# devmentality/LEAStereo

Hardware: AMD Instinct MI355X
Metric: stereo pairs/s at 576×960 D=192, 1/2/4/8 GPU; EPE vs reference (higher is better)
Workload: dtype f32; 1 GPU; SceneFlow 576x960 D=192 fp32, batch 1 per GPU (BASELINE configs[1]); height=576, width=960, maxdisp=192, global_batch=1, parallelism=dp1 (pairs sharded over ranks, no collective in the step), launch=hip graph replay

## Files before the change

### include/leastereo_hip.h

```cpp
#ifndef LEASTEREO_HIP_H
#define LEASTEREO_HIP_H

#include <stddef.h>
#include <stdint.h>

#ifdef __cplusplus
extern "C" {
#endif

#define LEA_ABI_VERSION 14

#define LEA_F32 0
#define LEA_BF16 1

#define LEA_OK 0
#define LEA_E_INVALID 1001
#define LEA_E_UNSUPPORTED 1002

#define LEA_RELU 1u
#define LEA_RESIDUAL 2u
#define LEA_PAIR_SUM 4u

int lea_abi_version(void);
const char* lea_last_error(void);

int lea_build_cost_volume(const void* left, const void* right, void* cost,
                          int B, int C, int H, int W, int D3, int dtype, void* stream);

size_t lea_conv3d_packed_floats(int cout, int cin, int k);

int lea_conv3d_pack_weights(const float* w, float* packed, int cout, int cin, int k,
                            void* stream);

int lea_conv3d_bnrelu(const void* x, int64_t x_bstride,
                      const void* x2, int64_t x2_bstride, int cin2,
                      const float* w_packed, const float* scale, const float* shift,
                      const void* residual, int64_t r_bstride,
                      void* y, int64_t y_bstride,
                      int B, int cin, int cout, int D, int H, int W, int k,
                      unsigned flags, int dtype, void* stream);

int lea_conv3d_bnrelu_resampled(const void* x, int64_t x_bstride, int Di, int Hi, int Wi,
                                const float* w_packed, const float* scale, const float* shift,
                                const void* residual, int64_t r_bstride,
                                void* y, int64_t y_bstride,
                                int B, int cin, int cout, int D, int H, int W, int k,
                                unsigned flags, int dtype, void* stream);

int lea_conv3d_bnrelu_costvolume(const void* left, const void* right, int64_t f_bstride,
                                 const float* w_packed, const float* scale, const float* shift,
                                 void* y, int64_t y_bstride, int B, int C, int cout, int D3,
                                 int H, int W, unsigned flags, int dtype, void* stream);
const char* lea_conv3d_costvolume_kernel_name(int B, int cout, int D3, int H, int W);

const char* lea_conv3d_kernel_name(int B, int cout, int D, int H, int W, int k, int resampled);


size_t lea_conv2d_packed_floats(int cout, int cin);
int lea_conv2d_pack_weights(const float* w, float* packed, int cout, int cin, void* stream);

int lea_conv2d_bnrelu(const void* x, int64_t x_bstride, const float* w_packed,
                      const float* scale, const float* shift, const void* residual,
                      int64_t r_bstride, void* y, int64_t y_bstride, int B, int cin, int cout,
                      int H, int W, unsigned flags, int dtype, void* stream);

const char* lea_conv2d_kernel_name(int B, int cout, int H, int W);

int lea_conv2d_bnrelu_pair(const void* x, int64_t x_bstride, const float* w_packed,
                           const float* scale, const float* shift, const void* residual,
                           int64_t r_bstride, void* y, int64_t y_bstride, void* y2,
                           int64_t y2_bstride, int B, int cin, int cout, int c1, int H, int W,
                           unsigned flags, void* stream);

int lea_conv2d_s3_bnrelu(const void* x, int64_t x_bstride, const float* w, const float* scale,
                         const float* shift, void* y, int64_t y_bstride, int B, int cin, int cout,
                         int Hi, int Wi, unsigned flags, int dtype, void* stream);

int lea_feature_stem_bnrelu(const float* x, int64_t x_bstride, const float* w0, const float* scale0,
                            const float* shift0, const float* w1, const float* scale1,
                            const float* shift1, void* y, int64_t y_bstride, int B, int cin, int c0,
                            int c1, int Hi, int Wi, int dtype, void* stream);


int lea_resample3d_trilinear(const void* x, int64_t x_bstride, void* y, int64_t y_bstride,
                             int B, int C, int Di, int Hi, int Wi, int Do, int Ho, int Wo,
                             int align_corners, const float* scale, const float* shift,
                             unsigned flags, int dtype, void* stream);

size_t lea_tapsum_workspace_bytes(int B, int cout, int Hi, int Wi, int Do);
int lea_tapsum_upsample(const void* q, int64_t q_bstride, void* y, int64_t y_bstride,
                        int B, int cout, int Di, int Hi, int Wi, int Do, int Ho, int Wo,
                        const float* scale, const float* shift, unsigned flags,
                        void* workspace, int dtype, void* stream);

int lea_disparity_regression(const void* cost, float* disp, int B, int D3, int H3, int W3,
                             int maxdisp, int dtype, void* stream);

int lea_disparity_regression_stats(const void* cost, float* disp, float* entropy, float* peak,
                                   float* disp_local, int B, int D3, int H3, int W3, int maxdisp,
                                   int radius, int dtype, void* stream);

int lea_disparity_regression_right(const void* cost, float* disp_right, int B, int D3, int H3,
                                   int W3, int maxdisp, int dtype, void* stream);

int lea_disparity_lr_check(const float* disp_left, const float* disp_right, uint8_t* state,
                           float* disp_filled, int B, int H, int W, float threshold, void* stream);

int lea_median5x5_f32(const float* x, int64_t x_bstride, float* y, int64_t y_bstride, int B,
                      int H, int W, int iterations, void* stream);

size_t lea_edge_loss_workspace_bytes(int B, int H, int W);
int lea_edge_loss_f32(const float* pred, int64_t pred_bstride, const float* target,
                      int64_t target_bstride, const float* tsmooth, int64_t tsmooth_bstride,
                      int B, int H, int W, float maxdisp, double* sums, void* workspace,
                      void* stream);

int lea_edge_loss_grad_f32(const float* pred, int64_t pred_bstride, const float* target,
                           int64_t target_bstride, const float* tsmooth, int64_t tsmooth_bstride,
                           const double* sums, const float* scales, float* dpred,
                           int64_t dpred_bstride, int B, int H, int W, float maxdisp,
                           void* stream);

size_t lea_photometric_workspace_bytes(int B, int H, int W);
// ... 57 lines not shown
int lea_conv3d_bnrelu_costvolume_bf16(const void* left, const void* right, int64_t f_bstride,
                                      const void* w_packed, const float* scale, const float* shift,
                                      void* y, int64_t y_bstride, int B, int C, int cout, int D3,
                                      int H, int W, unsigned flags, void* stream);


const char* lea_conv3d_kernel_name_bf16(int B, int cout, int cin, int D, int H, int W, int k,
                                        int costvolume);

int lea_conv3d_bf16_pair_supported(int B, int cin, int cout, int D, int H, int W);

int lea_conv1x1_resampled_bf16(const void* x, int64_t x_bstride, int Di, int Hi, int Wi,
                               const void* w_packed, const float* scale, const float* shift,
                               void* y, int64_t y_bstride, int B, int cin, int cout, int D, int H,
                               int W, unsigned flags, void* stream);

int lea_resample3d_trilinear_bf16(const void* x, int64_t x_bstride, void* y, int64_t y_bstride,
                                  int B, int C, int Di, int Hi, int Wi, int Do, int Ho, int Wo,
                                  int align_corners, const float* scale, const float* shift,
                                  unsigned flags, void* stream);


int lea_to_c8_bf16(const float* x, int64_t x_bstride, void* y, int64_t y_bstride, int B, int C,
                   int64_t vol, void* stream);
int lea_from_c8_bf16(const void* x, int64_t x_bstride, float* y, int64_t y_bstride, int B, int C,
                     int64_t vol, void* stream);


size_t lea_conv2d_packed_elems_bf16(int cout, int cin);
int lea_conv2d_pack_weights_bf16(const float* w, void* packed, int cout, int cin, void* stream);
int lea_conv2d_bnrelu_bf16(const void* x, int64_t x_bstride, const void* w_packed,
                           const float* scale, const float* shift, const void* residual,
                           int64_t r_bstride, void* y, int64_t y_bstride, int B, int cin, int cout,
                           int H, int W, unsigned flags, void* stream);

size_t lea_conv3d_wino_packed_floats(int cout, int cin);
int lea_conv3d_wino_pack_weights(const float* w, float* packed, int cout, int cin, void* stream);
int lea_conv3d_bnrelu_wino(const void* x, int64_t x_bstride, const void* x2, int64_t x2_bstride,
                           int cin2, const float* w_packed, const float* scale, const float* shift,
                           const void* residual, int64_t r_bstride, void* y, int64_t y_bstride,
                           int B, int cin, int cout, int D, int H, int W, unsigned flags, int dtype,
                           void* stream);
int lea_conv3d_bnrelu_costvolume_wino(const void* left, const void* right, int64_t f_bstride,
                                      const float* w_packed, const float* scale,
                                      const float* shift, void* y, int64_t y_bstride, int B, int C,
                                      int cout, int D3, int H, int W, unsigned flags, int dtype,
                                      void* stream);
const char* lea_conv3d_wino_kernel_name(int B, int cin, int cout, int D, int H, int W, int costvolume);
int lea_conv3d_wino_down2_supported(int B, int cin, int cout, int D, int H, int W);
const char* lea_conv3d_wino_down2_kernel_name(int B, int cin, int cout, int D, int H, int W);
int lea_conv3d_bnrelu_wino_down2(const void* x, int64_t x_bstride, const float* w_packed,
                                 const float* scale, const float* shift, void* y, int64_t y_bstride,
                                 int B, int cin, int cout, int D, int H, int W, unsigned flags, int dtype,
                                 void* stream);
int lea_conv3d_wino_down2_cat_supported(int B, int cin, int cin2, int cout, int D, int H, int W);
const char* lea_conv3d_wino_down2_cat_kernel_name(int B, int cin, int cin2, int cout, int D, int H, int W);
int lea_conv3d_bnrelu_wino_down2_cat(const void* x, int64_t x_bstride, const void* x2, int64_t x2_bstride,
                                     int cin2, const float* w_packed, const float* scale, const float* shift,
                                     void* y, int64_t y_bstride, int B, int cin, int cout, int D, int H,
                                     int W, unsigned flags, int dtype, void* stream);
int lea_conv3d_wino_dp_down2_supported(int B, int cin, int cout, int D, int H, int W);
const char* lea_conv3d_wino_dp_down2_kernel_name(int B, int cin, int cout, int D, int H, int W, int only);
int lea_conv3d_bnrelu_wino_dp_down2(const void* x, int64_t x_bstride, const float* w_packed,
                                    const float* scale, const float* shift, const void* residual,
                                    int64_t r_bstride, void* y, int64_t y_bstride, void* y2,
                                    int64_t y2_bstride, int B, int cin, int cout, int D, int H, int W,
                                    unsigned flags, int dtype, void* stream);
int lea_resample3d_down2_supported(int Di, int Hi, int Wi, int Do, int Ho, int Wo, int dtype);
int lea_resample3d_trilinear_down2(const void* x, int64_t x_bstride, void* y, int64_t y_bstride, void* y2,
                                   int64_t y2_bstride, int B, int C, int Di, int Hi, int Wi, int Do, int Ho,
                                   int Wo, const float* scale, const float* shift, unsigned flags, int dtype,
                                   void* stream);

int lea_cv_stem_split_weights(const float* w, float* wl, float* wr, int cout, int C, void* stream);
int lea_cv_stem_combine(const void* lmaps, int64_t l_bstride, const void* rmaps, int64_t r_bstride,
                        const float* scale, const float* shift, void* y, int64_t y_bstride, int B,
                        int cout, int D3, int H, int W, unsigned flags, int dtype, void* stream);
int lea_cv_stem_down2_supported(int cout, int D3, int H, int W, int dtype);
int lea_cv_stem_combine_down2(const void* lmaps, int64_t l_bstride, const void* rmaps, int64_t r_bstride,
                              const float* scale, const float* shift, void* y, int64_t y_bstride,
                              void* y2, int64_t y2_bstride, int B, int cout, int D3, int H, int W,
                              unsigned flags, int dtype, void* stream);


size_t lea_standardize_workspace_bytes(int B);
int lea_standardize_crop_u8(const void* left, const void* right, int B, int H, int W,
                            int pix_stride, float* out_left, float* out_right, int crop_h,
                            int crop_w, void* workspace, void* stream);

size_t lea_train_transform_workspace_bytes(int B);
int lea_train_transform_u8(const void* left, const void* right, int B, int H, int W, int pix_stride,
                           const float* disp_left, const float* disp_right, const int* params,
                           float* out_left, float* out_right, float* out_target, int crop_h,
                           int crop_w, float maxdisp, int* n_valid, void* workspace, void* stream);


size_t lea_standardize_tiles_workspace_bytes(void);
int lea_standardize_tiles_u8(const void* left, const void* right, int H, int W, int pix_stride,
                             const int* origins, int N, float* out_left, float* out_right, int tile_h,
                             int tile_w, void* workspace, void* stream);

int lea_tile_blend_f32(const float* tiles, int64_t tile_bstride, const int* ys, int ny, const int* xs,
                       int nx, int tile_h, int tile_w, int guard_y0, int guard_y1, int guard_x0,
                       int guard_x1, int ramp, float* out, int H, int W, int* n_uncovered, void* stream);

size_t lea_disparity_metrics_workspace_bytes(int B, int H, int W);
int lea_disparity_metrics(const float* pred, int64_t pred_bstride, const float* gt,
                          int64_t gt_bstride, int B, int H, int W, float maxdisp, int round_pred,
                          int z_shift, int thr1, int thr2, int thr3, unsigned char* correct,
                          double* out, void* workspace, void* stream);


size_t lea_conv3d_wgrad_workspace_bytes(int B, int cin, int cout, int D, int H, int W, int k);
int lea_conv3d_wgrad(const float* x, const float* dz, float* dw, void* workspace, size_t ws_bytes,
                     int B, int cin, int cout, int D, int H, int W, int k, void* stream);

size_t lea_conv2d_wgrad_workspace_bytes(int B, int cin, int cout, int H, int W);
int lea_conv2d_wgrad(const float* x, const float* dz, float* dw, void* workspace, size_t ws_bytes,
                     int B, int cin, int cout, int H, int W, void* stream);

int lea_conv2d_s3_backward_data(const float* dz, const float* w, float* dx, int B, int cin, int cout,
                                int Hi, int Wi, void* stream);
size_t lea_conv2d_s3_wgrad_workspace_bytes(int B, int cin, int cout, int Hi, int Wi);
int lea_conv2d_s3_wgrad(const float* x, const float* dz, float* dw, void* workspace, size_t ws_bytes,
                        int B, int cin, int cout, int Hi, int Wi, void* stream);

int lea_conv3d_flip_weights(const float* w, float* wt, int cout, int cin, int k, void* stream);

size_t lea_bn_workspace_bytes(int C);
int lea_bn_forward_f32(const float* z, float* y, int B, int C, int64_t V, const float* gamma,
                       const float* beta, float* running_mean, float* running_var, float momentum,
                       float eps, int training, unsigned flags, float* mean, float* invstd,
                       void* workspace, void* stream);

int lea_bn_backward_f32(const float* dy, const float* y, const float* z, float* dz, int B, int C,
                        int64_t V, const float* gamma, const float* mean, const float* invstd,
                        int training, unsigned flags, float* dgamma, float* dbeta, void* workspace,
                        void* stream);

size_t lea_resample3d_backward_workspace_bytes(int B, int C, int Di, int Hi, int Wi, int Do, int Ho,
                                               int Wo);
int lea_resample3d_trilinear_backward(const float* dy, float* dx, void* workspace, size_t ws_bytes,
                                      int B, int C, int Di, int Hi, int Wi, int Do, int Ho, int Wo,
                                      int align_corners, void* stream);

int lea_disparity_regression_backward(const float* cost, const float* disp, const float* dout,
                                      float* dV, int B, int D3, int H3, int W3, int maxdisp,
                                      void* stream);

int lea_build_cost_volume_backward(const float* dcost, float* dleft, float* dright, int B, int C,
                                   int H, int W, int D3, void* stream);

#ifdef __cplusplus
}
#endif
#endif
```

### leastereo_amd/_lib.py

```python
from __future__ import annotations

import ctypes
import os
import threading

LIB_PATH = os.environ.get(
    "LEASTEREO_HIP_LIB",
    os.path.join(os.path.dirname(os.path.abspath(__file__)), "libleastereo_hip.so"))

ABI_VERSION = 14
LEA_F32 = 0
LEA_BF16 = 1
LEA_RELU = 1
LEA_RESIDUAL = 2
LEA_PAIR_SUM = 4
LEA_E_INVALID = 1001

_p = ctypes.c_void_p
_i = ctypes.c_int
_i64 = ctypes.c_int64
_u = ctypes.c_uint

SIGNATURES = {
    "lea_abi_version": (_i, []),
    "lea_last_error": (ctypes.c_char_p, []),
    "lea_build_cost_volume": (_i, [_p, _p, _p, _i, _i, _i, _i, _i, _i, _p]),
    "lea_conv3d_packed_floats": (ctypes.c_size_t, [_i, _i, _i]),
    "lea_conv3d_pack_weights": (_i, [_p, _p, _i, _i, _i, _p]),
    "lea_conv3d_bnrelu": (_i, [_p, _i64, _p, _i64, _i, _p, _p, _p, _p, _i64, _p, _i64,
                               _i, _i, _i, _i, _i, _i, _i, _u, _i, _p]),
    "lea_conv3d_bnrelu_resampled": (_i, [_p, _i64, _i, _i, _i, _p, _p, _p, _p, _i64, _p, _i64,
                                         _i, _i, _i, _i, _i, _i, _i, _u, _i, _p]),
    "lea_conv3d_kernel_name": (ctypes.c_char_p, [_i, _i, _i, _i, _i, _i, _i]),
    "lea_conv3d_set_tile_override": (_i, [_i, _i, _i]),
    "lea_conv3d_bnrelu_costvolume": (_i, [_p, _p, _i64, _p, _p, _p, _p, _i64, _i, _i, _i, _i, _i,
                                          _i, _u, _i, _p]),
    "lea_conv3d_costvolume_kernel_name": (ctypes.c_char_p, [_i, _i, _i, _i, _i]),
    "lea_conv2d_packed_floats": (ctypes.c_size_t, [_i, _i]),
    "lea_conv2d_pack_weights": (_i, [_p, _p, _i, _i, _p]),
    "lea_conv2d_bnrelu": (_i, [_p, _i64, _p, _p, _p, _p, _i64, _p, _i64, _i, _i, _i, _i, _i, _u,
                               _i, _p]),
    "lea_conv2d_kernel_name": (ctypes.c_char_p, [_i, _i, _i, _i]),
    "lea_conv2d_s3_bnrelu": (_i, [_p, _i64, _p, _p, _p, _p, _i64, _i, _i, _i, _i, _i, _u, _i, _p]),
    "lea_feature_stem_bnrelu": (_i, [_p, _i64, _p, _p, _p, _p, _p, _p, _p, _i64, _i, _i, _i, _i, _i, _i,
                                     _i, _p]),
    "lea_resample3d_trilinear": (_i, [_p, _i64, _p, _i64, _i, _i, _i, _i, _i, _i, _i, _i,
                                      _i, _p, _p, _u, _i, _p]),
    "lea_tapsum_workspace_bytes": (ctypes.c_size_t, [_i, _i, _i, _i, _i]),
    "lea_tapsum_upsample": (_i, [_p, _i64, _p, _i64, _i, _i, _i, _i, _i, _i, _i, _i, _p, _p, _u,
                                 _p, _i, _p]),
    "lea_disparity_regression": (_i, [_p, _p, _i, _i, _i, _i, _i, _i, _p]),
    "lea_disparity_regression_stats": (_i, [_p, _p, _p, _p, _p, _i, _i, _i, _i, _i, _i, _i, _p]),
    "lea_disparity_regression_right": (_i, [_p, _p, _i, _i, _i, _i, _i, _i, _p]),
    "lea_disparity_lr_check": (_i, [_p, _p, _p, _p, _i, _i, _i, ctypes.c_float, _p]),
    "lea_median5x5_f32": (_i, [_p, _i64, _p, _i64, _i, _i, _i, _i, _p]),
    "lea_edge_loss_workspace_bytes": (ctypes.c_size_t, [_i, _i, _i]),
    "lea_edge_loss_f32": (_i, [_p, _i64, _p, _i64, _p, _i64, _i, _i, _i, ctypes.c_float, _p, _p, _p]),
    "lea_edge_loss_grad_f32": (_i, [_p, _i64, _p, _i64, _p, _i64, _p, _p, _p, _i64, _i, _i, _i,
                                    ctypes.c_float, _p]),
    "lea_photometric_workspace_bytes": (ctypes.c_size_t, [_i, _i, _i]),
    "lea_photometric_f32": (_i, [_p, _i64, _p, _i64, _p, _i64, _p, _i64, _i, _i, _i, _i, ctypes.c_float,
                                 ctypes.c_float, ctypes.c_float, _p, _p, _p, _p, _p]),
    "lea_photometric_grad_f32": (_i, [_p, _i64, _p, _i64, _p, _i64, _p, _i64, _i, _i, _i, _i, ctypes.c_float,
                                      ctypes.c_float, _p, _p, _p, _i64, _p]),
    "lea_disparity_refine_workspace_bytes": (ctypes.c_size_t, [_i, _i, _i]),
    "lea_disparity_refine_f32": (_i, [_p, _i64, _p, _p, _p, _i, _i, _i, _i, ctypes.c_float, ctypes.c_float, _i,
                                      _p, _p, _p, _p]),
    "lea_disparity_speckle_workspace_bytes": (ctypes.c_size_t, [_i, _i, _i]),
    "lea_disparity_speckle_f32": (_i, [_p, _p, _i, _i, _i, ctypes.c_float, _i, ctypes.c_float, _p, _p, _p, _p, _p,
                                       _p]),
    "lea_disparity_pointcloud_workspace_bytes": (ctypes.c_size_t, [_i, _i, _i]),
    "lea_disparity_pointcloud_f32": (_i, [_p, _p, _p, _i, _p, _i64, _i, _i, _i, ctypes.c_float, ctypes.c_float,
                                          ctypes.c_float, _i, _p, _p, _p, _p, _p, _p, _p, _p, _p]),
    "lea_rectify_pair_u8": (_i, [_p, _p, _i, _i, _i, _i, _p, _i, _p, _i, _i, _i, _i, _p, _p, _p, _p, _p]),
    "lea_rectify_set_tile": (_i, [_i]),
    "lea_forward_warp_f32": (_i, [_p, _i64, _p, _i64, _p, _p, _i, _i, _i, _i, ctypes.c_float, ctypes.c_float, _i,
                                  ctypes.c_float, _p, _p, _p, _p, _p]),
    "lea_conv3d_packed_elems_bf16": (ctypes.c_size_t, [_i, _i, _i]),
    "lea_conv3d_pack_weights_bf16": (_i, [_p, _p, _i, _i, _i, _p]),
    "lea_conv3d_bnrelu_bf16": (_i, [_p, _i64, _p, _i64, _i, _p, _p, _p, _p, _i64, _p, _i64,
                                    _i, _i, _i, _i, _i, _i, _i, _u, _p]),
    "lea_conv3d_bnrelu_costvolume_bf16": (_i, [_p, _p, _i64, _p, _p, _p, _p, _i64, _i, _i, _i, _i,
                                               _i, _i, _u, _p]),
    "lea_conv3d_kernel_name_bf16": (ctypes.c_char_p, [_i, _i, _i, _i, _i, _i, _i, _i]),
    "lea_conv3d_bf16_pair_supported": (_i, [_i, _i, _i, _i, _i, _i]),
    "lea_conv3d_bf16_set_tile_override": (_i, [_i, _i, _i]),
    "lea_conv3d_bf16_set_variant": (_i, [_i]),
    "lea_resample3d_trilinear_bf16": (_i, [_p, _i64, _p, _i64, _i, _i, _i, _i, _i, _i, _i, _i,
                                           _i, _p, _p, _u, _p]),
    "lea_resample_bf16_set_batch": (_i, [_i]),
    "lea_resample_bf16_set_cols": (_i, [_i]),
    "lea_conv3d_wino_set_w22": (_i, [_i]),
    "lea_conv3d_bf16_set_pair_split": (_i, [_i]),
    "lea_disparity_set_register_form": (_i, [_i]),
    "lea_tapsum_set_rows": (_i, [_i]),
    "lea_staged_rows": (_i, [_i, _i, _i, _i, _i]),
    "lea_conv1x1_resampled_bf16": (_i, [_p, _i64, _i, _i, _i, _p, _p, _p, _p, _i64, _i, _i, _i, _i, _i,
                                        _i, _u, _p]),
    "lea_to_c8_bf16": (_i, [_p, _i64, _p, _i64, _i, _i, _i64, _p]),
    "lea_conv2d_packed_elems_bf16": (ctypes.c_size_t, [_i, _i]),
    "lea_conv2d_pack_weights_bf16": (_i, [_p, _p, _i, _i, _p]),
    "lea_conv2d_bnrelu_bf16": (_i, [_p, _i64, _p, _p, _p, _p, _i64, _p, _i64, _i, _i, _i, _i, _i,
                                    _u, _p]),
    "lea_from_c8_bf16": (_i, [_p, _i64, _p, _i64, _i, _i, _i64, _p]),
    "lea_conv3d_wino_packed_floats": (ctypes.c_size_t, [_i, _i]),
    "lea_conv3d_wino_pack_weights": (_i, [_p, _p, _i, _i, _p]),
    "lea_conv3d_bnrelu_wino": (_i, [_p, _i64, _p, _i64, _i, _p, _p, _p, _p, _i64, _p, _i64,
                                    _i, _i, _i, _i, _i, _i, _u, _i, _p]),
    "lea_conv3d_bnrelu_costvolume_wino": (_i, [_p, _p, _i64, _p, _p, _p, _p, _i64, _i, _i, _i,
                                               _i, _i, _i, _u, _i, _p]),
    "lea_conv3d_wino_kernel_name": (ctypes.c_char_p, [_i, _i, _i, _i, _i, _i, _i]),
    "lea_conv3d_wino_down2_supported": (_i, [_i, _i, _i, _i, _i, _i]),
    "lea_conv3d_wino_down2_kernel_name": (ctypes.c_char_p, [_i, _i, _i, _i, _i, _i]),
    "lea_conv3d_bnrelu_wino_down2": (_i, [_p, _i64, _p, _p, _p, _p, _i64, _i, _i, _i, _i, _i, _i, _u, _i, _p]),
    "lea_conv3d_wino_down2_cat_supported": (_i, [_i, _i, _i, _i, _i, _i, _i]),
    "lea_conv3d_wino_down2_cat_kernel_name": (ctypes.c_char_p, [_i, _i, _i, _i, _i, _i, _i]),
    "lea_conv3d_bnrelu_wino_down2_cat": (_i, [_p, _i64, _p, _i64, _i, _p, _p, _p, _p, _i64, _i, _i, _i, _i, _i, _i,
                                              _u, _i, _p]),
    "lea_conv3d_wino_dp_down2_supported": (_i, [_i, _i, _i, _i, _i, _i]),
    "lea_conv3d_wino_dp_down2_kernel_name": (ctypes.c_char_p, [_i, _i, _i, _i, _i, _i, _i]),
    "lea_conv3d_bnrelu_wino_dp_down2": (_i, [_p, _i64, _p, _p, _p, _p, _i64, _p, _i64, _p, _i64, _i, _i, _i, _i, _i,
                                             _i, _u, _i, _p]),
    "lea_resample3d_down2_supported": (_i, [_i, _i, _i, _i, _i, _i, _i]),
    "lea_resample3d_trilinear_down2": (_i, [_p, _i64, _p, _i64, _p, _i64, _i, _i, _i, _i, _i, _i, _i, _i, _p, _p,
                                            _u, _i, _p]),
    "lea_conv3d_wino_set_tile_override": (_i, [_i, _i, _i]),
    "lea_conv3d_wino_set_variant": (_i, [_i]),
    "lea_conv3d_wino2_set_walk": (_i, [_i]),
    "lea_conv3d_wino2_set_halo16": (_i, [_i]),
    "lea_conv3d_wino2_set_lane_halo16": (_i, [_i]),
    "lea_conv3d_wino_set_fence": (_i, [_i]),
    "lea_resample_set_mode": (_i, [_i]),
    "lea_conv2d_set_small": (_i, [_i]),
    "lea_conv2d_kernel_name_cin": (ctypes.c_char_p, [_i, _i, _i, _i, _i]),
    "lea_conv2d_bnrelu_pair": (_i, [_p, _i64, _p, _p, _p, _p, _i64, _p, _i64, _p, _i64, _i, _i, _i, _i, _i,
                                    _i, _u, _p]),
    "lea_conv3d_wino2_set_pipeline": (_i, [_i]),
    "lea_conv3d_wino2p_set_wpre": (_i, [_i]),
    "lea_conv3d_wino44_set": (_i, [_i]),
    "lea_conv3d_wino44_set_upre": (_i, [_i]),
    "lea_conv3d_wino44_set_sched": (_i, [_i]),
    "lea_conv3d_wino44_set_group": (_i, [_i]),
    "lea_conv3d_wino_set_epi_buf": (_i, [_i]),
    "lea_conv3d_set_rs_gather": (_i, [_i]),
    "lea_conv1x1_set_vector": (_i, [_i]),
    "lea_conv3d_bf16_set_stream1x1": (_i, [_i]),
    "lea_conv3d_wino_set_small_cout": (_i, [_i]),
    "lea_conv3d_wino_set_block48": (_i, [_i]),
    "lea_cv_stem_split_weights": (_i, [_p, _p, _p, _i, _i, _p]),
    "lea_cv_stem_combine": (_i, [_p, _i64, _p, _i64, _p, _p, _p, _i64, _i, _i, _i, _i, _i, _u, _i,
                                 _p]),
    "lea_cv_stem_down2_supported": (_i, [_i, _i, _i, _i, _i]),
    "lea_cv_stem_combine_down2": (_i, [_p, _i64, _p, _i64, _p, _p, _p, _i64, _p, _i64, _i, _i, _i, _i, _i,
                                       _u, _i, _p]),
    "lea_standardize_workspace_bytes": (ctypes.c_size_t, [_i]),
    "lea_standardize_crop_u8": (_i, [_p, _p, _i, _i, _i, _i, _p, _p, _i, _i, _p, _p]),
    "lea_train_transform_workspace_bytes": (ctypes.c_size_t, [_i]),
    "lea_train_transform_u8": (_i, [_p, _p, _i, _i, _i, _i, _p, _p, _p, _p, _p, _p, _i, _i,
                                    ctypes.c_float, _p, _p, _p]),
    "lea_standardize_tiles_workspace_bytes": (ctypes.c_size_t, []),
    "lea_standardize_tiles_u8": (_i, [_p, _p, _i, _i, _i, _p, _i, _p, _p, _i, _i, _p, _p]),
    "lea_tile_blend_f32": (_i, [_p, _i64, _p, _i, _p, _i, _i, _i, _i, _i, _i, _i, _i, _p, _i, _i, _p, _p]),
    "lea_disparity_metrics_workspace_bytes": (ctypes.c_size_t, [_i, _i, _i]),
    "lea_disparity_metrics": (_i, [_p, _i64, _p, _i64, _i, _i, _i, ctypes.c_float, _i, _i,
                                   _i, _i, _i, _p, _p, _p, _p]),
    "lea_conv3d_wgrad_workspace_bytes": (ctypes.c_size_t, [_i, _i, _i, _i, _i, _i, _i]),
    "lea_conv3d_wgrad": (_i, [_p, _p, _p, _p, ctypes.c_size_t, _i, _i, _i, _i, _i, _i, _i, _p]),
    "lea_conv2d_wgrad_workspace_bytes": (ctypes.c_size_t, [_i, _i, _i, _i, _i]),
    "lea_conv2d_wgrad": (_i, [_p, _p, _p, _p, ctypes.c_size_t, _i, _i, _i, _i, _i, _p]),
    "lea_conv2d_s3_backward_data": (_i, [_p, _p, _p, _i, _i, _i, _i, _i, _p]),
    "lea_conv2d_s3_wgrad_workspace_bytes": (ctypes.c_size_t, [_i, _i, _i, _i, _i]),
    "lea_conv2d_s3_wgrad": (_i, [_p, _p, _p, _p, ctypes.c_size_t, _i, _i, _i, _i, _i, _p]),
    "lea_conv3d_flip_weights": (_i, [_p, _p, _i, _i, _i, _p]),
    "lea_bn_workspace_bytes": (ctypes.c_size_t, [_i]),
    "lea_bn_forward_f32": (_i, [_p, _p, _i, _i, _i64, _p, _p, _p, _p, ctypes.c_float, ctypes.c_float,
                                _i, _u, _p, _p, _p, _p]),
    "lea_bn_backward_f32": (_i, [_p, _p, _p, _p, _i, _i, _i64, _p, _p, _p, _i, _u, _p, _p, _p, _p]),
    "lea_disparity_regression_backward": (_i, [_p, _p, _p, _p, _i, _i, _i, _i, _i, _p]),
    "lea_build_cost_volume_backward": (_i, [_p, _p, _p, _i, _i, _i, _i, _i, _p]),
    "lea_resample3d_backward_workspace_bytes": (ctypes.c_size_t, [_i, _i, _i, _i, _i, _i, _i, _i]),
    "lea_resample3d_trilinear_backward": (_i, [_p, _p, _p, ctypes.c_size_t, _i, _i, _i, _i, _i, _i, _i, _i,
                                               _i, _p]),
}

_lib = None
_lock = threading.Lock()


class HipKernelError(RuntimeError):
    pass


def load():
    global _lib
    if _lib is not None:
        return _lib
    with _lock:
        if _lib is None:
            if not os.path.exists(LIB_PATH):
                raise HipKernelError(
                    f"{LIB_PATH} not found: build it with `make` (hipcc --offload-arch=gfx950); "
                    "the LEAStereo hot path has no fallback")
            lib = ctypes.CDLL(LIB_PATH)
            for name, (res, args) in SIGNATURES.items():
                fn = getattr(lib, name)
                fn.restype = res
                fn.argtypes = args
            _apply_env_tuning(lib)
            _lib = lib
    return _lib


TUNING_ENV = {"LEASTEREO_WINO2_WALK": "lea_conv3d_wino2_set_walk",
              "LEASTEREO_HALO16": "lea_conv3d_wino2_set_halo16",
              "LEASTEREO_LANE_HALO16": "lea_conv3d_wino2_set_lane_halo16",
              "LEASTEREO_WINO_FENCE": "lea_conv3d_wino_set_fence",
              "LEASTEREO_RESAMPLE_MODE": "lea_resample_set_mode",
              "LEASTEREO_CONV2D_SMALL": "lea_conv2d_set_small",
              "LEASTEREO_WINO2_PIPE": "lea_conv3d_wino2_set_pipeline",
              "LEASTEREO_WINO2P_WPRE": "lea_conv3d_wino2p_set_wpre",
              "LEASTEREO_WINO44": "lea_conv3d_wino44_set",
              "LEASTEREO_WINO44_UPRE": "lea_conv3d_wino44_set_upre",
              "LEASTEREO_EPI_BUF": "lea_conv3d_wino_set_epi_buf",
              "LEASTEREO_RS_GATHER": "lea_conv3d_set_rs_gather",
              "LEASTEREO_1X1_VEC": "lea_conv1x1_set_vector",
              "LEASTEREO_BF16_1X1": "lea_conv3d_bf16_set_stream1x1",
              "LEASTEREO_RESAMPLE_K": "lea_resample_bf16_set_batch",
              "LEASTEREO_RESAMPLE_COLS": "lea_resample_bf16_set_cols",
              "LEASTEREO_W22": "lea_conv3d_wino_set_w22",
              "LEASTEREO_PAIR_SPLIT": "lea_conv3d_bf16_set_pair_split",
              "LEASTEREO_DISP_REG": "lea_disparity_set_register_form",
              "LEASTEREO_TAPSUM_ROWS": "lea_tapsum_set_rows"}


# ... 12 lines not shown
```

### leastereo_amd/csrc/conv3d.hip

```cpp
#include "conv3d_impl.h"

namespace lea {

template <int KS, int MT, int NT, int TW, bool RS>
__global__ __launch_bounds__(kConvThreads, 2) void conv3d_reg_kernel(const ConvArgs a) {
  using C = TileCfg<KS, MT, NT, TW>;
  constexpr int CIN_B = C::CIN_B;
  __shared__ __attribute__((aligned(16))) float smem[C::STAGE];
  __shared__ Axis tabs[RS ? (KS + C::RH + C::RW) : 1];
  float* xs = smem;
  float* ws = smem + C::XS;

  const int tid = threadIdx.x;
  const int lane = tid & 63;
  const int wave = tid >> 6;
  const int tile = blockIdx.x;
  const int h0 = (tile / a.tiles_w) * C::TH;
  const int w0 = (tile % a.tiles_w) * TW;
  const int d0 = blockIdx.y;
  const int b = blockIdx.z / a.ncob;
  const int co0 = (blockIdx.z - b * a.ncob) * C::COP;
  const int nchunks = (a.cin + CIN_B - 1) / CIN_B;
  const float* wp = a.wp + (long long)(co0 / C::COP) * nchunks * C::WS;
  const long long HW = (long long)a.H * a.W;
// ... 94 lines not shown
  {
    const float4* src = reinterpret_cast<const float4*>(a.wp + (long long)cob * nch * 32 * COP);
    float4* dst = reinterpret_cast<float4*>(ws);
    for (int i = threadIdx.x; i < nch * 32 * COP / 4; i += 256) dst[i] = src[i];
  }
  float sc[MT][4], sh[MT][4];
#pragma unroll
  for (int m = 0; m < MT; ++m)
#pragma unroll
    for (int r = 0; r < 4; ++r) {
      const int co = co0 + 16 * m + 4 * g + r;
      sc[m][r] = (a.scale && co < a.cout) ? a.scale[co] : 1.f;
      sh[m][r] = (a.scale && co < a.cout) ? a.shift[co] : 0.f;
    }
  __syncthreads();
  const bool relu = a.flags & LEA_RELU, resid = a.flags & LEA_RESIDUAL;
  const int HWo = a.H * a.W;
  const long long vout = (long long)HWo * a.D;
  const unsigned HWi = (unsigned)(a.Hi * a.Wi), vin = HWi * (unsigned)a.Di;
  const __amdgpu_buffer_rsrc_t xrs =
      __builtin_amdgcn_make_buffer_rsrc((void*)(a.x + (long long)b * a.xbs), 0, (int)(unsigned)((long long)a.cin * vin * 4), 0x00020000);
  const long long t0 = ((long long)blockIdx.x * 4 + wave) * tpw;
  for (int tt = 0; tt < tpw; ++tt) {
    const long long v0 = (t0 + tt) * 16;
    if (v0 >= vout) break;
    const long long v = min(v0 + n, vout - 1);
    const int od = (int)(v / HWo), rem = (int)(v - (long long)od * HWo);
    const int oh = rem / a.W, ow = rem - oh * a.W;
    const Axis ad = axis_index(a.rd, od, a.Di, a.D, 1), ah = axis_index(a.rh, oh, a.Hi, a.H, 1),
               aw = axis_index(a.rw, ow, a.Wi, a.W, 1);
    const unsigned r00 = ((unsigned)ad.i0 * HWi + (unsigned)(ah.i0 * a.Wi)) * 4u;
    const unsigned r01 = ((unsigned)ad.i0 * HWi + (unsigned)(ah.i1 * a.Wi)) * 4u;
    const unsigned r10 = ((unsigned)ad.i1 * HWi + (unsigned)(ah.i0 * a.Wi)) * 4u;
    const unsigned r11 = ((unsigned)ad.i1 * HWi + (unsigned)(ah.i1 * a.Wi)) * 4u;
    const unsigned w0 = (unsigned)aw.i0 * 4u, w1 = (unsigned)aw.i1 * 4u;
    f32x4 acc[MT];
#pragma unroll
    for (int m = 0; m < MT; ++m) acc[m] = f32x4{0.f, 0.f, 0.f, 0.f};
    for (int ch = 0; ch < nch; ++ch) {
      float c[8][8];
#pragma unroll
      for (int s = 0; s < 8; ++s) {
        const int ci = ch * 32 + 4 * s + g;
        const unsigned co = ci < a.cin ? (unsigned)ci * vin * 4u : 0u;
        const unsigned rr[4] = {r00, r01, r10, r11};
#pragma unroll
        for (int q = 0; q < 4; ++q) {
          c[s][2 * q] = __builtin_bit_cast(float, __builtin_amdgcn_raw_buffer_load_b32(xrs, co + rr[q] + w0, 0, 0));
          c[s][2 * q + 1] = __builtin_bit_cast(float, __builtin_amdgcn_raw_buffer_load_b32(xrs, co + rr[q] + w1, 0, 0));
        }
      }
#pragma unroll
      for (int s = 0; s < 8; ++s) {
        const float* e = c[s];
        const int ci = ch * 32 + 4 * s + g;
        const float bv = ci >= a.cin ? 0.f :
            ad.l0 * (ah.l0 * (aw.l0 * e[0] + aw.l1 * e[1]) + ah.l1 * (aw.l0 * e[2] + aw.l1 * e[3])) +
            ad.l1 * (ah.l0 * (aw.l0 * e[4] + aw.l1 * e[5]) + ah.l1 * (aw.l0 * e[6] + aw.l1 * e[7]));
#pragma unroll
        for (int m = 0; m < MT; ++m) {
          const int col = 16 * m + n;
          const float av = ws[ci * COP + ((SWZ && (ci & 1)) ? (col ^ 16) : col)];
          acc[m] = __builtin_amdgcn_mfma_f32_16x16x4f32(av, bv, acc[m], 0, 0, 0);
        }
      }
    }
    if (v0 + n < vout) {
#pragma unroll
      for (int m = 0; m < MT; ++m)
#pragma unroll
        for (int r = 0; r < 4; ++r) {
          const int co = co0 + 16 * m + 4 * g + r;
          if (co >= a.cout) continue;
          float y = acc[m][r] * sc[m][r] + sh[m][r];
          if (relu) y = fmaxf(y, 0.f);
          const long long o = (long long)co * vout + v0 + n;
          if (resid) y += a.res[(long long)b * a.rbs + o];
          a.y[(long long)b * a.ybs + o] = y;
        }
    }
  }
}

template <int MT, int NT, bool VEC>
__global__ __launch_bounds__(kConvThreads) void conv1x1_kernel(const ConvArgs a) {
  using P = PackCfg<1, MT>;
  constexpr int CIN_B = P::CIN_B;
  constexpr int KS = CIN_B / 4;
  using vecf = float __attribute__((ext_vector_type(NT)));
  __shared__ __attribute__((aligned(16))) float ws[P::CHUNK];
  const int tid = threadIdx.x;
  const int lane = tid & 63;
  const int wave = tid >> 6;
  const int b = blockIdx.y / a.ncob;
  const int co0 = (blockIdx.y - b * a.ncob) * P::COP;
  const int nchunks = (a.cin + CIN_B - 1) / CIN_B;
  const float* wp = a.wp + (long long)(co0 / P::COP) * nchunks * P::CHUNK;
  const long long V = (long long)a.D * a.H * a.W;
  const long long v0 = ((long long)blockIdx.x * kConvWaves + wave) * NT * 16;
  const int kq = lane >> 4, n = lane & 15;
  auto vox = [&](int j) -> long long { return VEC ? v0 + NT * n + j : v0 + j * 16 + n; };
  const bool full = VEC && vox(NT - 1) < V;

  f32x4 acc[MT][NT];
#pragma unroll
  for (int m = 0; m < MT; ++m)
#pragma unroll
    for (int j = 0; j < NT; ++j) acc[m][j] = f32x4{0.f, 0.f, 0.f, 0.f};

  for (int ch = 0; ch < nchunks; ++ch) {
    float bv[KS][NT];
#pragma unroll
    for (int s = 0; s < KS; ++s) {
      const int c = ch * CIN_B + 4 * s + kq;
      const float* src = (c < a.cin1) ? a.x + (long long)b * a.xbs + (long long)c * V
                                      : a.x2 + (long long)b * a.x2bs + (long long)(c - a.cin1) * V;
      if (VEC && full && c < a.cin) {
        const vecf t = *reinterpret_cast<const vecf*>(src + vox(0));
#pragma unroll
        for (int j = 0; j < NT; ++j) bv[s][j] = t[j];
      } else {
#pragma unroll
        for (int j = 0; j < NT; ++j) {
          const long long v = vox(j);
          bv[s][j] = (c < a.cin && v < V) ? src[v] : 0.f;
        }
      }
    }
    __syncthreads();
    {
      const float4* src = reinterpret_cast<const float4*>(wp + (long long)ch * P::CHUNK);
      float4* dst = reinterpret_cast<float4*>(ws);
#pragma unroll
      for (int i = tid; i < P::CHUNK / 4; i += kConvThreads) dst[i] = src[i];
    }
    __syncthreads();
#pragma unroll
    for (int s = 0; s < KS; ++s) {
      float av[MT];
#pragma unroll
      for (int m = 0; m < MT; ++m) av[m] = ws[(4 * s + kq) * P::COPS + a_col<1, MT>(m, kq, n)];
#pragma unroll
      for (int m = 0; m < MT; ++m)
#pragma unroll
        for (int j = 0; j < NT; ++j)
          acc[m][j] = __builtin_amdgcn_mfma_f32_16x16x4f32(av[m], bv[s][j], acc[m][j], 0, 0, 0);
    }
  }

  const bool relu = a.flags & LEA_RELU;
  const bool resid = a.flags & LEA_RESIDUAL;
#pragma unroll
  for (int m = 0; m < MT; ++m) {
#pragma unroll
    for (int r = 0; r < 4; ++r) {
      const int co = co0 + m * 16 + kq * 4 + r;
      if (co >= a.cout) continue;
      const float sc = a.scale ? a.scale[co] : 1.f;
      const float sh = a.shift ? a.shift[co] : 0.f;
      if (VEC && full) {
        const long long o = (long long)co * V + vox(0);
        vecf val;
#pragma unroll
        for (int j = 0; j < NT; ++j) {
          val[j] = acc[m][j][r] * sc + sh;
          if (relu) val[j] = fmaxf(val[j], 0.f);
        }
        if (resid) {
          const vecf rv = *reinterpret_cast<const vecf*>(a.res + (long long)b * a.rbs + o);
#pragma unroll
          for (int j = 0; j < NT; ++j) val[j] += rv[j];
        }
        *reinterpret_cast<vecf*>(a.y + (long long)b * a.ybs + o) = val;
        continue;
      }
#pragma unroll
      for (int j = 0; j < NT; ++j) {
        const long long v = vox(j);
        if (v >= V) continue;
        const long long o = (long long)co * V + v;
        float val = acc[m][j][r] * sc + sh;
        if (relu) val = fmaxf(val, 0.f);
        if (resid) val += a.res[(long long)b * a.rbs + o];
        a.y[(long long)b * a.ybs + o] = val;
      }
    }
  }
}

template <int COUT>
__global__ __launch_bounds__(kConvThreads) void conv3d_valu_kernel(const ConvArgs a) {
  constexpr int TH = 8, TW = 64, RH = TH + 2, RW = TW + 2, PLANE = RH * RW, IMG = 3 * PLANE;
  constexpr int CIN_B = PackCfg<3, 1>::CIN_B;
  constexpr int CIS = (IMG + 15) / 16 * 16;
  constexpr int STAGE = CIN_B * CIS;
  constexpr int XSLOTS = (IMG + 63) / 64;
  constexpr int XSLOTS_W = (XSLOTS + kConvWaves - 1) / kConvWaves;
  constexpr int CHUNK = PackCfg<3, 1>::CHUNK;
  __shared__ __attribute__((aligned(16))) float smem[2 * STAGE];

  const int tid = threadIdx.x;
  const int lane = tid & 63;
  const int wave = __builtin_amdgcn_readfirstlane(tid >> 6);
  const int h0 = (blockIdx.x / a.tiles_w) * TH;
  const int w0 = (blockIdx.x % a.tiles_w) * TW;
  const int d0 = blockIdx.y;
  const int b = blockIdx.z;
  const int nchunks = (a.cin + CIN_B - 1) / CIN_B;
  const int HW = a.H * a.W;
  const unsigned nrec = (unsigned)(HW * a.D) * 4u;

  unsigned voff[XSLOTS_W];
#pragma unroll
  for (int t = 0; t < XSLOTS_W; ++t) {
    const int e = (wave + kConvWaves * t) * 64 + lane;
    unsigned v = 0xFFFFFFF0u;
    if (e < IMG) {
      const int kd = e / PLANE;
      const int r = e - kd * PLANE;
      const int rr = r / RW;
      const int cc = r - rr * RW;
      const int d = d0 + kd - 1, h = h0 + rr - 1, w = w0 + cc - 1;
      if ((unsigned)d < (unsigned)a.D && (unsigned)h < (unsigned)a.H && (unsigned)w < (unsigned)a.W)
        v = (unsigned)(d * HW + h * a.W + w) * 4u;
    }
    voff[t] = v;
  }
  auto issue = [&](int ch, float* st) {
#pragma unroll
    for (int ci = 0; ci < CIN_B; ++ci) {
      const int c = ch * CIN_B + ci;
      const float* base = a.x;
      unsigned n = 0;
      if (c < a.cin1) {
        base = a.x + (long long)b * a.xbs + (long long)c * HW * a.D;
        n = nrec;
      } else if (c < a.cin) {
        base = a.x2 + (long long)b * a.x2bs + (long long)(c - a.cin1) * HW * a.D;
        n = nrec;
      }
      const __amdgpu_buffer_rsrc_t rs = __builtin_amdgcn_make_buffer_rsrc((void*)base, 0, n, 0x00020000);
#pragma unroll
      for (int t = 0; t < XSLOTS_W; ++t) {
        const int j = wave + kConvWaves * t;
        if (j < XSLOTS && j * 64 + lane < IMG)
          __builtin_amdgcn_raw_ptr_buffer_load_lds(rs, (lds_void*)(st + ci * CIS + j * 64), 4,
                                                   voff[t], 0, 0, 0);
      }
    }
  };

  const int row = tid >> 5;
  const int col = (tid & 31) * 2;
  float acc[COUT][2];
#pragma unroll
  for (int co = 0; co < COUT; ++co) acc[co][0] = acc[co][1] = 0.f;

  issue(0, smem);
  for (int ch = 0; ch < nchunks; ++ch) {
    asm volatile("s_waitcnt vmcnt(0)" ::: "memory");
    __syncthreads();
    if (ch + 1 < nchunks) issue(ch + 1, smem + ((ch + 1) & 1) * STAGE);
    const float* xs = smem + (ch & 1) * STAGE;
    const float* wc = a.wp + (long long)ch * CHUNK;
#pragma unroll
    for (int ci = 0; ci < CIN_B; ++ci) {
#pragma unroll
      for (int kd = 0; kd < 3; ++kd) {
#pragma unroll
        for (int kh = 0; kh < 3; ++kh) {
// ... 125 lines not shown

inline Plan make_plan(int B, int cout, int D, int H, int W, int k, bool resample) {
  Plan p;
  p.td = 1;
  p.mt = mt_for(cout);
  if (k == 1 && resample && g_rs_gather && (long long)B * D * H * W <= 131072) {
    p.engine = 5;
    p.nt = 0;
    p.tw = 0;
    return p;
  }
  if (k == 1 && !resample) {
    p.engine = 1;
    p.nt = 4;
    p.tw = 0;
    const long long vox = (long long)D * H * W;
    if ((vox + kConvWaves * 64 - 1) / (kConvWaves * 64) * B < 512) p.nt = 2;
    return p;
  }
  if (k == 3 && cout <= 2 && !resample) {
    p.engine = 3;
    p.mt = cout;
    p.nt = 0;
    p.tw = 64;
    return p;
  }
  if (depth_paired(cout, k) && !resample) {
    p.engine = 4;
    p.mt = 1;
    p.tw = 16;
    p.td = 1;
    const long long wgs8 = (long long)((W + 15) / 16) * ((H + 7) / 8) * ((D + 1) / 2) * B;
    p.nt = wgs8 >= 512 ? 2 : 1;
    return p;
  }
  p.engine = resample ? 2 : 0;
  p.tw = prefer_tw64(W) ? 64 : 32;
  p.td = 1;
  if (resample) {
    p.nt = (k == 1) ? (p.mt == 1 ? 2 : 1) : (p.mt == 1 ? 8 : 4);
    return p;
  }
  const long long ncob = (cout + p.mt * 16 - 1) / (p.mt * 16);
  if (g_tile_override[0] > 0) {
    p.nt = g_tile_override[0];
    p.tw = g_tile_override[1];
    p.td = g_tile_override[2];
    return p;
  }
  auto wgs = [&](int nt, int td) {
    const int th = kConvWaves * nt;
    return (long long)((W + 15) / 16) * ((H + th - 1) / th) * ((D + td - 1) / td) * B * ncob;
  };
  p.tw = 16;
  p.nt = 2;
  p.td = wgs(2, 2) >= 384 ? 2 : 1;
  if (p.td == 1 && wgs(2, 1) < 256) p.nt = 1;
  return p;
}

template <typename K>
int launch(K kernel, const ConvArgs& a0, int th, int tw, int B, hipStream_t st, int td = 1) {
  ConvArgs a = a0;
  const long long nt = (long long)((a.W + tw - 1) / tw) * ((a.H + th - 1) / th);
  LEA_CHECK_ARG(nt < (1LL << 31) && a.D <= 65535 && (long long)B * a.ncob <= 65535,
                "lea_conv3d: grid too large");
  a.tiles_w = (a.W + tw - 1) / tw;
  dim3 grid((unsigned)nt, (a.D + td - 1) / td, B * a.ncob);
  kernel<<<grid, kConvThreads, 0, st>>>(a);
  return launch_status("lea_conv3d");
}

#define LEA_TILE_TH(KS, MT, NT, TW) (TileCfg<KS, MT, NT, TW>::TH)

template <int KS, int MT, int NT>
int run_rs(const ConvArgs& a, int tw, int B, hipStream_t st) {
  if (tw == 64) return launch(conv3d_reg_kernel<KS, MT, NT, 64, true>, a, LEA_TILE_TH(KS, MT, NT, 64), 64, B, st);
  return launch(conv3d_reg_kernel<KS, MT, NT, 32, true>, a, LEA_TILE_TH(KS, MT, NT, 32), 32, B, st);
}

int g_1x1_vec = 1;

template <int MT, int NT>
int launch_1x1(const ConvArgs& a, int B, hipStream_t st) {
  const long long vox = (long long)a.D * a.H * a.W;
  const long long per = kConvWaves * NT * 16;
  const long long gx = (vox + per - 1) / per;
  LEA_CHECK_ARG(gx < (1LL << 31) && (long long)B * a.ncob <= 65535, "lea_conv3d: grid too large");
  auto al = [](const void* q) { return q == nullptr || ((uintptr_t)q % (NT * 4)) == 0; };
  const bool vec = g_1x1_vec && vox % NT == 0 && al(a.x) && al(a.x2) && al(a.y) && al(a.res) &&
                   a.xbs % NT == 0 && a.x2bs % NT == 0 && a.ybs % NT == 0 && a.rbs % NT == 0;
  if (vec) conv1x1_kernel<MT, NT, true><<<dim3((unsigned)gx, B * a.ncob), kConvThreads, 0, st>>>(a);
  else conv1x1_kernel<MT, NT, false><<<dim3((unsigned)gx, B * a.ncob), kConvThreads, 0, st>>>(a);
  return launch_status("lea_conv3d");
}

int run_1x1(const Plan& p, const ConvArgs& a, int B, hipStream_t st) {
  if (p.mt == 1) return p.nt == 4 ? launch_1x1<1, 4>(a, B, st) : launch_1x1<1, 2>(a, B, st);
  if (p.mt == 2) return p.nt == 4 ? launch_1x1<2, 4>(a, B, st) : launch_1x1<2, 2>(a, B, st);
  if (p.mt == 3) return p.nt == 4 ? launch_1x1<3, 4>(a, B, st) : launch_1x1<3, 2>(a, B, st);
  return p.nt == 4 ? launch_1x1<4, 4>(a, B, st) : launch_1x1<4, 2>(a, B, st);
}

template <int MT>
int launch_rs_gather(ConvArgs a, int B, hipStream_t st) {
  const long long vout = (long long)a.D * a.H * a.W;
  const long long tiles = (vout + 15) / 16;
  const long long tpw = std::max(1LL, (tiles * B * a.ncob + 8191) / 8192);
  const long long gx = (tiles + 4 * tpw - 1) / (4 * tpw);
  LEA_CHECK_ARG(gx < (1LL << 31) && (long long)B * a.ncob <= 65535, "lea_conv3d: grid too large");
  conv1x1_rs_f32_kernel<MT><<<dim3((unsigned)gx, B * a.ncob), 256, 0, st>>>(a, (int)tpw);
  return launch_status("lea_conv3d(rs gather)");
}

int run_plan(const Plan& p, ConvArgs a, int B, int k, hipStream_t st) {
  a.ncob = (a.cout + p.mt * 16 - 1) / (p.mt * 16);
  if (p.engine == 5) {
    const long long xbytes = (long long)a.cin * a.Di * a.Hi * a.Wi * 4;
    if (a.cin <= kRsMaxCin && a.cin1 == a.cin && xbytes < 0xFFFFFF00LL) {
      if (p.mt == 1) return launch_rs_gather<1>(a, B, st);
      if (p.mt == 2) return launch_rs_gather<2>(a, B, st);
      if (p.mt == 3) return launch_rs_gather<3>(a, B, st);
      return launch_rs_gather<4>(a, B, st);
    }
    if (p.mt == 1) return run_rs<1, 1, 2>(a, prefer_tw64(a.W) ? 64 : 32, B, st);
    if (p.mt == 2) return run_rs<1, 2, 1>(a, prefer_tw64(a.W) ? 64 : 32, B, st);
    if (p.mt == 3) return run_rs<1, 3, 1>(a, prefer_tw64(a.W) ? 64 : 32, B, st);
    return run_rs<1, 4, 1>(a, prefer_tw64(a.W) ? 64 : 32, B, st);
  }
  if (p.engine == 3) {
    if (a.cout == 1) return launch(conv3d_valu_kernel<1>, a, 8, 64, B, st);
    return launch(conv3d_valu_kernel<2>, a, 8, 64, B, st);
  }
  if (p.engine == 4) return run_dma_dp(p, a, B, st);
  if (p.engine == 0) {
    if (p.mt == 1) return run_dma_mt1(p, a, B, st);
    if (p.mt == 2) return run_dma_mt2(p, a, B, st);
    if (p.mt == 3) return run_dma_mt3(p, a, B, st);
    return run_dma_mt4(p, a, B, st);
  }
  if (p.engine == 2) {
    if (k == 3) {
      if (p.mt == 1) return run_rs<3, 1, 8>(a, p.tw, B, st);
      if (p.mt == 2) return run_rs<3, 2, 4>(a, p.tw, B, st);
      if (p.mt == 3) return run_rs<3, 3, 4>(a, p.tw, B, st);
      return run_rs<3, 4, 4>(a, p.tw, B, st);
    }
    if (p.mt == 1) return run_rs<1, 1, 2>(a, p.tw, B, st);
    if (p.mt == 2) return run_rs<1, 2, 1>(a, p.tw, B, st);
    if (p.mt == 3) return run_rs<1, 3, 1>(a, p.tw, B, st);
    return run_rs<1, 4, 1>(a, p.tw, B, st);
  }
  return run_1x1(p, a, B, st);
}

thread_local char g_name[96];

const char* plan_name(const Plan& p, int k) {
  if (p.engine == 5)
    snprintf(g_name, sizeof(g_name), "conv1x1_rs_f32_kernel<%d>", p.mt);
  else if (p.engine == 3)
    snprintf(g_name, sizeof(g_name), "conv3d_valu_kernel<%d>", p.mt == 1 ? 1 : 2);
  else if (p.engine == 0)
    snprintf(g_name, sizeof(g_name), "conv3d_dma_kernel<%d, %d, %d, %d, %d, false>", p.mt, p.nt,
             p.tw, p.td, k == 2 ? 1 : 3);
  else if (p.engine == 4)
    snprintf(g_name, sizeof(g_name), "conv3d_dma_kernel<1, %d, %d, 1, 4, false>", p.nt, p.tw);
  else if (p.engine == 2)
    snprintf(g_name, sizeof(g_name), "conv3d_reg_kernel<%d, %d, %d, %d, true>", k, p.mt, p.nt, p.tw);
  else
    snprintf(g_name, sizeof(g_name), "conv1x1_kernel<%d, %d>", p.mt, p.nt);
  return g_name;
}

size_t packed_floats_2d(int cout, int cin) {
  const int mt = mt_for(cout);
  return mt == 1 ? packed_floats_t<3, 1, 1>(cout, cin)
         : mt == 2 ? packed_floats_t<3, 2, 1>(cout, cin)
         : mt == 3 ? packed_floats_t<3, 3, 1>(cout, cin) : packed_floats_t<3, 4, 1>(cout, cin);
}

inline Plan make_plan_2d(int B, int cout, int H, int W) {
  Plan p;
  p.engine = 0;
// ... 55 lines not shown
}

extern "C" int lea_conv1x1_set_vector(int on) {
  lea::clear_error();
  LEA_CHECK_ARG(on == 0 || on == 1, "lea_conv1x1_set_vector: on=%d", on);
  lea::g_1x1_vec = on;
  return 0;
}

extern "C" int lea_conv3d_set_tile_override(int nt, int tw, int td) {
  lea::clear_error();
  if (nt <= 0) {
    lea::g_tile_override[0] = 0;
    return 0;
  }
  LEA_CHECK_ARG((tw == 16 || tw == 32 || tw == 64) && (td == 1 || td == 2) &&
                    (nt == 1 || nt == 2 || nt == 4 || nt == 8),
                "lea_conv3d_set_tile_override: bad tile nt=%d tw=%d td=%d", nt, tw, td);
  lea::g_tile_override[0] = nt;
  lea::g_tile_override[1] = tw;
  lea::g_tile_override[2] = td;
  return 0;
}

extern "C" size_t lea_conv3d_packed_floats(int cout, int cin, int k) {
  if (cout <= 0 || cin <= 0 || (k != 1 && k != 3)) return 0;
  return lea::packed_floats(cout, cin, k);
}

extern "C" int lea_conv3d_pack_weights(const float* w, float* packed, int cout, int cin, int k,
                                       void* stream) {
  using namespace lea;
  clear_error();
  LEA_CHECK_ARG(w && packed, "lea_conv3d_pack_weights: null pointer");
  LEA_CHECK_ARG(cout > 0 && cin > 0 && (k == 1 || k == 3),
                "lea_conv3d_pack_weights: unsupported shape cout=%d cin=%d k=%d", cout, cin, k);
  const long long total = (long long)packed_floats(cout, cin, k);
  const int threads = 256;
  const long long want = (total + threads - 1) / threads;
  const int grid = (int)(want < 4096 ? want : 4096);
  const int mt = mt_for(cout);
  hipStream_t st = as_stream(stream);
  const int cin_b = k == 3 ? PackCfg<3, 1>::CIN_B : PackCfg<1, 1>::CIN_B;
  const int nchunks = (cin + cin_b - 1) / cin_b;
#define LEA_PACK(KS, MT) \
  pack_weights_kernel<KS, MT><<<grid, threads, 0, st>>>(w, packed, cout, cin, nchunks, total)
  if (depth_paired(cout, k)) {
    pack_weights_dp_kernel<<<grid, threads, 0, st>>>(w, packed, cout, cin, nchunks, total);
  } else if (k == 3) {
    if (mt == 1) LEA_PACK(3, 1); else if (mt == 2) LEA_PACK(3, 2); else if (mt == 3) LEA_PACK(3, 3); else LEA_PACK(3, 4);
  } else {
    if (mt == 1) LEA_PACK(1, 1); else if (mt == 2) LEA_PACK(1, 2); else if (mt == 3) LEA_PACK(1, 3); else LEA_PACK(1, 4);
  }
#undef LEA_PACK
  return launch_status("lea_conv3d_pack_weights");
}

extern "C" int lea_conv3d_bnrelu(const void* x, int64_t x_bstride, const void* x2,
                                 int64_t x2_bstride, int cin2, const float* w_packed,
                                 const float* scale, const float* shift, const void* residual,
                                 int64_t r_bstride, void* y, int64_t y_bstride, int B, int cin,
                                 int cout, int D, int H, int W, int k, unsigned flags, int dtype,
                                 void* stream) {
  lea::ConvArgs a{};
  a.x = (const float*)x;
  a.xbs = x_bstride;
  a.x2 = (const float*)x2;
  a.x2bs = x2_bstride;
  a.cin1 = cin - cin2;
  a.wp = w_packed;
  a.scale = scale;
  a.shift = shift;
  a.res = (const float*)residual;
  a.rbs = r_bstride;
  a.y = (float*)y;
  a.ybs = y_bstride;
  a.cin = cin;
  a.cout = cout;
  a.D = D;
  a.H = H;
  a.W = W;
  a.flags = flags;
  return lea::conv_common(a, B, k, false, dtype, stream);
}

extern "C" size_t lea_conv2d_packed_floats(int cout, int cin) {
  if (cout <= 0 || cin <= 0) return 0;
  return lea::packed_floats_2d(cout, cin);
}

extern "C" int lea_conv2d_pack_weights(const float* w, float* packed, int cout, int cin,
                                       void* stream) {
  using namespace lea;
  clear_error();
  LEA_CHECK_ARG(w && packed, "lea_conv2d_pack_weights: null pointer");
  LEA_CHECK_ARG(cout > 0 && cin > 0, "lea_conv2d_pack_weights: bad shape cout=%d cin=%d", cout, cin);
  const long long total = (long long)packed_floats_2d(cout, cin);
  const int threads = 256;
  const long long want = (total + threads - 1) / threads;
  const int grid = (int)(want < 4096 ? want : 4096);
  const int nchunks = (cin + PackCfg<3, 1, 1>::CIN_B - 1) / PackCfg<3, 1, 1>::CIN_B;
  hipStream_t st = as_stream(stream);
  switch (mt_for(cout)) {
    case 1: pack_weights_kernel<3, 1, 1><<<grid, threads, 0, st>>>(w, packed, cout, cin, nchunks, total); break;
    case 2: pack_weights_kernel<3, 2, 1><<<grid, threads, 0, st>>>(w, packed, cout, cin, nchunks, total); break;
    case 3: pack_weights_kernel<3, 3, 1><<<grid, threads, 0, st>>>(w, packed, cout, cin, nchunks, total); break;
    default: pack_weights_kernel<3, 4, 1><<<grid, threads, 0, st>>>(w, packed, cout, cin, nchunks, total);
  }
  return launch_status("lea_conv2d_pack_weights");
}

extern "C" const char* lea_conv2d_kernel_name(int B, int cout, int H, int W) {
  if (B <= 0 || cout <= 0 || H <= 0 || W <= 0) return nullptr;
  return lea::plan_name(lea::make_plan_2d(B, cout, H, W), 2);
}

extern "C" int lea_conv2d_bnrelu(const void* x, int64_t x_bstride, const float* w_packed,
                                 const float* scale, const float* shift, const void* residual,
                                 int64_t r_bstride, void* y, int64_t y_bstride, int B, int cin,
                                 int cout, int H, int W, unsigned flags, int dtype, void* stream) {
  using namespace lea;
  clear_error();
  ConvArgs a{};
  a.x = (const float*)x;
  a.xbs = x_bstride;
  a.cin1 = cin;
  a.wp = w_packed;
  a.scale = scale;
  a.shift = shift;
  a.res = (const float*)residual;
  a.rbs = r_bstride;
  a.y = (float*)y;
  a.ybs = y_bstride;
  a.cin = cin;
  a.cout = cout;
  a.D = 1;
  a.H = H;
  a.W = W;
  a.flags = flags;
  LEA_CHECK_ARG(a.x && a.wp && a.y, "lea_conv2d: null pointer");
  LEA_CHECK_ARG((a.scale == nullptr) == (a.shift == nullptr),
                "lea_conv2d: scale/shift must both be set or both NULL");
  LEA_CHECK_FLAGS(flags, LEA_RELU | LEA_RESIDUAL, "lea_conv2d");
  LEA_CHECK_ARG(!(flags & LEA_RESIDUAL) || a.res, "lea_conv2d: LEA_RESIDUAL without residual");
  LEA_CHECK_ARG(B > 0 && cin > 0 && cout > 0 && H > 0 && W > 0,
                "lea_conv2d: bad shape B=%d cin=%d cout=%d H=%d W=%d", B, cin, cout, H, W);
  LEA_CHECK_ARG((long long)(cout + 63) * H * W < (1LL << 31), "lea_conv2d: plane too large");
  LEA_CHECK_ARG(a.x != a.y, "lea_conv2d: input aliases output");
  if (dtype != LEA_F32) {
    set_error("lea_conv2d: dtype %d unsupported", dtype);
    return LEA_E_UNSUPPORTED;
  }
  hipStream_t st = as_stream(stream);
  if (conv2d_small_ok(cin, cout)) return run_conv2d_small(a, B, st);
  const Plan p = make_plan_2d(B, cout, H, W);
  a.ncob = (cout + p.mt * 16 - 1) / (p.mt * 16);
  switch (p.mt) {
    case 1: return run_dma2d_mt1(p, a, B, st);
    case 2: return run_dma2d_mt2(p, a, B, st);
    case 3: return run_dma2d_mt3(p, a, B, st);
    default: return run_dma2d_mt4(p, a, B, st);
  }
}

extern "C" const char* lea_conv3d_costvolume_kernel_name(int B, int cout, int D3, int H, int W) {
  if (B <= 0 || cout <= 0 || D3 <= 0 || H <= 0 || W <= 0) return nullptr;
  const lea::Plan p = lea::make_plan(B, cout, D3, H, W, 3, false);
  if (p.engine != 0) return nullptr;
  snprintf(lea::g_name, sizeof(lea::g_name), "conv3d_dma_kernel<%d, %d, %d, %d, 3, true>", p.mt, p.nt,
           p.tw, p.td);
  return lea::g_name;
}

extern "C" int lea_conv3d_bnrelu_costvolume(const void* left, const void* right, int64_t f_bstride,
                                            const float* w_packed, const float* scale,
                                            const float* shift, void* y, int64_t y_bstride, int B,
                                            int C, int cout, int D3, int H, int W, unsigned flags,
                                            int dtype, void* stream) {
  using namespace lea;
  clear_error();
  ConvArgs a{};
  a.x = (const float*)left;
  a.xbs = f_bstride;
  a.x2 = (const float*)right;
  a.x2bs = f_bstride;
  a.cin1 = C;
  a.wp = w_packed;
  a.scale = scale;
  a.shift = shift;
  a.y = (float*)y;
  a.ybs = y_bstride;
  a.cin = 2 * C;
  a.cout = cout;
  a.D = D3;
  a.H = H;
  a.W = W;
  a.flags = flags & LEA_RELU;
  LEA_CHECK_FLAGS(flags, LEA_RELU, "lea_conv3d_bnrelu_costvolume");
  LEA_CHECK_ARG(left && right && w_packed && y && y != left && y != right,
                "lea_conv3d_bnrelu_costvolume: null or aliased pointer");
  LEA_CHECK_ARG((scale == nullptr) == (shift == nullptr),
                "lea_conv3d_bnrelu_costvolume: scale/shift must both be set or both NULL");
  LEA_CHECK_ARG(B > 0 && C > 0 && cout > 0 && D3 > 0 && H > 0 && W > 0,
                "lea_conv3d_bnrelu_costvolume: bad shape B=%d C=%d cout=%d D3=%d H=%d W=%d", B, C,
                cout, D3, H, W);
  constexpr int kCinB = PackCfg<3, 1>::CIN_B;
  LEA_CHECK_ARG(C % kCinB == 0, "lea_conv3d_bnrelu_costvolume: C=%d must be a multiple of %d", C,
                kCinB);
  LEA_CHECK_ARG((long long)(cout + 63) * D3 * H * W < (1LL << 31),
                "lea_conv3d_bnrelu_costvolume: volume too large");
  if (dtype != LEA_F32) {
    set_error("lea_conv3d_bnrelu_costvolume: dtype %d unsupported", dtype);
    return LEA_E_UNSUPPORTED;
  }
  const Plan p = make_plan(B, cout, D3, H, W, 3, false);
  LEA_CHECK_ARG(p.engine == 0, "lea_conv3d_bnrelu_costvolume: no DMA plan for cout=%d", cout);
  a.ncob = (cout + p.mt * 16 - 1) / (p.mt * 16);
  hipStream_t st = as_stream(stream);
  switch (p.mt) {
    case 1: return run_dma_cv_mt1(p, a, B, st);
    case 2: return run_dma_cv_mt2(p, a, B, st);
    case 3: return run_dma_cv_mt3(p, a, B, st);
    default: return run_dma_cv_mt4(p, a, B, st);
  }
}

extern "C" int lea_conv3d_bnrelu_resampled(const void* x, int64_t x_bstride, int Di, int Hi,
                                           int Wi, const float* w_packed, const float* scale,
                                           const float* shift, const void* residual,
                                           int64_t r_bstride, void* y, int64_t y_bstride, int B,
                                           int cin, int cout, int D, int H, int W, int k,
                                           unsigned flags, int dtype, void* stream) {
  lea::ConvArgs a{};
  a.x = (const float*)x;
  a.xbs = x_bstride;
  a.cin1 = cin;
  a.wp = w_packed;
  a.scale = scale;
  a.shift = shift;
  a.res = (const float*)residual;
  a.rbs = r_bstride;
  a.y = (float*)y;
  a.ybs = y_bstride;
  a.cin = cin;
  a.cout = cout;
// ... 13 lines not shown
```

### leastereo_amd/csrc/conv3d_impl.h

```cpp
#pragma once
#include "common.h"

namespace lea {

constexpr int kConvWaves = 4;
constexpr int kConvThreads = kConvWaves * kWave;

using f32x4 = __attribute__((__vector_size__(4 * sizeof(float)))) float;
using lds_void = __attribute__((address_space(3))) void;

__host__ __device__ constexpr int cout_stride(int cop) { return (cop % 32 == 0) ? cop + 16 : cop; }
__host__ __device__ constexpr int round_16mod32(int n) {
  return (n % 32 <= 16) ? n + (16 - n % 32) : n + (48 - n % 32);
}

struct ConvArgs {
  const float* x;
  long long xbs;
  const float* x2;
  long long x2bs;
  int cin1;
  const float* wp;
  const float* scale;
  const float* shift;
  const float* res;
  long long rbs;
  float* y;
  long long ybs;
  int cin, cout, D, H, W;
  int Di, Hi, Wi;
  float rd, rh, rw;
  int tiles_w, ncob;
  int ntiles, ndz, nblk;
  unsigned flags;
  int spw;
  unsigned* dbg;
  float* y2;
  long long y2bs;
  int csplit;
  long long uoff;
  int grp;
};

template <int KS, int MT, int KD = KS>
struct PackCfg {
  static constexpr int KT = KD * KS * KS;
  static constexpr int CIN_B = (KS == 3) ? 4 : 32;
  static constexpr int COP = MT * 16;
  static constexpr int COPS = COP;
  static constexpr bool SWZ = (COP % 32) == 0;
  static constexpr int CHUNK = KT * CIN_B * COPS;
};

template <int KS, int MT>
__device__ __forceinline__ int a_col(int m, int kq, int n) {
  return ((PackCfg<KS, MT>::SWZ ? (m ^ (kq & 1)) : m) * 16) + n;
}

template <int KS, int MT, int NT, int TW, int TD = 1, int KD = KS>
struct TileCfg : PackCfg<KS, MT, KD> {
  using P = PackCfg<KS, MT, KD>;
  static constexpr int PAD = KS / 2;
  static constexpr int NTILES = kConvWaves * NT;
  static constexpr int TPR = TW / 16;
  static constexpr int TH = NTILES / TPR;
  static_assert(NTILES % TPR == 0, "tile rows");
  static constexpr int RH = TH + KS - 1;
  static constexpr int RW = TW + KS - 1;
  static constexpr int PLANE = RH * RW;
  static constexpr int PLANES = KD + TD - 1;
  static constexpr int IMG = PLANES * PLANE;
  static constexpr int CIS = round_16mod32(IMG);
  static constexpr int XS = P::CIN_B * CIS;
  static constexpr int WS = P::CHUNK;
  static constexpr int STAGE = XS + WS;
  static_assert(XS % 16 == 0 && WS % 16 == 0, "16-byte aligned LDS regions");
};

template <int KS, int MT, int NT, int TW, int TD, int KD = KS>
__device__ __forceinline__ void mfma_chunk(const float* xs, const float* ws, const int (&xoff)[NT],
                                           const int (&woff)[MT], f32x4 (&acc)[TD][MT][NT]) {
  using C = TileCfg<KS, MT, NT, TW, TD, KD>;
  constexpr int CIN_B = C::CIN_B;
#pragma unroll
  for (int s = 0; s < CIN_B / 4; ++s) {
#pragma unroll
    for (int kd = 0; kd < KD; ++kd) {
#pragma unroll
      for (int kh = 0; kh < KS; ++kh) {
#pragma unroll
        for (int kw = 0; kw < KS; ++kw) {
          const int tap = (kd * KS + kh) * KS + kw;
          float av[MT], bv[TD][NT];
#pragma unroll
          for (int m = 0; m < MT; ++m) av[m] = ws[woff[m] + (tap * CIN_B + 4 * s) * C::COPS];
#pragma unroll
          for (int t = 0; t < TD; ++t)
#pragma unroll
            for (int j = 0; j < NT; ++j)
              bv[t][j] = xs[xoff[j] + 4 * s * C::CIS + (t + kd) * C::PLANE + kh * C::RW + kw];
#pragma unroll
          for (int t = 0; t < TD; ++t)
#pragma unroll
            for (int m = 0; m < MT; ++m)
#pragma unroll
              for (int j = 0; j < NT; ++j)
                acc[t][m][j] =
                    __builtin_amdgcn_mfma_f32_16x16x4f32(av[m], bv[t][j], acc[t][m][j], 0, 0, 0);
        }
      }
    }
  }
}

template <int KS, int MT, int NT, int TW, int TD>
__device__ __forceinline__ void epilogue(const ConvArgs& a, const f32x4 (&acc)[TD][MT][NT], int b,
                                         int co0, int d0, int h0, int w0, int wave, int lane) {
  using C = TileCfg<KS, MT, NT, TW, TD>;
  const long long HW = (long long)a.H * a.W;
  const long long DHW = HW * a.D;
  const bool relu = a.flags & LEA_RELU;
  const bool resid = a.flags & LEA_RESIDUAL;
  const int kq = lane >> 4, n = lane & 15;
#pragma unroll
// ... 81 lines not shown
      e.sc[m][r] = (cv && a.scale) ? a.scale[co] : 1.f;
      e.sh[m][r] = (cv && a.shift) ? a.shift[co] : 0.f;
    }
  if constexpr (RES) {
    const bool resid = a.flags & LEA_RESIDUAL;
    const float* rb = a.res + (long long)b * a.rbs + g.base;
#pragma unroll
    for (int t = 0; t < TD; ++t)
#pragma unroll
      for (int m = 0; m < MT; ++m)
#pragma unroll
        for (int j = 0; j < NT; ++j)
#pragma unroll
          for (int r = 0; r < 4; ++r)
            e.rv[t][m][j][r] =
                (resid && (g.interior || g.inside(a, m, r, t, j))) ? rb[g.rel(m, r, t, j)] : 0.f;
  }
}

template <int KS, int MT, int NT, int TW, int TD, bool RES, int KD>
__device__ __forceinline__ void epilogue_dma(const ConvArgs& a, const f32x4 (&acc)[TD][MT][NT],
                                             const EpiRegs<MT, NT, TD, RES>& e,
                                             const EpiGeom<KS, MT, NT, TW, TD, KD>& g, int b) {
  const bool relu = a.flags & LEA_RELU;
  const bool resid = a.flags & LEA_RESIDUAL;
  float* yb = a.y + (long long)b * a.ybs + g.base;
  const float* rb = a.res + (long long)b * a.rbs + g.base;
  auto value = [&](int m, int r, int t, int j) {
    float v = acc[t][m][j][r] * e.sc[m][r] + e.sh[m][r];
    if (relu) v = fmaxf(v, 0.f);
    if (resid) {
      if constexpr (RES)
        v += e.rv[t][m][j][r];
      else
        v += rb[g.rel(m, r, t, j)];
    }
    return v;
  };
  if (g.interior) {
#pragma unroll
    for (int t = 0; t < TD; ++t)
#pragma unroll
      for (int m = 0; m < MT; ++m)
#pragma unroll
        for (int j = 0; j < NT; ++j)
#pragma unroll
          for (int r = 0; r < 4; ++r) yb[g.rel(m, r, t, j)] = value(m, r, t, j);
  } else {
#pragma unroll
    for (int t = 0; t < TD; ++t)
#pragma unroll
      for (int m = 0; m < MT; ++m)
#pragma unroll
        for (int j = 0; j < NT; ++j)
#pragma unroll
          for (int r = 0; r < 4; ++r)
            if (g.inside(a, m, r, t, j)) yb[g.rel(m, r, t, j)] = value(m, r, t, j);
  }
}

template <int MT, int NT, int TW, int TD, int KD = 3, bool CV = false>
__global__ __launch_bounds__(kConvThreads, 2) void conv3d_dma_kernel(const ConvArgs a) {
  using C = TileCfg<3, MT, NT, TW, TD, KD>;
  static_assert(KD != 4 || (MT == 1 && TD == 1), "depth pairing is an MT=1, TD=1 tile");
  constexpr int DSTEP = KD == 4 ? 2 : TD;
  constexpr int DOFF = KD == 4 ? 1 : KD / 2;
  constexpr int XSLOTS = (C::IMG + 63) / 64;
  constexpr int XSLOTS_W = (XSLOTS + kConvWaves - 1) / kConvWaves;
  constexpr int WSLOTS = (C::WS + 255) / 256;
  constexpr int WSLOTS_W = (WSLOTS + kConvWaves - 1) / kConvWaves;
  __shared__ __attribute__((aligned(16))) float smem[2 * C::STAGE];

  const int tid = threadIdx.x;
  const int lane = tid & 63;
  const int wave = __builtin_amdgcn_readfirstlane(tid >> 6);
  const int nblk = a.nblk;
  const int xcd = blockIdx.x % 8, idx = blockIdx.x / 8;
  const int q8 = nblk / 8, r8 = nblk % 8;
  const int lin = (xcd < r8 ? xcd * (q8 + 1) : r8 * (q8 + 1) + (xcd - r8) * q8) + idx;
  const int dz = lin % a.ndz;
  const int tile = (lin / a.ndz) % a.ntiles;
  const int bc = lin / (a.ndz * a.ntiles);
  const int h0 = (tile / a.tiles_w) * C::TH;
  const int w0 = (tile % a.tiles_w) * TW;
  const int d0 = dz * DSTEP;
  const int b = bc / a.ncob;
  const int co0 = (bc - b * a.ncob) * C::COP;
  const int nchunks = (a.cin + C::CIN_B - 1) / C::CIN_B;
  const float* wp = a.wp + (long long)(co0 / C::COP) * nchunks * C::WS;
  const int HW = a.H * a.W;
  const unsigned nrec = (unsigned)(HW * a.D) * 4u;

  unsigned voff[XSLOTS_W], voffr[CV ? XSLOTS_W : 1];
#pragma unroll
  for (int t = 0; t < XSLOTS_W; ++t) {
    const int e = (wave + kConvWaves * t) * 64 + lane;
    unsigned v = 0xFFFFFFF0u, vr = 0xFFFFFFF0u;
    if (e < C::IMG) {
      const int kd = e / C::PLANE;
      const int r = e - kd * C::PLANE;
      const int rr = r / C::RW;
      const int cc = r - rr * C::RW;
      const int d = d0 + kd - DOFF, h = h0 + rr - 1, w = w0 + cc - 1;
      if ((unsigned)d < (unsigned)a.D && (unsigned)h < (unsigned)a.H && (unsigned)w < (unsigned)a.W) {
        if constexpr (CV) {
          if (w >= d) {
            v = (unsigned)(h * a.W + w) * 4u;
            vr = (unsigned)(h * a.W + w - d) * 4u;
          }
        } else {
          v = (unsigned)(d * HW + h * a.W + w) * 4u;
        }
      }
    }
    voff[t] = v;
    if constexpr (CV) voffr[t] = vr;
  }

  auto issue = [&](int ch, float* st) {
    const float* wsrc = wp + (long long)ch * C::WS;
    float* wdst = st + C::XS;
#pragma unroll
    for (int t = 0; t < WSLOTS_W; ++t) {
      const int j = wave + kConvWaves * t;
      if (j < WSLOTS && j * 256 + lane * 4 < C::WS)
        __builtin_amdgcn_global_load_lds(wsrc + j * 256 + lane * 4, (lds_void*)(wdst + j * 256), 16, 0, 0);
    }
#pragma unroll
    for (int ci = 0; ci < C::CIN_B; ++ci) {
      const int c = ch * C::CIN_B + ci;
      const float* base = a.x;
      unsigned n = 0;
      const long long cvol = CV ? (long long)HW : (long long)HW * a.D;
      const unsigned crec = CV ? (unsigned)HW * 4u : nrec;
      if (c < a.cin1) {
        base = a.x + (long long)b * a.xbs + (long long)c * cvol;
        n = crec;
      } else if (c < a.cin) {
        base = a.x2 + (long long)b * a.x2bs + (long long)(c - a.cin1) * cvol;
        n = crec;
      }
      const __amdgpu_buffer_rsrc_t rs = __builtin_amdgcn_make_buffer_rsrc((void*)base, 0, n, 0x00020000);
      const unsigned rmask = (CV && c >= a.cin1) ? 0xFFFFFFFFu : 0u;
#pragma unroll
      for (int t = 0; t < XSLOTS_W; ++t) {
        const int j = wave + kConvWaves * t;
        unsigned vo = voff[t];
        if constexpr (CV) vo = voff[t] ^ ((voff[t] ^ voffr[t]) & rmask);
        if (j < XSLOTS && j * 64 + lane < C::IMG)
          __builtin_amdgcn_raw_ptr_buffer_load_lds(rs, (lds_void*)(st + ci * C::CIS + j * 64), 4,
                                                   vo, 0, 0, 0);
      }
    }
  };

  const int kq = lane >> 4;
  const int n = lane & 15;
  int xoff[NT];
#pragma unroll
  for (int j = 0; j < NT; ++j) {
    const int g = wave * NT + j;
    xoff[j] = kq * C::CIS + (g / C::TPR) * C::RW + (g % C::TPR) * 16 + n;
  }
  int woff[MT];
#pragma unroll
  for (int m = 0; m < MT; ++m) woff[m] = kq * C::COPS + a_col<3, MT>(m, kq, n);

  f32x4 acc[TD][MT][NT];
#pragma unroll
  for (int t = 0; t < TD; ++t)
#pragma unroll
    for (int m = 0; m < MT; ++m)
#pragma unroll
      for (int j = 0; j < NT; ++j) acc[t][m][j] = f32x4{0.f, 0.f, 0.f, 0.f};

  issue(0, smem);
  constexpr bool RES = TD * MT * NT <= 8;
  const EpiGeom<3, MT, NT, TW, TD, KD> geo(a, co0, d0, h0, w0, wave, lane);
  EpiRegs<MT, NT, TD, RES> epi;
  epi_prefetch<3, MT, NT, TW, TD, RES, KD>(a, epi, geo, b);
  for (int ch = 0; ch < nchunks; ++ch) {
    asm volatile("s_waitcnt vmcnt(0)" ::: "memory");
    __syncthreads();
    if (ch + 1 < nchunks) issue(ch + 1, smem + ((ch + 1) & 1) * C::STAGE);
    const float* xs = smem + (ch & 1) * C::STAGE;
    mfma_chunk<3, MT, NT, TW, TD, KD>(xs, xs + C::XS, xoff, woff, acc);
  }
  epilogue_dma<3, MT, NT, TW, TD, RES, KD>(a, acc, epi, geo, b);
}

struct Plan {
  int engine;
  int mt, nt, tw, td;
};

template <typename K>
int launch_dma(K kernel, const ConvArgs& a0, int th, int tw, int td, int B, hipStream_t st) {
  ConvArgs a = a0;
  a.tiles_w = (a.W + tw - 1) / tw;
  a.ntiles = a.tiles_w * ((a.H + th - 1) / th);
  a.ndz = (a.D + td - 1) / td;
  const long long n = (long long)a.ntiles * a.ndz * B * a.ncob;
  LEA_CHECK_ARG(n < (1LL << 31), "lea_conv3d: grid too large");
  a.nblk = (int)n;
  kernel<<<dim3((unsigned)n), kConvThreads, 0, st>>>(a);
  return launch_status("lea_conv3d");
}

#define LEA_DMA_TW_ALL(X, MT, NT, TD) X(MT, NT, 16, TD) X(MT, NT, 32, TD) X(MT, NT, 64, TD)
#define LEA_DMA_TW_BIG(X, MT, NT, TD) X(MT, NT, 32, TD) X(MT, NT, 64, TD)
#define LEA_DMA_LIST_1(X)                                                               \
  LEA_DMA_TW_ALL(X, 1, 1, 1) LEA_DMA_TW_ALL(X, 1, 2, 1) LEA_DMA_TW_BIG(X, 1, 4, 1)      \
  LEA_DMA_TW_BIG(X, 1, 8, 1) LEA_DMA_TW_ALL(X, 1, 1, 2) LEA_DMA_TW_ALL(X, 1, 2, 2)      \
  LEA_DMA_TW_BIG(X, 1, 4, 2)
#define LEA_DMA_LIST_2(X)                                                               \
  LEA_DMA_TW_ALL(X, 2, 1, 1) LEA_DMA_TW_ALL(X, 2, 2, 1) LEA_DMA_TW_BIG(X, 2, 4, 1)      \
  LEA_DMA_TW_ALL(X, 2, 1, 2) LEA_DMA_TW_ALL(X, 2, 2, 2) LEA_DMA_TW_BIG(X, 2, 4, 2)
#define LEA_DMA_LIST_3(X)                                                               \
  LEA_DMA_TW_ALL(X, 3, 1, 1) LEA_DMA_TW_ALL(X, 3, 2, 1) LEA_DMA_TW_BIG(X, 3, 4, 1)      \
  LEA_DMA_TW_ALL(X, 3, 1, 2) LEA_DMA_TW_ALL(X, 3, 2, 2)
#define LEA_DMA_LIST_4(X)                                                               \
  LEA_DMA_TW_ALL(X, 4, 1, 1) LEA_DMA_TW_ALL(X, 4, 2, 1) LEA_DMA_TW_ALL(X, 4, 1, 2)      \
  X(4, 2, 16, 2) X(4, 2, 32, 2)

#define LEA_DMA_CV_LIST(X, MT) \
  X(MT, 1, 16, 1, 3) X(MT, 2, 16, 1, 3) X(MT, 1, 16, 2, 3) X(MT, 2, 16, 2, 3)

#define LEA_DMA2D_LIST(X, MT) X(MT, 1, 16, 1, 1) X(MT, 2, 16, 1, 1)
#define LEA_DMA_DP_LIST(X) X(1, 1, 16, 1, 4) X(1, 2, 16, 1, 4)

#define LEA_DMA_DECL(MT)                                                  \
  int dma_lds_bytes_mt##MT(int nt, int tw, int td);                       \
  int run_dma_mt##MT(const Plan& p, const ConvArgs& a, int B, hipStream_t st);   \
  int run_dma2d_mt##MT(const Plan& p, const ConvArgs& a, int B, hipStream_t st);
#define LEA_DMA_DECL_CV(MT) \
  int run_dma_cv_mt##MT(const Plan& p, const ConvArgs& a, int B, hipStream_t st);
LEA_DMA_DECL_CV(1)
LEA_DMA_DECL_CV(2)
LEA_DMA_DECL_CV(3)
LEA_DMA_DECL_CV(4)
#undef LEA_DMA_DECL_CV
int run_dma_dp(const Plan& p, const ConvArgs& a, int B, hipStream_t st);
bool conv2d_small_ok(int cin, int cout);
int run_conv2d_small(const ConvArgs& a, int B, hipStream_t st);
LEA_DMA_DECL(1)
LEA_DMA_DECL(2)
LEA_DMA_DECL(3)
LEA_DMA_DECL(4)
#undef LEA_DMA_DECL

#define LEA_DMA_LDS_CASE(MT, NT, TW, TD) \
  if (nt == NT && tw == TW && td == TD) return 2 * TileCfg<3, MT, NT, TW, TD>::STAGE * 4;
#define LEA_DMA_RUN_CASE(MT, NT, TW, TD)                                                      \
  if (p.nt == NT && p.tw == TW && p.td == TD)                                                 \
    return launch_dma(conv3d_dma_kernel<MT, NT, TW, TD>, a, TileCfg<3, MT, NT, TW, TD>::TH, TW, \
                      TD, B, st);
#define LEA_DMA2D_RUN_CASE(MT, NT, TW, TD, KD)                                           \
  if (p.nt == NT && p.tw == TW && p.td == TD)                                             \
    return launch_dma(conv3d_dma_kernel<MT, NT, TW, TD, KD>,                              \
                      a, TileCfg<3, MT, NT, TW, TD, KD>::TH, TW, TD, B, st);
#define LEA_DMA_DP_RUN_CASE(MT, NT, TW, TD, KD)                                          \
  if (p.nt == NT && p.tw == TW)                                                           \
    return launch_dma(conv3d_dma_kernel<MT, NT, TW, TD, KD>,                              \
                      a, TileCfg<3, MT, NT, TW, TD, KD>::TH, TW, 2, B, st);
#define LEA_DMA_CV_RUN_CASE(MT, NT, TW, TD, KD)                                          \
  if (p.nt == NT && p.tw == TW && p.td == TD)                                             \
    return launch_dma(conv3d_dma_kernel<MT, NT, TW, TD, KD, true>,                        \
                      a, TileCfg<3, MT, NT, TW, TD, KD>::TH, TW, TD, B, st);
#define LEA_DMA_TU(MT)                                                            \
  int dma_lds_bytes_mt##MT(int nt, int tw, int td) {                              \
    LEA_DMA_LIST_##MT(LEA_DMA_LDS_CASE) return 0;                                 \
  }                                                                               \
  int run_dma_mt##MT(const Plan& p, const ConvArgs& a, int B, hipStream_t st) {   \
    LEA_DMA_LIST_##MT(LEA_DMA_RUN_CASE)                                           \
    set_error("lea_conv3d: no DMA tile <%d, %d, %d, %d>", MT, p.nt, p.tw, p.td);  \
    return LEA_E_UNSUPPORTED;                                                     \
  }                                                                               \
  int run_dma2d_mt##MT(const Plan& p, const ConvArgs& a, int B, hipStream_t st) { \
    LEA_DMA2D_LIST(LEA_DMA2D_RUN_CASE, MT)                                        \
    set_error("lea_conv2d: no DMA tile <%d, %d, %d, 1, 1>", MT, p.nt, p.tw);     \
    return LEA_E_UNSUPPORTED;                                                     \
  }                                                                               \
// ... 8 lines not shown
```

### leastereo_amd/csrc/cv_stem.hip

```cpp
#include "common.h"

namespace lea {
namespace cvs {

using bf16x8 = __attribute__((ext_vector_type(8))) __bf16;
constexpr int kThreads = 256;
constexpr int WS = 64;

struct Args {
  const void* lk;
  long long lbs;
  const void* rk;
  long long rbs;
  const float* scale;
  const float* shift;
  void* y;
  long long ybs;
  int cout, D, H, W, nseg, ncob;
  int nds, dchunk;
  unsigned flags;
  float* y2;
  long long y2bs;
  float rd, rh, rw;
};

constexpr int kLdsBytes = 80 * 1024;

__device__ __forceinline__ int stage_u(int p, int NU, int u0, int w0, int D) {
  return p < NU ? u0 + p : (p < NU + WS ? w0 + p - NU : w0 + p - NU - WS - (D - 1));
}
__device__ __forceinline__ float stage_sum(int p, int NU, const float bz[3]) {
  return p < NU ? bz[0] + bz[1] + bz[2] : (p < NU + WS ? bz[1] + bz[2] : bz[0] + bz[1]);
}
__device__ __forceinline__ long long bz_offset(int kd, int z, int o, int cout, long long HW, int W) {
  return (z >= 0 && z < W) ? (long long)(kd * cout + o) * HW + z : (long long)((3 + kd) * cout + o) * HW;
}
__device__ __forceinline__ bool bz_valid(int z, int W) { return z >= -1 && z < W; }
__device__ __forceinline__ bool plane_valid(int d, int kd, int D) {
  return d + kd - 1 >= 0 && d + kd - 1 < D;
}

__device__ __forceinline__ float left_sum(const float lk[3][3], int d, int u, int D) {
  float s = 0.f;
#pragma unroll
  for (int kd = 0; kd < 3; ++kd) {
    const int t = kd - u;
    const float v = t <= 0 ? lk[kd][0] : (t == 1 ? lk[kd][1] : (t == 2 ? lk[kd][2] : 0.f));
    if (plane_valid(d, kd, D)) s += v;
  }
  return s;
}

struct Tile {
  int D, H, W, NU, NT, h, cob, b, d0, d1, w0, u0;
  long long HW;
};

__device__ __forceinline__ Tile tile_of(const Args& a, int rows) {
  Tile t;
  t.D = a.D;
  t.H = a.H;
  t.W = a.W;
  t.NU = a.dchunk + WS - 1;
  t.NT = t.NU + 2 * WS;
  int blk = blockIdx.x;
  const int seg = blk % a.nseg;
  blk /= a.nseg;
  const int ds = blk % a.nds;
  blk /= a.nds;
  t.h = blk % rows;
  blk /= rows;
  t.cob = blk % a.ncob;
  t.b = blk / a.ncob;
  t.d0 = ds * a.dchunk;
  t.d1 = min(a.D, t.d0 + a.dchunk);
  t.w0 = seg * WS;
  t.u0 = t.w0 - (t.d0 + a.dchunk - 1);
  t.HW = (long long)a.H * a.W;
  return t;
}

constexpr int OB = 16;

template <int OB = 16>
__device__ __forceinline__ void stage_row_f32(const Args& a, const Tile& T, const float* rkh, float* rs,
                                              float* corr) {
  const int D = T.D, W = T.W, NU = T.NU, NT = T.NT, d0 = T.d0, d1 = T.d1, w0 = T.w0;
  const long long HW = T.HW;
  const int tid = threadIdx.x;
  const int NE = OB * NT;
  for (int e0 = 0; e0 < NE; e0 += 4 * kThreads) {
    float q[4][3];
#pragma unroll
    for (int k = 0; k < 4; ++k) {
      const int e = min(e0 + k * kThreads + tid, NE - 1);
      const int ol = e / NT, p = e % NT;
      const int o = min(T.cob * OB + ol, a.cout - 1), u = stage_u(p, NU, T.u0, w0, D);
#pragma unroll
      for (int kd = 0; kd < 3; ++kd) q[k][kd] = rkh[bz_offset(kd, u - kd + 1, o, a.cout, HW, W)];
    }
#pragma unroll
    for (int k = 0; k < 4; ++k) {
      const int e = e0 + k * kThreads + tid;
      if (e >= NE) break;
      const int ol = e / NT, p = e % NT;
      const bool ok = T.cob * OB + ol < a.cout;
      const int u = stage_u(p, NU, T.u0, w0, D);
      float bz[3];
#pragma unroll
      for (int kd = 0; kd < 3; ++kd) bz[kd] = (ok && bz_valid(u - kd + 1, W)) ? q[k][kd] : 0.f;
      rs[e] = stage_sum(p, NU, bz);
    }
  }
  if (w0 + WS >= W) {
    const int dl = d1 - d0;
    for (int e = tid; e < OB * dl; e += kThreads) {
      const int ol = e / dl, d = d0 + e % dl;
      const int o = min(T.cob * OB + ol, a.cout - 1);
      float v[3];
#pragma unroll
      for (int kd = 0; kd < 3; ++kd) {
        const int x = min(max(W + 1 - d - kd, 0), W - 1);
        v[kd] = rkh[(long long)((3 + kd) * a.cout + o) * HW + x];
      }
      float s = 0.f;
#pragma unroll
      for (int kd = 0; kd < 3; ++kd) {
        const int x = W + 1 - d - kd;
        if (plane_valid(d, kd, D) && x >= 0 && x < W) s += v[kd];
      }
      corr[ol * a.dchunk + (d - d0)] = s;
    }
  }
}

__global__ __launch_bounds__(kThreads) void cv_stem_f32_kernel(const Args a) {
  extern __shared__ float rs[];
  const Tile T = tile_of(a, a.H);
  const int D = T.D, W = T.W, NU = T.NU, NT = T.NT, d0 = T.d0, d1 = T.d1, w0 = T.w0;
  const long long HW = T.HW;
  if (a.flags & 0x100u) {
    const int ol = threadIdx.x >> 4, o = T.cob * OB + ol, w = w0 + 4 * (threadIdx.x & 15);
    if (o >= a.cout || w >= W) return;
    float* yp = static_cast<float*>(a.y) + T.b * a.ybs + (long long)o * D * HW + (long long)T.h * W + w;
    for (int d = d0; d < d1; ++d) *reinterpret_cast<float4*>(yp + (long long)d * HW) = make_float4(d, 0.f, 0.f, 1.f);
    return;
  }
  const float* lk = static_cast<const float*>(a.lk) + T.b * a.lbs;
  const float* rkh = static_cast<const float*>(a.rk) + T.b * a.rbs + (long long)T.h * W;
  float* corr = rs + OB * NT;
  const int tid = threadIdx.x;
  stage_row_f32(a, T, rkh, rs, corr);
  __syncthreads();

  const int ol = tid >> 4, o = T.cob * OB + ol;
  const int w = w0 + 4 * (tid & 15);
  if (o >= a.cout || w >= W) return;
  const bool band = w - (d1 - 1) <= 1;
  float lkv[3][3][4];
#pragma unroll
  for (int kd = 0; kd < 3; ++kd)
#pragma unroll
    for (int t = 0; t < 3; ++t) {
      float4 v = make_float4(0.f, 0.f, 0.f, 0.f);
      if (t == 0 || band)
        v = *reinterpret_cast<const float4*>(lk + (long long)((3 * kd + t) * a.cout + o) * HW +
                                             (long long)T.h * W + w);
      lkv[kd][t][0] = v.x;
      lkv[kd][t][1] = v.y;
      lkv[kd][t][2] = v.z;
      lkv[kd][t][3] = v.w;
    }
  const float sc = a.scale ? a.scale[o] : 1.f, sh = a.scale ? a.shift[o] : 0.f;
  const float lo = (a.flags & LEA_RELU) ? 0.f : -INFINITY;
  const float* r0 = rs + ol * NT;
  const float* cr = corr + ol * a.dchunk - d0;
  float* yp = static_cast<float*>(a.y) + T.b * a.ybs + (long long)o * D * HW + (long long)T.h * W + w;
  const int jedge = W - 1 - w;
  auto store = [&](int d, const float pre[4]) {
    float4 out;
    float* po = reinterpret_cast<float*>(&out);
#pragma unroll
    for (int j = 0; j < 4; ++j) {
      po[j] = fmaxf(pre[j] * sc + sh, lo);
    }
    *reinterpret_cast<float4*>(yp + (long long)d * HW) = out;
  };
  auto boundary = [&](int d, int pbase) {
    float pre[4];
#pragma unroll
    for (int j = 0; j < 4; ++j) {
      float l3[3][3];
#pragma unroll
      for (int kd = 0; kd < 3; ++kd)
#pragma unroll
        for (int t = 0; t < 3; ++t) l3[kd][t] = lkv[kd][t][j];
      pre[j] = left_sum(l3, d, w + j - d, D) + r0[pbase + (w - w0) + j] - (j == jedge ? cr[d] : 0.f);
    }
    store(d, pre);
  };
  if (d0 == 0) boundary(0, NU);
  if (d1 == D) boundary(D - 1, NU + WS);
  float gl[4], bl[4][4];
#pragma unroll
  for (int j = 0; j < 4; ++j) {
    float l3[3][3];
#pragma unroll
    for (int kd = 0; kd < 3; ++kd)
#pragma unroll
      for (int t = 0; t < 3; ++t) l3[kd][t] = lkv[kd][t][j];
    gl[j] = lkv[0][0][j] + lkv[1][0][j] + lkv[2][0][j];
#pragma unroll
    for (int m = 0; m < 4; ++m) bl[m][j] = left_sum(l3, 1, m - 2, D);
  }
  const int da = max(d0, 1), db = min(d1, D - 1);
  if (w0 - (db - 1) >= 2) {
    for (int d = da; d < db; ++d) {
      const int iu = w - d - T.u0;
      const float c = cr[d];
      float pre[4];
#pragma unroll
      for (int j = 0; j < 4; ++j) pre[j] = gl[j] + r0[iu + j] - (j == jedge ? c : 0.f);
      store(d, pre);
    }
    return;
  }
  for (int d = da; d < db; ++d) {
    const int iu = w - d - T.u0;
    const float c = cr[d];
    float pre[4];
#pragma unroll
    for (int j = 0; j < 4; ++j) {
      const int u = w + j - d;
      float l = u >= 2 ? gl[j] : 0.f;
#pragma unroll
      for (int m = 0; m < 4; ++m) l = u == m - 2 ? bl[m][j] : l;
      pre[j] = l + r0[iu + j] - (j == jedge ? c : 0.f);
    }
    store(d, pre);
  }
}

__device__ __forceinline__ float lerp2(float l0, float v0, float l1, float v1) {
#pragma clang fp contract(off)
  return l0 * v0 + l1 * v1;
}

constexpr int OBD = 8;

__global__ __launch_bounds__(kThreads) void cv_stem_f32_down2_kernel(const Args a) {
  extern __shared__ float rs[];
  const Tile T = tile_of(a, a.H / 2);
  const int D = T.D, H = T.H, W = T.W, NU = T.NU, NT = T.NT, w0 = T.w0, hp = T.h;
  const long long HW = T.HW;
  const float* lk = static_cast<const float*>(a.lk) + T.b * a.lbs;
  const float* rk = static_cast<const float*>(a.rk) + T.b * a.rbs;
  const int rowf = OBD * (NT + a.dchunk);
  const int tid = threadIdx.x;
#pragma unroll
  for (int r = 0; r < 2; ++r)
    stage_row_f32<OBD>(a, T, rk + (long long)(2 * hp + r) * W, rs + r * rowf, rs + r * rowf + OBD * NT);
  __syncthreads();

  const int r = (tid >> 5) & 1;
  const int ol = ((tid >> 6) << 1) | ((tid >> 4) & 1), o = T.cob * OBD + ol;
  const int w = w0 + 4 * (tid & 15);
  if (o >= a.cout || w >= W) return;
  const bool band = w - (D - 1) <= 1;
  float gl[4], bl[4][4], lf[4], ll[4];
  {
    float lkv[3][3][4];
#pragma unroll
    for (int kd = 0; kd < 3; ++kd)
#pragma unroll
      for (int t = 0; t < 3; ++t) {
        float4 v = make_float4(0.f, 0.f, 0.f, 0.f);
        if (t == 0 || band)
          v = *reinterpret_cast<const float4*>(lk + (long long)((3 * kd + t) * a.cout + o) * HW +
                                               (long long)(2 * hp + r) * W + w);
        lkv[kd][t][0] = v.x;
        lkv[kd][t][1] = v.y;
        lkv[kd][t][2] = v.z;
        lkv[kd][t][3] = v.w;
      }
#pragma unroll
    for (int j = 0; j < 4; ++j) {
      float l3[3][3];
#pragma unroll
      for (int kd = 0; kd < 3; ++kd)
#pragma unroll
        for (int t = 0; t < 3; ++t) l3[kd][t] = lkv[kd][t][j];
      gl[j] = lkv[0][0][j] + lkv[1][0][j] + lkv[2][0][j];
#pragma unroll
      for (int m = 0; m < 4; ++m) bl[m][j] = left_sum(l3, 1, m - 2, D);
      lf[j] = left_sum(l3, 0, w + j, D);
      ll[j] = left_sum(l3, D - 1, w + j - (D - 1), D);
    }
  }
  const float sc = a.scale ? a.scale[o] : 1.f, sh = a.scale ? a.shift[o] : 0.f;
  const float lo = (a.flags & LEA_RELU) ? 0.f : -INFINITY;
  const int jedge = W - 1 - w;
  const bool far = w0 - (D - 2) >= 2;
  float* yp = static_cast<float*>(a.y) + T.b * a.ybs + (long long)o * D * HW + (long long)(2 * hp + r) * W + w;
  const int D2 = D / 2, H2 = H / 2, W2 = W / 2;
  float* y2p = a.y2 + T.b * a.y2bs + ((long long)o * D2 * H2 + hp) * W2 + w / 2 + r;
  Axis aw[2];
#pragma unroll
  for (int c = 0; c < 2; ++c) aw[c] = axis_index(a.rw, w / 2 + c, W, W2, 1);
  const Axis ah = axis_index(a.rh, hp, H, H2, 1);
  const bool h0odd = ah.i0 & 1, h1odd = ah.i1 & 1;
  const float* r0 = rs + r * rowf + ol * NT;
  const float* cr = rs + r * rowf + OBD * NT + ol * a.dchunk;

  float ev[2] = {0.f, 0.f};
  for (int d = 0; d < D; ++d) {
    const float c = cr[d];
    float pre[4];
    if (d == 0 || d == D - 1) {
      const int pb = (d == 0 ? NU : NU + WS) + (w - w0);
#pragma unroll
      for (int j = 0; j < 4; ++j) pre[j] = (d == 0 ? lf[j] : ll[j]) + r0[pb + j] - (j == jedge ? c : 0.f);
    } else {
      const int iu = w - d - T.u0;
#pragma unroll
      for (int j = 0; j < 4; ++j) {
        const int u = w + j - d;
        float l = (far || u >= 2) ? gl[j] : 0.f;
        if (!far) {
#pragma unroll
          for (int m = 0; m < 4; ++m) l = u == m - 2 ? bl[m][j] : l;
        }
        pre[j] = l + r0[iu + j] - (j == jedge ? c : 0.f);
      }
    }
    float4 o4;
    float* out = reinterpret_cast<float*>(&o4);
#pragma unroll
    for (int j = 0; j < 4; ++j) out[j] = fmaxf(pre[j] * sc + sh, lo);
    *reinterpret_cast<float4*>(yp + (long long)d * HW) = o4;
    float hv[2];
#pragma unroll
    for (int k = 0; k < 2; ++k) {
      const float v0 = (aw[k].i0 & 1) ? out[2 * k + 1] : out[2 * k];
      const float v1 = (aw[k].i1 & 1) ? out[2 * k + 1] : out[2 * k];
      const float mine = lerp2(aw[k].l0, v0, aw[k].l1, v1);
      const float other = __shfl_xor(mine, 32);
      const float row0 = r ? other : mine, row1 = r ? mine : other;
      hv[k] = lerp2(ah.l0, h0odd ? row1 : row0, ah.l1, h1odd ? row1 : row0);
    }
    if (!(d & 1)) {
      ev[0] = hv[0];
      ev[1] = hv[1];
    } else {
      const Axis ad = axis_index(a.rd, d >> 1, D, D2, 1);
      const float e = r ? ev[1] : ev[0], v = r ? hv[1] : hv[0];
      y2p[(long long)(d >> 1) * H2 * W2] = lerp2(ad.l0, (ad.i0 & 1) ? v : e, ad.l1, (ad.i1 & 1) ? v : e);
    }
  }
}

constexpr int OB8 = 32;
// ... 167 lines not shown
#pragma unroll
    for (int j = 0; j < 8; ++j) {
      float l = u >= 2 ? gl[j] : 0.f;
#pragma unroll
      for (int m = 0; m < 4; ++m) l = u == m - 2 ? bl[m][j] : l;
      pre[j] += l;
    }
    store(d, pre);
  }
}

__global__ void split_weights_kernel(const float* __restrict__ w, float* __restrict__ wl,
                                     float* __restrict__ wr, int cout, int C) {
  const long long nl = 9LL * cout * C * 9, nr = 6LL * cout * C * 9;
  for (long long i = blockIdx.x * (long long)blockDim.x + threadIdx.x; i < nl + nr;
       i += (long long)gridDim.x * blockDim.x) {
    const bool left = i < nl;
    long long r = left ? i : i - nl;
    const int kw = (int)(r % 3);
    r /= 3;
    const int kh = (int)(r % 3);
    r /= 3;
    const int c = (int)(r % C);
    r /= C;
    const int o = (int)(r % cout);
    const int m = (int)(r / cout);
    auto W = [&](int ci, int kd, int khh, int kww) {
      return w[((((long long)o * 2 * C + ci) * 3 + kd) * 3 + khh) * 3 + kww];
    };
    if (left) {
      const int kd = m / 3, t = m % 3;
      wl[i] = kw >= t ? W(c, kd, kh, kw) : 0.f;
    } else if (m < 3) {
      wr[i - nl] = W(C + c, m, kh, kw);
    } else {
      wr[i - nl] = kw == 1 ? W(C + c, m - 3, kh, 2) : 0.f;
    }
  }
}

}
}

using namespace lea;

extern "C" int lea_cv_stem_split_weights(const float* w, float* wl, float* wr, int cout, int C,
                                         void* stream) {
  clear_error();
  LEA_CHECK_ARG(w && wl && wr, "lea_cv_stem_split_weights: null pointer");
  LEA_CHECK_ARG(cout > 0 && C > 0, "lea_cv_stem_split_weights: bad shape cout=%d C=%d", cout, C);
  const long long total = 15LL * cout * C * 9;
  const int grid = (int)std::min<long long>((total + 255) / 256, 4096);
  cvs::split_weights_kernel<<<grid, 256, 0, as_stream(stream)>>>(w, wl, wr, cout, C);
  return launch_status("lea_cv_stem_split_weights");
}

extern "C" int lea_cv_stem_combine(const void* lmaps, int64_t l_bstride, const void* rmaps,
                                   int64_t r_bstride, const float* scale, const float* shift,
                                   void* y, int64_t y_bstride, int B, int cout, int D3, int H, int W,
                                   unsigned flags, int dtype, void* stream) {
  clear_error();
  LEA_CHECK_ARG(lmaps && rmaps && y, "lea_cv_stem_combine: null pointer");
  LEA_CHECK_ARG((scale == nullptr) == (shift == nullptr),
                "lea_cv_stem_combine: scale/shift must both be set or both NULL");
  LEA_CHECK_ARG(B > 0 && cout > 0 && D3 >= 2 && H > 0 && W > 0,
                "lea_cv_stem_combine: bad shape B=%d cout=%d D3=%d H=%d W=%d", B, cout, D3, H, W);
  LEA_CHECK_ARG(dtype == LEA_F32 || dtype == LEA_BF16, "lea_cv_stem_combine: dtype %d", dtype);
  LEA_CHECK_ARG(dtype != LEA_F32 || W % 4 == 0, "lea_cv_stem_combine: f32 needs W %% 4 == 0 (W=%d)", W);
  LEA_CHECK_ARG(dtype != LEA_BF16 || cout % 8 == 0, "lea_cv_stem_combine: bf16 needs cout %% 8 == 0");
  LEA_CHECK_ARG((long long)cout * D3 * H * W < (1LL << 40), "lea_cv_stem_combine: volume too large");
  cvs::Args a{};
  a.lk = lmaps;
  a.lbs = l_bstride;
  a.rk = rmaps;
  a.rbs = r_bstride;
  a.scale = scale;
  a.shift = shift;
  a.y = y;
  a.ybs = y_bstride;
  a.cout = cout;
  a.D = D3;
  a.H = H;
  a.W = W;
  LEA_CHECK_FLAGS(flags, LEA_RELU | 0x300u, "lea_cv_stem_combine");
  a.flags = flags & (LEA_RELU | 0x300u);
  a.nseg = (W + cvs::WS - 1) / cvs::WS;
  const int ob = dtype == LEA_F32 ? cvs::OB : cvs::OB8;
  a.dchunk = std::min(D3, (cvs::kLdsBytes / (int)sizeof(float) / ob - (3 * cvs::WS - 1)) / 2);
  a.nds = (D3 + a.dchunk - 1) / a.dchunk;
  a.ncob = (cout + ob - 1) / ob;
  const long long nblk = (long long)B * a.ncob * H * a.nds * a.nseg;
  LEA_CHECK_ARG(nblk < (1LL << 31), "lea_cv_stem_combine: grid too large");
  const size_t lds = (size_t)ob * (2 * a.dchunk + 3 * cvs::WS - 1) * sizeof(float);
  if (dtype == LEA_F32)
    cvs::cv_stem_f32_kernel<<<dim3((unsigned)nblk), cvs::kThreads, lds, as_stream(stream)>>>(a);
  else
    cvs::cv_stem_c8_kernel<<<dim3((unsigned)nblk), cvs::kThreads, lds, as_stream(stream)>>>(a);
  return launch_status("lea_cv_stem_combine");
}

static bool cv_stem_down2_ok(int cout, int D3, int H, int W, int dtype) {
  if (dtype != LEA_F32 || cout <= 0 || D3 < 2 || H < 2 || W < 4 || D3 % 2 || H % 2 || W % 4) return false;
  return (size_t)2 * cvs::OB * (2 * D3 + 3 * cvs::WS - 1) * sizeof(float) <= (size_t)cvs::kLdsBytes;
}

extern "C" int lea_cv_stem_down2_supported(int cout, int D3, int H, int W, int dtype) {
  return cv_stem_down2_ok(cout, D3, H, W, dtype) ? 1 : 0;
}

extern "C" int lea_cv_stem_combine_down2(const void* lmaps, int64_t l_bstride, const void* rmaps,
                                         int64_t r_bstride, const float* scale, const float* shift,
                                         void* y, int64_t y_bstride, void* y2, int64_t y2_bstride, int B,
                                         int cout, int D3, int H, int W, unsigned flags, int dtype,
                                         void* stream) {
  clear_error();
  LEA_CHECK_ARG(lmaps && rmaps && y && y2, "lea_cv_stem_combine_down2: null pointer");
  LEA_CHECK_ARG((scale == nullptr) == (shift == nullptr),
                "lea_cv_stem_combine_down2: scale/shift must both be set or both NULL");
  LEA_CHECK_ARG(B > 0 && cout > 0 && D3 >= 2 && H > 0 && W > 0,
                "lea_cv_stem_combine_down2: bad shape B=%d cout=%d D3=%d H=%d W=%d", B, cout, D3, H, W);
  LEA_CHECK_FLAGS(flags, LEA_RELU, "lea_cv_stem_combine_down2");
  if (!cv_stem_down2_ok(cout, D3, H, W, dtype)) {
    set_error("lea_cv_stem_combine_down2: needs f32, even D3 and H, W %% 4 == 0 and unsplit planes "
              "(D3=%d H=%d W=%d dtype=%d)", D3, H, W, dtype);
    return LEA_E_UNSUPPORTED;
  }
  LEA_CHECK_ARG((long long)cout * D3 * H * W < (1LL << 40), "lea_cv_stem_combine_down2: volume too large");
  LEA_CHECK_ARG((uintptr_t)y % 16 == 0 && y_bstride % 4 == 0 && (uintptr_t)y2 % 8 == 0 && y2_bstride % 2 == 0,
                "lea_cv_stem_combine_down2: y needs 16-byte, y2 8-byte alignment");
  const size_t ybytes = (size_t)((long long)(B - 1) * y_bstride + (long long)cout * D3 * H * W) * sizeof(float);
  const size_t y2bytes =
      (size_t)((long long)(B - 1) * y2_bstride + (long long)cout * (D3 / 2) * (H / 2) * (W / 2)) * sizeof(float);
  LEA_CHECK_ARG(!spans_overlap(y, ybytes, y2, y2bytes), "lea_cv_stem_combine_down2: y and y2 overlap");
  cvs::Args a{};
  a.lk = lmaps;
  a.lbs = l_bstride;
  a.rk = rmaps;
  a.rbs = r_bstride;
  a.scale = scale;
  a.shift = shift;
  a.y = y;
  a.ybs = y_bstride;
  a.y2 = static_cast<float*>(y2);
  a.y2bs = y2_bstride;
  a.cout = cout;
  a.D = D3;
  a.H = H;
  a.W = W;
  a.flags = flags & LEA_RELU;
  a.rd = axis_ratio(D3, D3 / 2, 1);
  a.rh = axis_ratio(H, H / 2, 1);
  a.rw = axis_ratio(W, W / 2, 1);
  a.nseg = (W + cvs::WS - 1) / cvs::WS;
  a.dchunk = D3;
  a.nds = 1;
  a.ncob = (cout + cvs::OBD - 1) / cvs::OBD;
  const long long nblk = (long long)B * a.ncob * (H / 2) * a.nseg;
  LEA_CHECK_ARG(nblk < (1LL << 31), "lea_cv_stem_combine_down2: grid too large");
  const size_t lds = (size_t)2 * cvs::OBD * (2 * D3 + 3 * cvs::WS - 1) * sizeof(float);
  cvs::cv_stem_f32_down2_kernel<<<dim3((unsigned)nblk), cvs::kThreads, lds, as_stream(stream)>>>(a);
  return launch_status("lea_cv_stem_combine_down2");
}
```

### leastereo_amd/executor.py

```python
from __future__ import annotations

import os
from dataclasses import dataclass

import torch

from . import kernels
from .arch import scale_dimension


def _stacked(fl: torch.Tensor, fr: torch.Tensor) -> torch.Tensor:
    if (fl.is_contiguous() and fr.is_contiguous() and fl.shape == fr.shape and fl.dtype == fr.dtype
            and fl.device == fr.device
            and fl.untyped_storage().data_ptr() == fr.untyped_storage().data_ptr()
            and fr.data_ptr() == fl.data_ptr() + fl.numel() * fl.element_size()):
        return fl.as_strided((2 * fl.shape[0],) + tuple(fl.shape[1:]), fl.stride())
    return torch.cat((fl, fr), 0)


@dataclass
class ConvParams:
    packed: torch.Tensor
    scale: torch.Tensor | None
    shift: torch.Tensor | None
    cin: int
    cout: int
    k: int
    relu: bool
    kind: str = "3d"
    wino: torch.Tensor | None = None


WINOGRAD = os.environ.get("LEASTEREO_WINOGRAD", "1") != "0"
CV_STEM = os.environ.get("LEASTEREO_CV_STEM", "1") != "0"


def _conv_params(mod, w=None, folded=None):
    w = mod.conv.weight if w is None else w
    scale, shift = mod.folded_bn() if folded is None else folded
    cout, cin, k = w.shape[0], w.shape[1], w.shape[-1]
    if w.dim() == 5:
        return ConvParams(kernels.pack_conv_weight(w), scale, shift, cin, cout, k, mod.relu)
    if k == 1:
        return ConvParams(kernels.pack_conv_weight(w.reshape(cout, cin, 1, 1, 1)), scale, shift,
                          cin, cout, 1, mod.relu)
    if mod.stride == 3:
        return ConvParams(w.detach().contiguous(), scale, shift, cin, cout, 3, mod.relu, "s3")
    if mod.stride != 1 or mod.padding != 1:
        raise ValueError(f"unsupported Conv2d stride={mod.stride} padding={mod.padding}")
    return ConvParams(kernels.pack_conv2d_weight(w), scale, shift, cin, cout, 3, mod.relu, "2d")


class CellGraphExecutor:

    tap = None

    def _emit(self, name, t):
        if self.tap is not None:
            self.tap(name, self._as_f32(t))

    @staticmethod
    def _as_f32(t):
        return t.detach().clone()

    SHARE_DOWNSAMPLE = os.environ.get("LEASTEREO_SHARE_DOWNSAMPLE", "1") != "0"
    SPLIT_S1_GROUP48 = False
    PAIR_S0 = False
    PAIR_STEPS = False
    PAIR_C = tuple(int(c) for c in os.environ.get("LEASTEREO_PAIR_C", "8,16,32").split(",") if c)

    def __init__(self, net):
        from .model import ConvBR
        self.m = net
        self.p = {}
        with torch.no_grad():
            for name, mod in net.named_modules():
                if isinstance(mod, ConvBR):
                    self.p[name] = _conv_params(mod)
            self.s1_group = {}
            self.s1_split = set()
            for i, cell in enumerate(net.cells):
                group = []
                for k, terms in enumerate(cell.plan):
                    for op, j in terms:
                        if j == 1 and cell.op_kinds[op] == "conv":
                            group.append((k, op))
                            break
                first_cat_state = 2 + cell.steps - cell.block_multiplier
                steps = [k for k, _ in group]
                if (len(group) < 2 or steps != list(range(steps[0], steps[0] + len(steps)))
                        or 2 + steps[0] < first_cat_state):
                    continue
                mods = [cell._ops[op] for _, op in group]
                split = (self.SPLIT_S1_GROUP48 and WINOGRAD and len(mods) == 3 and cell.c_out == 16
                         and mods[0].conv.weight.dim() == 5 and mods[0].conv.weight.shape[2] == 3)
                for key, part in ((("s1_group_head", mods[:1]), ("s1_group", mods[1:])) if split
                                  else (("s1_group", mods),)):
                    w = torch.cat([m.conv.weight for m in part], 0)
                    folded = [m.folded_bn() for m in part]
                    scale = torch.cat([f[0] for f in folded]).contiguous()
                    shift = torch.cat([f[1] for f in folded]).contiguous()
                    self.p[f"cells.{i}.{key}"] = _conv_params(part[0], w, (scale, shift))
                self.s1_group[i] = group
                if split:
                    self.s1_split.add(i)
            self.s0_pair = {}
            for i, cell in enumerate(net.cells) if self.PAIR_S0 else ():
                pair = [(k, op) for k, terms in enumerate(cell.plan) for op, j in terms
                        if j == 0 and cell.op_kinds[op] == "conv"]
                first_cat_state = 2 + cell.steps - cell.block_multiplier
                if (len(pair) != 2 or getattr(cell, "dims", 3) != 2 or 2 + pair[0][0] < first_cat_state
                        or cell.c_out % 8 or 2 * cell.c_out > 32):
                    continue
                (k0, op0), (k1, op1) = pair
                m0, m1 = cell._ops[op0], cell._ops[op1]
                other = [(o, j) for o, j in cell.plan[k1] if o != op1]
                if {k for k, _ in self.s1_group.get(i, [])} & {k0, k1}:
                    continue
                if (m0.relu != m1.relu or m0.conv.weight.dim() != 4 or m0.conv.weight.shape[-1] != 3
                        or m0.stride != 1 or m1.stride != 1 or cell.plan[k1][0][0] != op1
                        or not other or cell.op_kinds[other[0][0]] != "conv"):
                    continue
                w = torch.cat([m0.conv.weight, m1.conv.weight], 0)
                folded = [m0.folded_bn(), m1.folded_bn()]
                self.p[f"cells.{i}.s0_pair"] = _conv_params(
                    m0, w, (torch.cat([f[0] for f in folded]).contiguous(),
                            torch.cat([f[1] for f in folded]).contiguous()))
                self.s0_pair[i] = pair
            self.pair_steps = {}
            for i, cell in enumerate(net.cells) if self.PAIR_STEPS else ():
                terms = [[(op, j) for op, j in t] for t in cell.plan]
                if (getattr(cell, "dims", 3) != 3 or not terms or cell.c_out not in self.PAIR_C
                        or any(len(t) != 2 or any(cell.op_kinds[op] != "conv" for op, _ in t) for t in terms)):
                    continue
                mods = [[cell._ops[op] for op, _ in t] for t in terms]
                if any(m.conv.weight.shape[-1] != 3 or not m.relu for ms in mods for m in ms):
                    continue
                for k, (ma, mb) in enumerate(mods):
                    folded = [ma.folded_bn(), mb.folded_bn()]
                    self.p[f"cells.{i}.pair{k}"] = self._pair_params(
                        ma, torch.cat([ma.conv.weight, mb.conv.weight], 1),
                        (torch.cat([f[0] for f in folded]).contiguous(),
                         torch.cat([f[1] for f in folded]).contiguous()))
                self.pair_steps[i] = terms
            cells = list(net.cells)
            for i, (cell, nxt) in enumerate(zip(cells, cells[1:])):
                if (self.SHARE_DOWNSAMPLE and cell.downup_sample != 0 and nxt.downup_sample == 0
                        and nxt.c_out == cell.c_out and 2 + cell.steps - cell.block_multiplier == 1
                        and cell.preprocess.conv.weight.shape[1] == nxt.pre_preprocess.conv.weight.shape[1]
                        and cell.preprocess.conv.weight.shape[1] != nxt.c_out):
                    mods = [nxt.pre_preprocess, cell.preprocess]
                    folded = [m.folded_bn() for m in mods]
                    self.p[f"cells.{i}.share"] = _conv_params(
                        mods[0], torch.cat([m.conv.weight for m in mods], 0),
                        (torch.cat([f[0] for f in folded]).contiguous(),
                         torch.cat([f[1] for f in folded]).contiguous()))

    def conv(self, name, x, out=None, accumulate=False, x2=None, size=None, residual=None, down=None,
             down_only=False):
        p = self.p[name]
        cin = x.shape[1] + (x2.shape[1] if x2 is not None else 0)
        if cin != p.cin:
            raise ValueError(f"{name}: expected {p.cin} input channels, got {cin}")
        resized = size is not None and tuple(size) != tuple(x.shape[2:5])
        if p.kind == "s3":
            return kernels.conv2d_s3_bnrelu(x, p.packed, p.scale, p.shift, p.relu)
        if p.kind == "2d":
            if resized or x2 is not None:
                raise ValueError(f"{name}: 2D 3x3 conv takes one input at its own size")
            return kernels.conv2d_bnrelu(x, p.packed, p.cout, p.scale, p.shift, p.relu, out,
                                         accumulate, residual)
        if resized:
            if x2 is not None or residual is not None:
                raise ValueError("resampled conv takes one input and no residual")
            up = all(int(o) >= int(i) for o, i in zip(size, x.shape[2:]))
            if p.k == 1 and up and not accumulate:
                z = kernels.conv3d_bnrelu(x, p.packed, p.cout, 1, None, None, relu=False)
                if down is not None:
                    return kernels.resample_trilinear_down2(z, size, out, down, p.scale, p.shift, p.relu)[0]
                return kernels.resample_trilinear(z, size, True, out, p.scale, p.shift, p.relu)
            if down is not None:
                raise ValueError(f"{name}: no down-sampling form of this resampled conv")
            return kernels.conv3d_bnrelu_resampled(x, size, p.packed, p.cout, p.k, p.scale,
                                                   p.shift, p.relu, out, accumulate)
        if p.wino is not None and kernels.wino_preferred(x.shape[0], p.cout, p.cin, *x.shape[2:5]):
            if down is not None:
                if x2 is not None:
                    raise ValueError(f"{name}: the down-sampling epilogue takes one input")
                kernels.conv3d_bnrelu_wino_dp_down2(x, p.wino, p.cout, p.scale, p.shift, p.relu, out, down,
                                                    accumulate, residual, only=down_only)
                return out
            return kernels.conv3d_bnrelu_wino(x, p.wino, p.cout, p.scale, p.shift, p.relu, out,
                                              accumulate, x2, residual)
        if down is not None:
            raise ValueError(f"{name}: no down-sampling epilogue on this conv's engine")
        return kernels.conv3d_bnrelu(x, p.packed, p.cout, p.k, p.scale, p.shift, p.relu, out,
                                     accumulate, x2, residual)

    def _pair_params(self, mod, w, folded):
        p = _conv_params(mod, w, folded)
        p.cout = w.shape[0]
        return p

    def _pair_ok(self, x, x2, out):
        return kernels.pair_sum_supported(x, x2, out)

    def pair_conv(self, name, x, x2, out):
        p = self.p[name]
        return kernels.conv3d_bnrelu_wino(x, p.wino, p.cout, p.scale, p.shift, True, out, x2=x2, pair_sum=True)

    def _use_winograd(self):
        if not WINOGRAD:
            return
        with torch.no_grad():
            for name, p in self.p.items():
                if p.kind != "3d" or not kernels.wino_eligible(p.cout, p.cin, p.k):
                    continue
                if ".pair" in name:
                    i, k = int(name.split(".")[1]), int(name.rsplit("pair", 1)[1])
                    cell = self.m.cells[i]
                    w = torch.cat([cell._ops[op].conv.weight for op, _ in self.pair_steps[i][k]], 1)
                elif name.endswith("s1_group") or name.endswith("s1_group_head"):
                    i = int(name.split(".")[1])
                    mods = [self.m.cells[i]._ops[op] for _, op in self.s1_group[i]]
                    if i in self.s1_split:
                        mods = mods[:1] if name.endswith("_head") else mods[1:]
                    w = torch.cat([m.conv.weight for m in mods], 0)
                else:
                    w = self.m.get_submodule(name).conv.weight
                p.wino = kernels.pack_conv_weight_wino(w)

    def _empty(self, b, c, size, like):
        return torch.empty((b, c) + tuple(size), device=like.device, dtype=like.dtype)

    @staticmethod
    def _channels(t, c0, c1):
        return t[:, c0:c1]

    @staticmethod
    def _nchannels(t):
        return t.shape[1]

    @staticmethod
    def _volume(t):
        return tuple(t.shape[2:5])

    @staticmethod
    def _resample(x, size):
        return kernels.resample_trilinear(x, size)

    def _cell_output_takes_down(self, i, size):
        return False

    def cell(self, i, s0, s1, down=None):
        cell = self.m.cells[i]
        c = cell.c_out
        if down is not None and down[0] is not None:
            s0 = down[0]
        s1_down = down is not None and down[1] is not None
        if s1_down:
            s1 = down[1]
        prev_input = s1
        size = self._volume(s1)
        if cell.downup_sample != 0 and not s1_down:
            sc = 0.5 if cell.downup_sample < 0 else 2
            size = tuple(n if (cell.dims == 2 and ax == 0) else scale_dimension(n, sc)
                         for ax, n in enumerate(size))
        b = s1.shape[0]
        bm = cell.block_multiplier
        n_states = 2 + cell.steps
        memo, self._share_memo = getattr(self, "_share_memo", None), None
        share = f"cells.{i}.share" in self.p
        if share:
            big = self._empty(b, c + bm * c, size, s1)
            out = self._channels(big, c, c + bm * c)
        else:
            out = self._empty(b, bm * c, size, s1)
        slot = {idx: self._channels(out, k * c, (k + 1) * c)
                for k, idx in enumerate(range(n_states - bm, n_states))}
        dn = None
        if self._cell_output_takes_down(i, size) and self._down_kernels_take(s1, c, self._volume(s1), size):
            dn = self._empty(b, bm * c, tuple(n // 2 for n in size), s1)
        self._cell_down = dn
        dslot = {} if dn is None else {idx: self._channels(dn, k * c, (k + 1) * c) for k, idx in enumerate(slot)}
        group = self.s1_group.get(i, [])
        if memo is not None and memo[0] is s0 and memo[1] == size:
            s0 = memo[2]
            if 0 in slot:
                slot[0].copy_(s0)
        elif self._nchannels(s0) != c:
            s0 = self.conv(f"cells.{i}.pre_preprocess", s0, out=slot.get(0), size=size)
        else:
            if self._volume(s0) != size:
                s0 = self._resample(s0, size)
            if 0 in slot:
                slot[0].copy_(s0)
        if share:
            self.conv(f"cells.{i}.share", s1, out=self._channels(big, 0, 2 * c), size=size)
            self._share_memo = (prev_input, size, self._channels(big, 0, c))
            s1 = self._channels(big, c, 2 * c)
        else:
            s1 = self.conv(f"cells.{i}.preprocess", s1, out=slot.get(1), size=size,
                           **({} if dn is None else {"down": dslot[1]}))
        states = [s0, s1]
        pairs = self.pair_steps.get(i)
        if pairs is not None:
            dsts = [slot.get(2 + k) for k in range(len(pairs))]
            if all(d is not None for d in dsts) and all(
                    self._pair_ok(states[t[0][1]] if t[0][1] < 2 else dsts[t[0][1] - 2],
                                  states[t[1][1]] if t[1][1] < 2 else dsts[t[1][1] - 2], dsts[k])
                    for k, t in enumerate(pairs)):
                for k, ((_, ja), (_, jb)) in enumerate(pairs):
                    self.pair_conv(f"cells.{i}.pair{k}", states[ja], states[jb], dsts[k])
                    states.append(dsts[k])
                return prev_input, out
        written = set()
        done = set(group)
        consumed = set()
        pair = self.s0_pair.get(i)
        if pair is not None and self._nchannels(s0) == c and self._volume(s0) == size:
            (k0, op0), (k1, op1) = pair
            skips0 = [states[j] for o, j in cell.plan[k0] if cell.op_kinds[o] != "conv"]
            p = self.p[f"cells.{i}.s0_pair"]
            kernels.conv2d_bnrelu_pair(s0, p.packed, c, 2 * c, p.scale, p.shift, p.relu,
                                       slot[2 + k0], slot[2 + k1], skips0[-1] if skips0 else None)
            done |= {(k0, op0), (k1, op1)}
            written |= {k0, k1}
            if skips0:
                consumed.add(k0)
        if group:
            k0 = 2 + group[0][0] - (n_states - bm)
            if i in self.s1_split:
                self.conv(f"cells.{i}.s1_group", s1, out=self._channels(out, (k0 + 1) * c, (k0 + 3) * c))
                self.conv(f"cells.{i}.s1_group_head", s1, out=self._channels(out, k0 * c, (k0 + 1) * c))
            else:
                self.conv(f"cells.{i}.s1_group", s1, out=self._channels(out, k0 * c, (k0 + len(group)) * c))
            written |= {k for k, _ in group}
        for step, terms in enumerate(cell.plan):
            dst = slot.get(len(states))
            if dst is None:
                dst = self._empty(b, c, size, s1)
            skips = [states[j] for k, j in terms if cell.op_kinds[k] != "conv"]
            if step in consumed:
                skips.pop()
            todo = [k for k, _ in terms if (step, k) not in done and cell.op_kinds[k] == "conv"]
            for k, j in terms:
                if (step, k) in done or cell.op_kinds[k] != "conv":
                    continue
                residual = None
                if step not in written and skips:
                    residual = skips.pop()
                kw = {}
                if dn is not None and k == todo[-1]:
                    kw = {"down": dslot[len(states)], "down_only": len(states) == n_states - 1}
                self.conv(f"cells.{i}._ops.{k}", states[j], out=dst, accumulate=step in written,
                          residual=residual, **kw)
                written.add(step)
            for t in skips:
                if step in written:
                    dst.add_(t)
                else:
                    dst.copy_(t)
                written.add(step)
            states.append(dst)
        return prev_input, out


class MatchingExecutor(CellGraphExecutor):
    SPLIT_S1_GROUP48 = os.environ.get("LEASTEREO_SPLIT_GROUP48", "1") != "0"
    PAIR_STEPS = WINOGRAD and os.environ.get("LEASTEREO_PAIR_STEPS", "0") != "0"
    FUSED_DOWN = os.environ.get("LEASTEREO_FUSED_DOWN", "1") != "0"
    FUSED_DOWN_CELLS = os.environ.get("LEASTEREO_FUSED_DOWN_CELLS", "1") != "0"

    def run(self, x):
        return self._from_stem0(self.conv("stem0", x))

    def run_features(self, fl, fr, maxdisp):
        p = self.p["stem0"]
        if fl.shape[1] * 2 != p.cin:
            raise ValueError(f"stem0 expects {p.cin} cost-volume channels, got 2*{fl.shape[1]}")
        d3 = int(maxdisp / 3)
        if self.cv is not None and kernels.cv_stem_supported(p.cout, d3, fl.shape[3], False):
            return self._from_stem0(*self._cv_stem(fl.unsqueeze(2), fr.unsqueeze(2), d3))
        if p.wino is not None and kernels.wino_preferred(fl.shape[0], p.cout, p.cin, int(maxdisp / 3),
                                                         *fl.shape[2:4]):
            stem0 = kernels.conv3d_bnrelu_costvolume_wino(fl, fr, maxdisp, p.wino, p.cout, p.scale,
                                                          p.shift, p.relu)
        else:
            stem0 = kernels.conv3d_bnrelu_costvolume(fl, fr, maxdisp, p.packed, p.cout, p.scale,
                                                     p.shift, p.relu)
        return self._from_stem0(stem0)

    def _cv_stem(self, fl5, fr5, d3):
        p, (wl, wr) = self.p["stem0"], self.cv
        lm = kernels.conv2d_bnrelu(fl5, wl, 9 * p.cout, None, None, relu=False)
        rm = kernels.conv2d_bnrelu(fr5, wr, 6 * p.cout, None, None, relu=False)
        if self._cell0_takes_down((d3,) + tuple(lm.shape[3:5])) and kernels.cv_stem_down2_supported(lm, p.cout, d3):
            return kernels.cv_stem_combine_down2(lm, rm, p.cout, d3, p.scale, p.shift, p.relu)
        return kernels.cv_stem_combine(lm, rm, p.cout, d3, p.scale, p.shift, p.relu), None

    def _cell0_takes_down(self, vol):
        cells = self.m.cells
        return (self.FUSED_DOWN and self.tap is None and not isinstance(self, _C8Layout) and len(cells) > 0
                and cells[0].downup_sample < 0 and cells[0].dims == 3
                and all(n % 2 == 0 and scale_dimension(n, 0.5) == n // 2 for n in vol))

    def _conv1_takes_down(self, vol):
        cells = self.m.cells
        return (self.FUSED_DOWN_CELLS and self.tap is None and not isinstance(self, _C8Layout)
                and len(cells) == 12 and "cells.5.share" in self.p
                and cells[5].downup_sample < 0 and cells[5].dims == 3
                and all(n % 2 == 0 and scale_dimension(n, 0.5) == n // 2 for n in vol))

    def _cell_output_takes_down(self, i, size):
        cells = self.m.cells
        n = len(cells)
        if not (self.FUSED_DOWN_CELLS and self.tap is None and not isinstance(self, _C8Layout)
                and 0 <= i and i + 2 == n and not (n == 12 and i in (1, 4, 8))):
            return False
        cell, nxt = cells[i], cells[i + 1]
        pre = self.p.get(f"cells.{i}.preprocess")
        return (cell.dims == 3 and nxt.dims == 3
                and nxt.downup_sample < 0 and f"cells.{i + 1}.share" not in self.p
                and cell.downup_sample > 0 and f"cells.{i}.share" not in self.p
                and pre is not None and pre.k == 1
                and 2 + cell.steps - cell.block_multiplier == 1
                and self.pair_steps.get(i) is None and self.s0_pair.get(i) is None
                and all(cell.op_kinds[op] == "conv" for terms in cell.plan for op, _ in terms)
                and all(self._finishing_op(i, step) is not None for step in range(len(cell.plan)))
                and all(m % 2 == 0 and scale_dimension(m, 0.5) == m // 2 for m in size) and size[2] % 4 == 0)

    def _finishing_op(self, i, step):
        group = self.s1_group.get(i, [])
        rest = [op for op, _ in self.m.cells[i].plan[step] if (step, op) not in group]
        if not rest or self.p[f"cells.{i}._ops.{rest[-1]}"].wino is None:
            return None
        return rest[-1]

    def _down_kernels_take(self, like, c, in_size, size):
        b = like.shape[0]
        return (like.is_cuda and like.dtype == torch.float32
                and kernels.wino_preferred(b, c, c, *size)
                and kernels.wino_dp_down2_kernel_name(b, c, c, *size) is not None
                and kernels.resample_down2_shape_supported(in_size, size))

    def _cv_stem_pack(self, wl, wr):
        return kernels.pack_conv2d_weight(wl), kernels.pack_conv2d_weight(wr)

    def _from_stem0(self, stem0, stem0_down=None):
        out = self._matching_body(stem0, stem0_down)
        if self.tap is not None:
            self.tap("matching", out.detach().clone())
        return out

    def _matching_body(self, stem0, stem0_down=None):
        d, h, w = self._volume(stem0)
        self._emit("stem0", stem0)
        stem1 = stem1_down = None
        p1 = self.p["stem1"]
        if ("cells.0.share" in self.p and self._cell0_takes_down((d, h, w)) and p1.wino is not None
                and kernels.wino_preferred(stem0.shape[0], p1.cout, p1.cin, d, h, w)
                and kernels.conv3d_wino_down2_supported(stem0, p1.cout)):
            stem1_down = kernels.conv3d_bnrelu_wino_down2(stem0, p1.wino, p1.cout, p1.scale, p1.shift, p1.relu)
        else:
            stem1 = self.conv("stem1", stem0)
            self._emit("stem1", stem1)
        outs = []
        prev = (stem0, stem1)
        cell_down = None
        n = len(self.m.cells)
        for i in range(n):
            down = (stem0_down, stem1_down) if i == 0 else None
            if cell_down is not None:
                down = (None, cell_down)
            if i == 5 and n == 12:
                pc, xa, xb = self.p["conv1"], outs[1][1], outs[4][1]
                if (self._conv1_takes_down(self._volume(xa)) and pc.wino is not None
                        and kernels.wino_preferred(xa.shape[0], pc.cout, pc.cin, *xa.shape[2:5])
                        and kernels.conv3d_wino_down2_cat_supported(xa, xb, pc.cout)):
                    down = (None, kernels.conv3d_bnrelu_wino_down2_cat(xa, xb, pc.wino, pc.cout, pc.scale,
                                                                       pc.shift, pc.relu))
                    prev = (outs[4][0], None)
                else:
                    fused = self.conv("conv1", xa, x2=xb)
                    self._emit("conv1", fused)
                    prev = (outs[4][0], fused)
            elif i == 9 and n == 12:
                fused = self.conv("conv2", outs[4][1], x2=outs[8][1])
                self._emit("conv2", fused)
                prev = (outs[8][0], fused)
            o = self.cell(i, prev[0], prev[1], down=down)
            cell_down, self._cell_down = self._cell_down, None
            self._emit(f"cell{i}", o[1])
            outs.append(o)
            prev = o
        last = outs[-1][1]
        lh = self._volume(last)[1]
        full, half, quarter = (d, h, w), (d // 2, h // 2, w // 2), (d // 4, h // 4, w // 4)
        if lh == h:
            return self._last3_same_size(last)
        if lh == h // 2:
            y = self.conv("last_6", last)
        elif lh == h // 4:
            y = self.conv("last_6", self.conv("last_12", last), size=half)
        elif lh == h // 8:
            y = self.conv("last_12", self.conv("last_24", last), size=quarter)
            y = self.conv("last_6", y, size=half)
        else:
            raise ValueError(f"matching-net output size {tuple(last.shape[2:])} has no head")
        p3 = self.p["last_3"]
        q = self.conv("last_3.taps", y)
        return self._tapsum(q, p3, full)

    @staticmethod
    def _tapsum(q, p3, full):
        return kernels.tapsum_upsample(q, p3.cout, full, p3.scale, p3.shift, p3.relu)

    def _last3_same_size(self, last):
        return self.conv("last_3", last)

    def __init__(self, matching):
        super().__init__(matching)
        with torch.no_grad():
            last3 = matching.last_3.conv.weight
            co, ci = last3.shape[:2]
            taps = last3.permute(0, 2, 3, 4, 1).reshape(co * 27, ci, 1, 1, 1)
            self.p["last_3.taps"] = ConvParams(kernels.pack_conv_weight(taps), None, None,
                                               ci, co * 27, 1, False)
            self.cv = None
            if CV_STEM:
                self.cv = self._cv_stem_pack(*kernels.cv_stem_split_weights(matching.stem0.conv.weight))
        self._use_winograd()


class MatchingExecutorDirect(MatchingExecutor):

    SPLIT_S1_GROUP48 = False
    PAIR_STEPS = False

    def __init__(self, matching):
        super().__init__(matching)
        self.cv = None

    def _use_winograd(self):
        """Direct engine only."""


class FeatureExecutor(CellGraphExecutor):
    FUSED_STEM = os.environ.get("LEASTEREO_FEATURE_STEM", "1") != "0"
    PAIR_S0 = os.environ.get("LEASTEREO_PAIR_S0", "1") != "0"

    def _stems(self, x, c8=False, x2=None):
        p0, p1 = self.p["stem0"], self.p["stem1"]
        if (self.FUSED_STEM and p0.relu and p1.relu and (p0.cin, p0.cout, p1.cout) == (3, 16, 32)
                and p1.kind == "s3"):
            return kernels.feature_stem(x, self.m.stem0.conv.weight, p0.scale, p0.shift, p1.packed,
                                        p1.scale, p1.shift, c8, x2)
        if x2 is not None:
            x = torch.cat((x, x2), 0)
        stem1 = self.conv("stem1", self.conv("stem0", x.unsqueeze(2)))
        return kernels.to_c8(stem1) if c8 else stem1

    def run(self, x, x2=None):
        stem1 = self._stems(x, x2=x2)
        stem2 = self.conv("stem2", stem1)
        out = (stem1, stem2)
        for i in range(len(self.m.cells)):
            out = self.cell(i, out[0], out[1])
        last = out[-1]
        h, w = stem2.shape[3:]
        lh = last.shape[3]
        full, half, quarter = (1, h, w), (1, h // 2, w // 2), (1, h // 4, w // 4)
        if lh == h:
            y = last
        elif lh == h // 2:
            y = kernels.resample_trilinear(self.conv("last_6", last), full)
        elif lh == h // 4:
            y = self.conv("last_6", self.conv("last_12", last), size=half)
            y = kernels.resample_trilinear(y, full)
        elif lh == h // 8:
            y = self.conv("last_12", self.conv("last_24", last), size=quarter)
            y = kernels.resample_trilinear(self.conv("last_6", y, size=half), full)
        else:
            raise ValueError(f"feature size {tuple(x.shape[2:])} is not legal for the feature net")
        return self.conv("last_3", y).squeeze(2)


class _C8Layout:

    FUSED_RS = os.environ.get("LEASTEREO_BF16_FUSED_RS", "1") != "0"
    SHARE_DOWNSAMPLE = FUSED_RS and CellGraphExecutor.SHARE_DOWNSAMPLE

    def _empty(self, b, c, size, like):
        return torch.empty((b, c // 8) + tuple(size) + (8,), device=like.device, dtype=torch.bfloat16)

    @staticmethod
    def _as_f32(t):
        return kernels.from_c8(t)

    @staticmethod
    def _channels(t, c0, c1):
        return t[:, c0 // 8:c1 // 8]

    @staticmethod
    def _nchannels(t):
        return t.shape[1] * 8

    @staticmethod
    def _resample(x, size):
        return kernels.resample_trilinear_bf16(x, size)

    @staticmethod
    def _share_weight(net, name):
        i = int(name.split(".")[1])
        return torch.cat([net.cells[i + 1].pre_preprocess.conv.weight, net.cells[i].preprocess.conv.weight], 0)

    def _downsampled(self, x, size):
        memo = getattr(self, "_rs_memo", None)
        if memo is not None and memo[0] is x and memo[1] == tuple(size):
            return memo[2]
        y = kernels.resample_trilinear_bf16(x, size)
        self._rs_memo = (x, tuple(size), y)
        return y

    def _fresh(self):
        self._rs_memo = None

    def _conv_c8(self, name, x, out=None, accumulate=False, x2=None, size=None, residual=None):
        p = self.p[name]
        cin = (x.shape[1] + (x2.shape[1] if x2 is not None else 0)) * 8
        if cin != p.cin:
            raise ValueError(f"{name}: expected {p.cin} input channels, got {cin}")
        if size is not None and tuple(size) != tuple(x.shape[2:5]):
            if x2 is not None or residual is not None or accumulate:
                raise ValueError("resampled conv takes one input and no residual")
            up = all(int(o) >= int(i) for o, i in zip(size, x.shape[2:5]))
            if p.k == 1 and up:
                z = kernels.conv3d_bnrelu_bf16(x, p.packed, p.cout, 1, None, None, relu=False)
                return kernels.resample_trilinear_bf16(z, size, True, out, p.scale, p.shift, p.relu)
            if (self.FUSED_RS and p.k == 1 and p.kind == "bf16" and p.cin % 32 == 0 and p.cin <= 128
                    and p.cout in (16, 32, 64)):
                return kernels.conv1x1_resampled_bf16(x, size, p.packed, p.cout, p.scale, p.shift,
                                                      p.relu, out)
            x = self._downsampled(x, size)
        if p.kind == "bf16_2d":
            if x2 is not None:
                raise ValueError(f"{name}: 2D conv takes one input")
            return kernels.conv2d_bnrelu_bf16(x, p.packed, p.cout, p.scale, p.shift, p.relu, out,
                                              accumulate, residual)
        return kernels.conv3d_bnrelu_bf16(x, p.packed, p.cout, p.k, p.scale, p.shift, p.relu, out,
                                          accumulate, x2, residual)


class MatchingExecutorBF16(_C8Layout, MatchingExecutor):

    SPLIT_S1_GROUP48 = False
    PAIR_STEPS = os.environ.get("LEASTEREO_PAIR_STEPS", "1") != "0"

    def __init__(self, matching):
        from .model import ConvBR
        super().__init__(matching)
        with torch.no_grad():
            for name, p in list(self.p.items()):
                if name == "last_3":
                    continue
                if name == "last_3.taps":
                    w = matching.last_3.conv.weight
                    co, ci = w.shape[:2]
                    taps = w.permute(0, 2, 3, 4, 1).reshape(co * 27, ci, 1, 1, 1)
                    pad = (-taps.shape[0]) % 8
                    taps = torch.cat([taps, taps.new_zeros((pad,) + tuple(taps.shape[1:]))], 0)
                    self.p[name] = ConvParams(kernels.pack_conv_weight_bf16(taps), None, None, ci,
                                              taps.shape[0], 1, False, "bf16")
                    continue
                if ".pair" in name:
                    i, k = int(name.split(".")[1]), int(name.rsplit("pair", 1)[1])
                    wa, wb = (matching.cells[i]._ops[op].conv.weight for op, _ in self.pair_steps[i][k])
                    packed = torch.cat([kernels.pack_conv_weight_bf16(wa), kernels.pack_conv_weight_bf16(wb)])
                    self.p[name] = ConvParams(packed, p.scale, p.shift, p.cin, p.cout, p.k, p.relu, "bf16")
                    continue
                if name.endswith(".s1_group"):
                    i = int(name.split(".")[1])
                    mods = [matching.cells[i]._ops[op] for _, op in self.s1_group[i]]
                    w = torch.cat([m.conv.weight for m in mods], 0)
                elif name.endswith(".share"):
                    w = self._share_weight(matching, name)
                else:
                    mod = matching.get_submodule(name)
                    assert isinstance(mod, ConvBR)
                    w = mod.conv.weight
                self.p[name] = ConvParams(kernels.pack_conv_weight_bf16(w), p.scale, p.shift, p.cin,
                                          p.cout, p.k, p.relu, "bf16")

    def _use_winograd(self):
        """bf16 layers stay on the bf16 engine."""

    def _pair_ok(self, x, x2, out):
        return kernels.pair_sum_supported_bf16(x, x2, out)

    def pair_conv(self, name, x, x2, out):
        p = self.p[name]
        return kernels.conv3d_bnrelu_bf16(x, p.packed, p.cout, 3, p.scale, p.shift, True, out, x2=x2,
                                          pair_sum=True)

    def _cv_stem_pack(self, wl, wr):
        return kernels.pack_conv2d_weight_bf16(wl), kernels.pack_conv2d_weight_bf16(wr)

    def _cv_stem(self, fl8, fr8, d3):
        p, (wl, wr) = self.p["stem0"], self.cv
        lm = kernels.conv2d_bnrelu_bf16(fl8, wl, 9 * p.cout, None, None, relu=False)
        rm = kernels.conv2d_bnrelu_bf16(fr8, wr, 6 * p.cout, None, None, relu=False)
        return kernels.cv_stem_combine(lm, rm, p.cout, d3, p.scale, p.shift, p.relu,
                                       name="cv_stem_c8_kernel")

    @staticmethod
    def _tapsum(q, p3, full):
        return kernels.tapsum_upsample_bf16(q, p3.cout, full, p3.scale, p3.shift, p3.relu)

    def _last3_same_size(self, last):
        return self._tapsum(self.conv("last_3.taps", last), self.p["last_3"], self._volume(last))

    def conv(self, *args, **kw):
        return self._conv_c8(*args, **kw)

    def run(self, x):
        self._fresh()
        try:
            return self._from_stem0(self.conv("stem0", kernels.to_c8(x)))
        finally:
            self._fresh()

    def run_features(self, fl, fr, maxdisp):
        self._fresh()
        try:
            return self._run_features(fl, fr, maxdisp)
        finally:
            self._fresh()

    def _run_features(self, fl, fr, maxdisp):
# ... 76 lines not shown
```

### leastereo_amd/kernels.py

```python
from __future__ import annotations

import collections
import contextlib
import math
import os

import numpy as np
import torch

from . import _lib
from ._lib import LEA_BF16, LEA_F32, LEA_PAIR_SUM, LEA_RELU, LEA_RESIDUAL, check


def _stream():
    return torch.cuda.current_stream().cuda_stream


ProbeRecord = collections.namedtuple("ProbeRecord", "name flops bytes start end mfma_flops shape")


class KernelProbe:

    def __init__(self, names=None):
        self.names = None if names is None else set(names)
        self.records = []

    def __enter__(self):
        global _probe
        _probe = self
        return self

    def __exit__(self, *exc):
        global _probe
        _probe = None

    def _totals(self, key, name=None):
        torch.cuda.synchronize()
        out = {}
        for r in self.records:
            if name is not None and r.name != name:
                continue
            d = out.setdefault(key(r), {"launches": 0, "flops": 0.0, "bytes": 0.0, "ms": 0.0, "mfma_flops": 0.0})
            d["launches"] += 1
            d["flops"] += r.flops
            d["bytes"] += r.bytes
            d["ms"] += r.start.elapsed_time(r.end)
            d["mfma_flops"] += r.mfma_flops
        return out

    def summary(self):
        return self._totals(lambda r: r.name)

    def by_shape(self, name):
        return self._totals(lambda r: r.shape, name)


_probe = None


def _conv_record(b, cin, cout, d, h, w, k, accumulate, in_vox, resampled, name=None, mfma_scale=1.0,
                 esz=4, nbytes=None):
    if name is None:
        name = conv_kernel_name(b, cout, d, h, w, k, resampled)
    if _probe.names is not None and name not in _probe.names:
        return None
    vox = b * d * h * w
    flops = 2.0 * vox * cout * cin * k ** 3
    if nbytes is None:
        nbytes = esz * (in_vox * cin + vox * cout * (2 if accumulate else 1)) + 4.0 * cout * cin * k ** 3
    return ProbeRecord(name, flops, nbytes, None, None, flops * mfma_scale, (b, cin, cout, d, h, w, k))


def _op_record(name, flops, nbytes, mfma=None, shape=None):
    if _probe.names is not None and name not in _probe.names:
        return None
    return ProbeRecord(name, float(flops), float(nbytes), None, None, float(flops if mfma is None else mfma), shape)


@contextlib.contextmanager
def _timed(record):
    probe = _probe
    rec = None if probe is None or record is None else record()
    if rec is None:
        yield
        return
    e0, e1 = torch.cuda.Event(enable_timing=True), torch.cuda.Event(enable_timing=True)
    e0.record()
    yield
    e1.record()
    probe.records.append(rec._replace(start=e0, end=e1))


def _call(entry, *args):
    return getattr(_lib.load(), entry)(*args, _stream())
# ... 128 lines not shown
    if t is None:
        t = torch.empty(shape, device=device, dtype=torch.bfloat16 if c8 else torch.float32)
    if tuple(t.shape) != shape:
        raise ValueError(f"{name} shape {tuple(t.shape)} != {shape}")
    return t, _batch_stride(t, name, c8)


def _conv_out(b, cout, spatial, out, accumulate, device, c8=False):
    if out is None and accumulate:
        raise ValueError("accumulate needs out")
    return _out_view(out, _act_shape(b, cout, spatial, c8), device, c8)


def _residual(out, accumulate, residual, ybs, c8=False, shape=None):
    if accumulate:
        if residual is not None:
            raise ValueError("accumulate and residual are exclusive")
        return out.data_ptr(), ybs
    if residual is None:
        return None, 0
    (_require_c8 if c8 else _require_cuda)(residual)
    shape = tuple(out.shape) if shape is None else shape
    if tuple(residual.shape) != shape:
        raise ValueError(f"residual shape {tuple(residual.shape)} != {shape}")
    return residual.data_ptr(), _batch_stride(residual, "residual", c8)


def _second_source(x2, b, spatial, c8=False):
    if x2 is None:
        return None, 0, 0
    if x2.shape[0] != b or tuple(x2.shape[2:5]) != spatial:
        raise ValueError("x2 must match x in batch and volume")
    return x2.data_ptr(), _batch_stride(x2, "x2", c8), x2.shape[1] * (8 if c8 else 1)


def conv_kernel_name(b, cout, d, h, w, k, resampled=False):
    return _decode(_lib.load().lea_conv3d_kernel_name(b, cout, d, h, w, k, 1 if resampled else 0))


def build_cost_volume(fl: torch.Tensor, fr: torch.Tensor, maxdisp: int) -> torch.Tensor:
    _require_cuda(fl, fr)
    fl, fr = fl.contiguous(), fr.contiguous()
    if fl.shape != fr.shape or fl.dim() != 4:
        raise ValueError("left/right features must both be [B, C, H, W]")
    b, c, h, w = fl.shape
    d3 = int(maxdisp / 3)
    cost = torch.empty((b, 2 * c, d3, h, w), device=fl.device, dtype=fl.dtype)
    _launch("lea_build_cost_volume", fl.data_ptr(), fr.data_ptr(), cost.data_ptr(), b, c, h, w, d3, LEA_F32)
    return cost


def packed_floats(cout: int, cin: int, k: int) -> int:
    n = _lib.load().lea_conv3d_packed_floats(cout, cin, k)
    if n == 0:
        raise ValueError(f"unsupported conv shape cout={cout} cin={cin} k={k}")
    return n


def pack_conv_weight(w: torch.Tensor) -> torch.Tensor:
    _require_cuda(w)
    w = w.detach().contiguous()
    cout, cin, k = w.shape[0], w.shape[1], w.shape[-1]
    packed = torch.empty(packed_floats(cout, cin, k), device=w.device, dtype=torch.float32)
    _launch("lea_conv3d_pack_weights", w.data_ptr(), packed.data_ptr(), cout, cin, k)
    return packed


def conv3d_bnrelu(x: torch.Tensor, packed: torch.Tensor, cout: int, k: int,
                  scale: torch.Tensor | None, shift: torch.Tensor | None, relu: bool = True,
                  out: torch.Tensor | None = None, accumulate: bool = False,
                  x2: torch.Tensor | None = None,
                  residual: torch.Tensor | None = None) -> torch.Tensor:
    _require_cuda(x, x2, packed, scale, shift, out)
    b, cin, d, h, w = x.shape
    xbs = _check_volume_view(x, "x")
    x2ptr, x2bs, cin2 = _second_source(x2, b, (d, h, w))
    out, ybs = _conv_out(b, cout, (d, h, w), out, accumulate, x.device)
    rptr, rbs = _residual(out, accumulate, residual, ybs)
    _launch("lea_conv3d_bnrelu", x.data_ptr(), xbs, x2ptr, x2bs, cin2, packed.data_ptr(), _ptr(scale),
            _ptr(shift), rptr, rbs, out.data_ptr(), ybs, b, cin + cin2, cout, d, h, w, k,
            _flags(relu, rptr is not None), LEA_F32,
            probe=lambda: _conv_record(b, cin + cin2, cout, d, h, w, k, rptr is not None, b * d * h * w, False))
    return out


def costvolume_kernel_name(b, cout, d3, h, w):
    return _decode(_lib.load().lea_conv3d_costvolume_kernel_name(b, cout, d3, h, w))


def conv3d_bnrelu_costvolume(fl: torch.Tensor, fr: torch.Tensor, maxdisp: int, packed: torch.Tensor,
                             cout: int, scale: torch.Tensor | None, shift: torch.Tensor | None,
                             relu: bool = True) -> torch.Tensor:
    _require_cuda(fl, fr, packed, scale, shift)
    b, c, h, w = _feature_pair(fl, fr)
    d3 = int(maxdisp / 3)
    out = torch.empty((b, cout, d3, h, w), device=fl.device, dtype=fl.dtype)
    _launch("lea_conv3d_bnrelu_costvolume", fl.data_ptr(), fr.data_ptr(), fl.stride(0), packed.data_ptr(),
            _ptr(scale), _ptr(shift), out.data_ptr(), out.stride(0), b, c, cout, d3, h, w, _flags(relu), LEA_F32,
            probe=lambda: _conv_record(b, 2 * c, cout, d3, h, w, 3, False, 0, False,
                                       name=costvolume_kernel_name(b, cout, d3, h, w)))
    return out


def conv3d_bnrelu_resampled(x: torch.Tensor, size, packed: torch.Tensor, cout: int, k: int,
                            scale: torch.Tensor | None, shift: torch.Tensor | None,
                            relu: bool = True, out: torch.Tensor | None = None,
                            accumulate: bool = False) -> torch.Tensor:
    _require_cuda(x, packed, scale, shift, out)
    b, cin, di, hi, wi = x.shape
    d, h, w = (int(s) for s in size)
    xbs = _check_volume_view(x, "x")
    out, ybs = _conv_out(b, cout, (d, h, w), out, accumulate, x.device)
    rptr, rbs = _residual(out, accumulate, None, ybs)
    _launch("lea_conv3d_bnrelu_resampled", x.data_ptr(), xbs, di, hi, wi, packed.data_ptr(), _ptr(scale),
            _ptr(shift), rptr, rbs, out.data_ptr(), ybs, b, cin, cout, d, h, w, k, _flags(relu, accumulate),
            LEA_F32,
            probe=lambda: _conv_record(b, cin, cout, d, h, w, k, accumulate, b * di * hi * wi, True))
    return out



def conv2d_kernel_name(b, cout, h, w, cin=None):
    lib = _lib.load()
    return _decode(lib.lea_conv2d_kernel_name(b, cout, h, w) if cin is None
                   else lib.lea_conv2d_kernel_name_cin(b, cin, cout, h, w))


def _conv2d_weight(w):
    _require_cuda(w)
    w = w.detach().contiguous()
    if w.dim() != 4 or tuple(w.shape[2:]) != (3, 3):
        raise ValueError(f"expected a [cout, cin, 3, 3] weight, got {tuple(w.shape)}")
    return w, w.shape[0], w.shape[1]


def pack_conv2d_weight(w: torch.Tensor) -> torch.Tensor:
    w, cout, cin = _conv2d_weight(w)
    n = _lib.load().lea_conv2d_packed_floats(cout, cin)
    packed = torch.empty(n, device=w.device, dtype=torch.float32)
    _launch("lea_conv2d_pack_weights", w.data_ptr(), packed.data_ptr(), cout, cin)
    return packed


def conv2d_bnrelu(x: torch.Tensor, packed: torch.Tensor, cout: int,
                  scale: torch.Tensor | None, shift: torch.Tensor | None, relu: bool = True,
                  out: torch.Tensor | None = None, accumulate: bool = False,
                  residual: torch.Tensor | None = None) -> torch.Tensor:
    _require_cuda(x, packed, scale, shift, out)
    b, cin, d, h, w = x.shape
    if d != 1:
        raise ValueError("conv2d_bnrelu takes [B, C, 1, H, W] views")
    xbs = _check_volume_view(x, "x")
    out, ybs = _conv_out(b, cout, (1, h, w), out, accumulate, x.device)
    rptr, rbs = _residual(out, accumulate, residual, ybs)
    _launch("lea_conv2d_bnrelu", x.data_ptr(), xbs, packed.data_ptr(), _ptr(scale), _ptr(shift), rptr, rbs,
            out.data_ptr(), ybs, b, cin, cout, h, w, _flags(relu, rptr is not None), LEA_F32,
            probe=lambda: _op_record(
                conv2d_kernel_name(b, cout, h, w, cin), 2.0 * b * h * w * cout * cin * 9,
                4.0 * b * h * w * (cin + cout * (2 if rptr is not None else 1)) + 36.0 * cout * cin))
    return out


def conv2d_bnrelu_pair(x: torch.Tensor, packed: torch.Tensor, c1: int, cout: int,
                       scale: torch.Tensor | None, shift: torch.Tensor | None, relu: bool,
                       out1: torch.Tensor, out2: torch.Tensor,
                       residual: torch.Tensor | None = None) -> None:
    _require_cuda(x, packed, scale, shift, out1, out2, residual)
    b, cin, d, h, w = x.shape
    if d != 1:
        raise ValueError("conv2d_bnrelu_pair takes [B, C, 1, H, W] views")
    xbs = _check_volume_view(x, "x")
    if tuple(out1.shape) != (b, c1, 1, h, w) or tuple(out2.shape) != (b, cout - c1, 1, h, w):
        raise ValueError(f"conv2d_bnrelu_pair: outputs {tuple(out1.shape)} / {tuple(out2.shape)}")
    y1bs, y2bs = _check_volume_view(out1, "out1"), _check_volume_view(out2, "out2")
    rbs = 0
    if residual is not None:
        if tuple(residual.shape) != tuple(out1.shape):
            raise ValueError(f"conv2d_bnrelu_pair: residual {tuple(residual.shape)}")
        rbs = _check_volume_view(residual, "residual")
    _launch("lea_conv2d_bnrelu_pair", x.data_ptr(), xbs, packed.data_ptr(), _ptr(scale), _ptr(shift),
            _ptr(residual), rbs, out1.data_ptr(), y1bs, out2.data_ptr(), y2bs, b, cin, cout, c1, h, w,
            _flags(relu, residual is not None),
            probe=lambda: _op_record(
                conv2d_kernel_name(b, cout, h, w, cin), 2.0 * b * h * w * cout * cin * 9,
                4.0 * b * h * w * (cin + cout + (c1 if residual is not None else 0)) + 36.0 * cout * cin))


def feature_stem(x: torch.Tensor, w0: torch.Tensor, scale0, shift0, w1: torch.Tensor, scale1, shift1,
                 c8: bool = False, x2: torch.Tensor | None = None) -> torch.Tensor:
    _require_cuda(x, x2, scale0, shift0, scale1, shift1)
    w0, w1 = w0.detach().contiguous(), w1.detach().contiguous()
    _require_cuda(w0, w1)
    x = x.contiguous()
    srcs = [x]
    if x2 is not None:
        if tuple(x2.shape) != tuple(x.shape):
            raise ValueError(f"feature_stem: x2 {tuple(x2.shape)} differs from x {tuple(x.shape)}")
        x2 = x2.contiguous()
        srcs.append(x2)
    b, cin, hi, wi = x.shape
    c0, c1 = w0.shape[0], w1.shape[0]
    if tuple(w0.shape) != (c0, cin, 3, 3) or tuple(w1.shape) != (c1, c0, 3, 3):
        raise ValueError(f"feature_stem: weights {tuple(w0.shape)} / {tuple(w1.shape)} do not chain")
    ho, wo = (hi - 1) // 3 + 1, (wi - 1) // 3 + 1
    nb = b * len(srcs)
    if c8:
        out = torch.empty((nb, c1 // 8, 1, ho, wo, 8), device=x.device, dtype=torch.bfloat16)
    else:
        out = torch.empty((nb, c1, 1, ho, wo), device=x.device, dtype=torch.float32)
    if len(srcs) == 2 and b == 1:
        srcs, b, xbs = [x], 2, (x2.data_ptr() - x.data_ptr()) // x.element_size()
    else:
        xbs = x.stride(0)
    with _timed(lambda: _op_record(
            "feature_stem_kernel", 2.0 * nb * ho * wo * (9 * 9 * cin * c0 + 9 * c0 * c1),
            4.0 * nb * cin * hi * wi + out.numel() * out.element_size(), 0.0)):
        for i, src in enumerate(srcs):
            _launch("lea_feature_stem_bnrelu", src.data_ptr(), xbs, w0.data_ptr(), _ptr(scale0), _ptr(shift0),
                    w1.data_ptr(), _ptr(scale1), _ptr(shift1), out[i * b:].data_ptr(), out.stride(0), b, cin, c0,
                    c1, hi, wi, LEA_BF16 if c8 else LEA_F32)
    return out


def conv2d_s3_bnrelu(x: torch.Tensor, w: torch.Tensor, scale: torch.Tensor | None,
                     shift: torch.Tensor | None, relu: bool = True) -> torch.Tensor:
    _require_cuda(x, w, scale, shift)
    b, cin, d, hi, wi = x.shape
    if d != 1:
        raise ValueError("conv2d_s3_bnrelu takes [B, C, 1, H, W] views")
    w = w.detach().contiguous()
    cout = w.shape[0]
    if tuple(w.shape) != (cout, cin, 3, 3):
        raise ValueError(f"weight {tuple(w.shape)} does not match cin={cin}")
    xbs = _check_volume_view(x, "x")
    out = torch.empty((b, cout, 1, (hi - 1) // 3 + 1, (wi - 1) // 3 + 1), device=x.device,
                      dtype=x.dtype)
    _launch("lea_conv2d_s3_bnrelu", x.data_ptr(), xbs, w.data_ptr(), _ptr(scale), _ptr(shift), out.data_ptr(),
            out.stride(0), b, cin, cout, hi, wi, _flags(relu), LEA_F32,
            probe=lambda: _op_record("conv2d_s3_kernel", 2.0 * out.numel() * cin * 9,
                                     4.0 * (x.numel() + out.numel()), 0.0))
    return out

# ... 664 lines not shown
                                  relu: bool = True) -> torch.Tensor:
    _require_c8(fl, fr)
    if fl.shape != fr.shape or fl.shape[2] != 1:
        raise ValueError("left/right c8 features must match and have D = 1")
    fbs = _check_c8_view(fl, "left")
    if _check_c8_view(fr, "right") != fbs:
        raise ValueError("left/right batch strides differ")
    b, cb, _, h, w, _ = fl.shape
    d3 = int(maxdisp / 3)
    out = torch.empty((b, cout // 8, d3, h, w, 8), device=fl.device, dtype=torch.bfloat16)
    _launch("lea_conv3d_bnrelu_costvolume_bf16", fl.data_ptr(), fr.data_ptr(), fbs, packed.data_ptr(), _ptr(scale),
            _ptr(shift), out.data_ptr(), out.stride(0), b, cb * 8, cout, d3, h, w, _flags(relu),
            probe=lambda: _conv_record(b, 2 * cb * 8, cout, d3, h, w, 3, False, 0, False,
                                       name=conv_kernel_name_bf16(b, cout, 2 * cb * 8, d3, h, w, 3, True), esz=2))
    return out


def resample_trilinear_bf16(x: torch.Tensor, size, align_corners: bool = True,
                            out: torch.Tensor | None = None, scale=None, shift=None,
                            relu: bool = False) -> torch.Tensor:
    _require_c8(x, out)
    b, cb, di, hi, wi, _ = x.shape
    do, ho, wo = (int(s) for s in size)
    xbs = _check_c8_view(x, "x")
    out, ybs = _out_view(out, (b, cb, do, ho, wo, 8), x.device, c8=True)
    _launch("lea_resample3d_trilinear_bf16", x.data_ptr(), xbs, out.data_ptr(), ybs, b, cb * 8, di, hi, wi, do, ho,
            wo, 1 if align_corners else 0, _ptr(scale), _ptr(shift), _flags(relu),
            probe=lambda: _op_record("resample3d_c8", 0.0, 2.0 * b * cb * 8 * (di * hi * wi + do * ho * wo)))
    return out


def tapsum_upsample_bf16(q: torch.Tensor, cout: int, size, scale=None, shift=None,
                         relu: bool = False) -> torch.Tensor:
    _require_c8(q)
    b, cb, di, hi, wi, _ = q.shape
    if cb * 8 < 27 * cout:
        raise ValueError(f"q has {cb * 8} channels, need 27*{cout}")
    return _tapsum(q, _check_c8_view(q, "q"), cout, (di, hi, wi), size, scale, shift, relu, LEA_BF16,
                   lambda out: _op_record("tapsum_c8", 0.0, 2.0 * q.numel() + 4.0 * out.numel()))


def pack_conv2d_weight_bf16(w: torch.Tensor) -> torch.Tensor:
    w, cout, cin = _conv2d_weight(w)
    n = _lib.load().lea_conv2d_packed_elems_bf16(cout, cin)
    if n == 0:
        raise ValueError(f"unsupported bf16 conv2d shape cout={cout} cin={cin}")
    packed = torch.empty(n, device=w.device, dtype=torch.bfloat16)
    _launch("lea_conv2d_pack_weights_bf16", w.data_ptr(), packed.data_ptr(), cout, cin)
    return packed


def conv2d_bnrelu_bf16(x: torch.Tensor, packed: torch.Tensor, cout: int, scale, shift,
                       relu: bool = True, out: torch.Tensor | None = None, accumulate: bool = False,
                       residual: torch.Tensor | None = None) -> torch.Tensor:
    _require_c8(x, out, residual)
    _require_cuda(scale, shift)
    b, cb, d, h, w, _ = x.shape
    if d != 1:
        raise ValueError("conv2d_bnrelu_bf16 takes D = 1 maps")
    xbs = _check_c8_view(x, "x")
    out, ybs = _conv_out(b, cout, (1, h, w), out, accumulate, x.device, c8=True)
    rptr, rbs = _residual(out, accumulate, residual, ybs, c8=True)
    _launch("lea_conv2d_bnrelu_bf16", x.data_ptr(), xbs, packed.data_ptr(), _ptr(scale), _ptr(shift), rptr, rbs,
            out.data_ptr(), ybs, b, cb * 8, cout, h, w, _flags(relu, rptr is not None),
            probe=lambda: _op_record(
                "conv2d_bf16", 2.0 * b * h * w * cout * cb * 8 * 9,
                2.0 * b * h * w * (cb * 8 + cout * (2 if rptr is not None else 1)) + 18.0 * cout * cb * 8))
    return out



def cv_stem_split_weights(w: torch.Tensor):
    _require_cuda(w)
    w = w.detach().contiguous()
    if w.dim() != 5 or tuple(w.shape[2:]) != (3, 3, 3) or w.shape[1] % 2:
        raise ValueError(f"expected a [cout, 2C, 3, 3, 3] weight, got {tuple(w.shape)}")
    cout, c = w.shape[0], w.shape[1] // 2
    wl = torch.empty((9 * cout, c, 3, 3), device=w.device, dtype=torch.float32)
    wr = torch.empty((6 * cout, c, 3, 3), device=w.device, dtype=torch.float32)
    _launch("lea_cv_stem_split_weights", w.data_ptr(), wl.data_ptr(), wr.data_ptr(), cout, c)
    return wl, wr


def cv_stem_supported(cout: int, d3: int, w: int, bf16: bool) -> bool:
    return d3 >= 2 and (cout % 8 == 0 if bf16 else w % 4 == 0)


def _cv_stem_maps(who, lmaps, rmaps, cout, c8=False):
    (_require_c8 if c8 else _require_cuda)(lmaps, rmaps)
    b, h, w = lmaps.shape[0], lmaps.shape[3], lmaps.shape[4]
    lbs, rbs = _batch_stride(lmaps, "lmaps", c8), _batch_stride(rmaps, "rmaps", c8)
    per = 8 if c8 else 1
    if lmaps.shape[1] * per != 9 * cout or rmaps.shape[1] * per != 6 * cout:
        raise ValueError(f"{who}: map channels must be 9 / 6 x cout")
    return b, h, w, lbs, rbs


def cv_stem_combine(lmaps: torch.Tensor, rmaps: torch.Tensor, cout: int, d3: int,
                    scale: torch.Tensor | None, shift: torch.Tensor | None, relu: bool = True,
                    name: str = "cv_stem_f32_kernel") -> torch.Tensor:
    c8 = lmaps.dtype == torch.bfloat16
    b, h, w, lbs, rbs = _cv_stem_maps("cv_stem_combine", lmaps, rmaps, cout, c8)
    out = torch.empty(_act_shape(b, cout, (d3, h, w), c8), device=lmaps.device,
                      dtype=torch.bfloat16 if c8 else torch.float32)
    _require_cuda(scale, shift)
    if tuple(rmaps.shape[0:1]) != (b,) or tuple(rmaps.shape[3:5]) != (h, w):
        raise ValueError("cv_stem_combine: left/right maps differ in batch or size")
    _launch("lea_cv_stem_combine", lmaps.data_ptr(), lbs, rmaps.data_ptr(), rbs, _ptr(scale), _ptr(shift),
            out.data_ptr(), out.stride(0), b, cout, d3, h, w, _flags(relu), LEA_BF16 if c8 else LEA_F32,
            probe=lambda: _op_record(name, 0.0, out.numel() * out.element_size(), 0.0,
                                     shape=(b, 0, cout, d3, h, w, 0)))
    return out


def cv_stem_down2_supported(lmaps: torch.Tensor, cout: int, d3: int) -> bool:
    if not lmaps.is_cuda or lmaps.dtype != torch.float32 or lmaps.dim() != 5:
        return False
    return bool(_lib.load().lea_cv_stem_down2_supported(cout, d3, lmaps.shape[3], lmaps.shape[4], LEA_F32))


def cv_stem_combine_down2(lmaps: torch.Tensor, rmaps: torch.Tensor, cout: int, d3: int,
                          scale: torch.Tensor | None, shift: torch.Tensor | None, relu: bool = True):
    _require_cuda(scale, shift)
    b, h, w, lbs, rbs = _cv_stem_maps("cv_stem_combine_down2", lmaps, rmaps, cout)
    if tuple(rmaps.shape[0:1]) != (b,) or tuple(rmaps.shape[3:5]) != (h, w):
        raise ValueError("cv_stem_combine_down2: left/right maps differ in batch or size")
    out = torch.empty((b, cout, d3, h, w), device=lmaps.device, dtype=torch.float32)
    out2 = torch.empty((b, cout, d3 // 2, h // 2, w // 2), device=lmaps.device, dtype=torch.float32)
    _launch("lea_cv_stem_combine_down2", lmaps.data_ptr(), lbs, rmaps.data_ptr(), rbs, _ptr(scale), _ptr(shift),
            out.data_ptr(), out.stride(0), out2.data_ptr(), out2.stride(0), b, cout, d3, h, w, _flags(relu), LEA_F32,
            probe=lambda: _op_record("cv_stem_f32_down2_kernel", 0.0,
                                     4.0 * (lmaps.numel() + rmaps.numel() + out.numel() + out2.numel())))
    return out, out2



def _require_u8_images(who, left, right):
    for t in (left, right):
        if not t.is_cuda or t.dtype != torch.uint8:
            raise _lib.HipKernelError(f"{who} needs uint8 device images, got {t.dtype} on {t.device}")


def standardize_crop_u8(left: torch.Tensor, right: torch.Tensor, crop_height: int, crop_width: int):
    _require_u8_images("standardize_crop_u8", left, right)
    if left.dim() == 3:
        left, right = left.unsqueeze(0), right.unsqueeze(0)
    if left.shape != right.shape or left.dim() != 4 or left.shape[-1] not in (3, 4):
        raise ValueError(f"left/right must both be [B, H, W, 3|4] uint8, got {tuple(left.shape)} "
                         f"and {tuple(right.shape)}")
    left, right = left.contiguous(), right.contiguous()
    b, h, w, ps = left.shape
    lib = _lib.load()
    ws = torch.empty(lib.lea_standardize_workspace_bytes(b), device=left.device, dtype=torch.uint8)
    out_l = torch.empty((b, 3, crop_height, crop_width), device=left.device, dtype=torch.float32)
    out_r = torch.empty_like(out_l)
    rc = _call("lea_standardize_crop_u8", left.data_ptr(), right.data_ptr(), b, h, w, ps, out_l.data_ptr(),
               out_r.data_ptr(), crop_height, crop_width, ws.data_ptr())
    if rc == _lib.LEA_E_INVALID and b"test_transform" in lib.lea_last_error():
        raise ValueError(lib.lea_last_error().decode())
    check(rc, "lea_standardize_crop_u8")
    return out_l, out_r


def train_transform_u8(left: torch.Tensor, right: torch.Tensor, disp_left: torch.Tensor, disp_right,
                       params: torch.Tensor, crop_height: int, crop_width: int, maxdisp: float):
    _require_u8_images("train_transform_u8", left, right)
    _require_cuda(disp_left, disp_right)
    if not params.is_cuda or params.dtype != torch.int32:
        raise _lib.HipKernelError(f"train_transform_u8 needs int32 device params, got "
                                  f"{params.dtype} on {params.device}")
    if left.shape != right.shape or left.dim() != 4 or left.shape[-1] not in (3, 4):
        raise ValueError(f"left/right must both be [B, H, W, 3|4] uint8, got {tuple(left.shape)} "
                         f"and {tuple(right.shape)}")
    b, h, w, ps = left.shape
    for d in (disp_left, disp_right):
        if d is not None and tuple(d.shape) != (b, h, w):
            raise ValueError(f"disparities must be [B, H, W] = {(b, h, w)}, got {tuple(d.shape)}")
    if tuple(params.shape) != (b, 5):
        raise ValueError(f"params must be [B, 5] = {(b, 5)}, got {tuple(params.shape)}")
    left, right, disp_left, params = left.contiguous(), right.contiguous(), disp_left.contiguous(), params.contiguous()
    disp_right = _contiguous(disp_right)
    dev = left.device
    ws = torch.empty(_lib.load().lea_train_transform_workspace_bytes(b), device=dev, dtype=torch.uint8)
    out_l = torch.empty((b, 3, crop_height, crop_width), device=dev, dtype=torch.float32)
    out_r = torch.empty_like(out_l)
    out_t = torch.empty((b, 1, crop_height, crop_width), device=dev, dtype=torch.float32)
    n_valid = torch.empty((b,), device=dev, dtype=torch.int32)
    _launch("lea_train_transform_u8", left.data_ptr(), right.data_ptr(), b, h, w, ps, disp_left.data_ptr(),
            _ptr(disp_right), params.data_ptr(), out_l.data_ptr(), out_r.data_ptr(), out_t.data_ptr(), crop_height,
            crop_width, float(maxdisp), n_valid.data_ptr(), ws.data_ptr())
    return out_l, out_r, out_t, n_valid



def standardize_tiles_u8(left: torch.Tensor, right: torch.Tensor, origins: torch.Tensor, tile_height: int,
                         tile_width: int):
    _require_u8_images("standardize_tiles_u8", left, right)
    if not origins.is_cuda or origins.dtype != torch.int32:
        raise _lib.HipKernelError(f"standardize_tiles_u8 needs int32 device origins, got "
                                  f"{origins.dtype} on {origins.device}")
    if left.dim() == 4 and left.shape[0] == 1:
        left, right = left[0], right[0]
    if left.shape != right.shape or left.dim() != 3 or left.shape[-1] not in (3, 4):
        raise ValueError(f"left/right must both be [H, W, 3|4] uint8, got {tuple(left.shape)} "
                         f"and {tuple(right.shape)}")
    if origins.dim() != 2 or origins.shape[1] != 2 or origins.shape[0] < 1:
        raise ValueError(f"origins must be [N, 2] with N >= 1, got {tuple(origins.shape)}")
    left, right, origins = left.contiguous(), right.contiguous(), origins.contiguous()
    h, w, ps = left.shape
    n = origins.shape[0]
    ws = torch.empty(_lib.load().lea_standardize_tiles_workspace_bytes(), device=left.device, dtype=torch.uint8)
    out_l = torch.empty((n, 3, tile_height, tile_width), device=left.device, dtype=torch.float32)
    out_r = torch.empty_like(out_l)
# ... 271 lines not shown
```

Measured before the change: 164.2 pairs/s.

## Fuse twin 1x1 conv heads and window cost-volume stem map convolutions

```diff
diff --git a/include/leastereo_hip.h b/include/leastereo_hip.h
--- a/include/leastereo_hip.h
+++ b/include/leastereo_hip.h
@@ -39,6 +39,15 @@
                       void* y, int64_t y_bstride,
                       int B, int cin, int cout, int D, int H, int W, int k,
                       unsigned flags, int dtype, void* stream);
+
+int lea_conv1x1_heads(const void* x, int64_t x_bstride, const void* x2, int64_t x2_bstride,
+                      int cin2, const float* w_packed,
+                      const float* scale_a, const float* shift_a, void* y_a, int64_t ya_bstride,
+                      int cout_a, unsigned flags_a,
+                      const float* scale_b, const float* shift_b, void* y_b, int64_t yb_bstride,
+                      int cout_b, unsigned flags_b,
+                      int B, int cin, int D, int H, int W, int dtype, void* stream);
+const char* lea_conv1x1_heads_kernel_name(int B, int cout, int D, int H, int W);
 
 int lea_conv3d_bnrelu_resampled(const void* x, int64_t x_bstride, int Di, int Hi, int Wi,
                                 const float* w_packed, const float* scale, const float* shift,
@@ -262,6 +271,15 @@
                               void* y2, int64_t y2_bstride, int B, int cout, int D3, int H, int W,
                               unsigned flags, int dtype, void* stream);
 
+#define LEA_CVS_TMAJOR 8u
+int lea_cv_stem_map_windows(int D3, int W, int* left, int* right);
+int lea_conv2d_windowed_tiles(int W, int w1_begin, int w1_end, int w2_begin, int w2_end, int* tiles);
+int lea_conv2d_bnrelu_windowed(const void* x, int64_t x_bstride, const float* w_packed,
+                               const float* scale, const float* shift, void* y, int64_t y_bstride,
+                               int B, int cin, int cout, int split, int H, int W, int w1_begin,
+                               int w1_end, int w2_begin, int w2_end, unsigned flags, int dtype,
+                               void* stream);
+
 
 size_t lea_standardize_workspace_bytes(int B);
 int lea_standardize_crop_u8(const void* left, const void* right, int B, int H, int W,
diff --git a/leastereo_amd/_lib.py b/leastereo_amd/_lib.py
--- a/leastereo_amd/_lib.py
+++ b/leastereo_amd/_lib.py
@@ -14,6 +14,7 @@
 LEA_RELU = 1
 LEA_RESIDUAL = 2
 LEA_PAIR_SUM = 4
+LEA_CVS_TMAJOR = 8
 LEA_E_INVALID = 1001
 
 _p = ctypes.c_void_p
@@ -29,6 +30,9 @@
     "lea_conv3d_pack_weights": (_i, [_p, _p, _i, _i, _i, _p]),
     "lea_conv3d_bnrelu": (_i, [_p, _i64, _p, _i64, _i, _p, _p, _p, _p, _i64, _p, _i64,
                                _i, _i, _i, _i, _i, _i, _i, _u, _i, _p]),
+    "lea_conv1x1_heads": (_i, [_p, _i64, _p, _i64, _i, _p, _p, _p, _p, _i64, _i, _u, _p, _p, _p, _i64, _i, _u,
+                               _i, _i, _i, _i, _i, _i, _p]),
+    "lea_conv1x1_heads_kernel_name": (ctypes.c_char_p, [_i, _i, _i, _i, _i]),
     "lea_conv3d_bnrelu_resampled": (_i, [_p, _i64, _i, _i, _i, _p, _p, _p, _p, _i64, _p, _i64,
                                          _i, _i, _i, _i, _i, _i, _i, _u, _i, _p]),
     "lea_conv3d_kernel_name": (ctypes.c_char_p, [_i, _i, _i, _i, _i, _i, _i]),
@@ -150,6 +154,10 @@
     "lea_cv_stem_split_weights": (_i, [_p, _p, _p, _i, _i, _p]),
     "lea_cv_stem_combine": (_i, [_p, _i64, _p, _i64, _p, _p, _p, _i64, _i, _i, _i, _i, _i, _u, _i,
                                  _p]),
+    "lea_cv_stem_map_windows": (_i, [_i, _i, ctypes.POINTER(_i), ctypes.POINTER(_i)]),
+    "lea_conv2d_windowed_tiles": (_i, [_i, _i, _i, _i, _i, ctypes.POINTER(_i)]),
+    "lea_conv2d_bnrelu_windowed": (_i, [_p, _i64, _p, _p, _p, _p, _i64, _i, _i, _i, _i, _i, _i, _i, _i, _i, _i,
+                                        _u, _i, _p]),
     "lea_cv_stem_down2_supported": (_i, [_i, _i, _i, _i, _i]),
     "lea_cv_stem_combine_down2": (_i, [_p, _i64, _p, _i64, _p, _p, _p, _i64, _p, _i64, _i, _i, _i, _i, _i,
                                        _u, _i, _p]),
diff --git a/leastereo_amd/csrc/conv3d.hip b/leastereo_amd/csrc/conv3d.hip
--- a/leastereo_amd/csrc/conv3d.hip
+++ b/leastereo_amd/csrc/conv3d.hip
@@ -200,8 +200,17 @@
   }
 }
 
-template <int MT, int NT, bool VEC>
-__global__ __launch_bounds__(kConvThreads) void conv1x1_kernel(const ConvArgs a) {
+struct Conv1x1HeadB {
+  float* y;
+  long long ybs;
+  const float* scale;
+  const float* shift;
+  int c0;
+  unsigned flags;
+};
+
+template <int MT, int NT, bool VEC, bool TWO>
+__device__ __forceinline__ void conv1x1_body(const ConvArgs& a, const Conv1x1HeadB& hb) {
   using P = PackCfg<1, MT>;
   constexpr int CIN_B = P::CIN_B;
   constexpr int KS = CIN_B / 4;
@@ -266,16 +275,26 @@
     }
   }
 
-  const bool relu = a.flags & LEA_RELU;
-  const bool resid = a.flags & LEA_RESIDUAL;
+  const bool resid = !TWO && (a.flags & LEA_RESIDUAL);
 #pragma unroll
   for (int m = 0; m < MT; ++m) {
 #pragma unroll
     for (int r = 0; r < 4; ++r) {
-      const int co = co0 + m * 16 + kq * 4 + r;
+      int co = co0 + m * 16 + kq * 4 + r;
       if (co >= a.cout) continue;
-      const float sc = a.scale ? a.scale[co] : 1.f;
-      const float sh = a.shift ? a.shift[co] : 0.f;
+      float* y = a.y + (long long)b * a.ybs;
+      const float* scale = a.scale;
+      const float* shift = a.shift;
+      bool relu = a.flags & LEA_RELU;
+      if (TWO && co >= hb.c0) {
+        y = hb.y + (long long)b * hb.ybs;
+        scale = hb.scale;
+        shift = hb.shift;
+        relu = hb.flags & LEA_RELU;
+        co -= hb.c0;
+      }
+      const float sc = scale ? scale[co] : 1.f;
+      const float sh = shift ? shift[co] : 0.f;
       if (VEC && full) {
         const long long o = (long long)co * V + vox(0);
         vecf val;
@@ -289,7 +308,7 @@
 #pragma unroll
           for (int j = 0; j < NT; ++j) val[j] += rv[j];
         }
-        *reinterpret_cast<vecf*>(a.y + (long long)b * a.ybs + o) = val;
+        *reinterpret_cast<vecf*>(y + o) = val;
         continue;
       }
 #pragma unroll
@@ -300,10 +319,20 @@
         float val = acc[m][j][r] * sc + sh;
         if (relu) val = fmaxf(val, 0.f);
         if (resid) val += a.res[(long long)b * a.rbs + o];
-        a.y[(long long)b * a.ybs + o] = val;
+        y[o] = val;
       }
     }
   }
+}
+
+template <int MT, int NT, bool VEC>
+__global__ __launch_bounds__(kConvThreads) void conv1x1_kernel(const ConvArgs a) {
+  conv1x1_body<MT, NT, VEC, false>(a, Conv1x1HeadB{});
+}
+
+template <int MT, int NT, bool VEC>
+__global__ __launch_bounds__(kConvThreads) void conv1x1_heads_kernel(const ConvArgs a, const Conv1x1HeadB hb) {
+  conv1x1_body<MT, NT, VEC, true>(a, hb);
 }
 
 template <int COUT>
@@ -595,24 +624,31 @@
 int g_1x1_vec = 1;
 
 template <int MT, int NT>
-int launch_1x1(const ConvArgs& a, int B, hipStream_t st) {
+int launch_1x1(const ConvArgs& a, int B, hipStream_t st, const Conv1x1HeadB* hb = nullptr) {
   const long long vox = (long long)a.D * a.H * a.W;
   const long long per = kConvWaves * NT * 16;
   const long long gx = (vox + per - 1) / per;
   LEA_CHECK_ARG(gx < (1LL << 31) && (long long)B * a.ncob <= 65535, "lea_conv3d: grid too large");
   auto al = [](const void* q) { return q == nullptr || ((uintptr_t)q % (NT * 4)) == 0; };
   const bool vec = g_1x1_vec && vox % NT == 0 && al(a.x) && al(a.x2) && al(a.y) && al(a.res) &&
-                   a.xbs % NT == 0 && a.x2bs % NT == 0 && a.ybs % NT == 0 && a.rbs % NT == 0;
-  if (vec) conv1x1_kernel<MT, NT, true><<<dim3((unsigned)gx, B * a.ncob), kConvThreads, 0, st>>>(a);
-  else conv1x1_kernel<MT, NT, false><<<dim3((unsigned)gx, B * a.ncob), kConvThreads, 0, st>>>(a);
+                   a.xbs % NT == 0 && a.x2bs % NT == 0 && a.ybs % NT == 0 && a.rbs % NT == 0 &&
+                   (hb == nullptr || (al(hb->y) && hb->ybs % NT == 0));
+  const dim3 grid((unsigned)gx, B * a.ncob);
+  if (hb != nullptr) {
+    if (vec) conv1x1_heads_kernel<MT, NT, true><<<grid, kConvThreads, 0, st>>>(a, *hb);
+    else conv1x1_heads_kernel<MT, NT, false><<<grid, kConvThreads, 0, st>>>(a, *hb);
+    return launch_status("lea_conv1x1_heads");
+  }
+  if (vec) conv1x1_kernel<MT, NT, true><<<grid, kConvThreads, 0, st>>>(a);
+  else conv1x1_kernel<MT, NT, false><<<grid, kConvThreads, 0, st>>>(a);
   return launch_status("lea_conv3d");
 }
 
-int run_1x1(const Plan& p, const ConvArgs& a, int B, hipStream_t st) {
-  if (p.mt == 1) return p.nt == 4 ? launch_1x1<1, 4>(a, B, st) : launch_1x1<1, 2>(a, B, st);
-  if (p.mt == 2) return p.nt == 4 ? launch_1x1<2, 4>(a, B, st) : launch_1x1<2, 2>(a, B, st);
-  if (p.mt == 3) return p.nt == 4 ? launch_1x1<3, 4>(a, B, st) : launch_1x1<3, 2>(a, B, st);
-  return p.nt == 4 ? launch_1x1<4, 4>(a, B, st) : launch_1x1<4, 2>(a, B, st);
+int run_1x1(const Plan& p, const ConvArgs& a, int B, hipStream_t st, const Conv1x1HeadB* hb = nullptr) {
+  if (p.mt == 1) return p.nt == 4 ? launch_1x1<1, 4>(a, B, st, hb) : launch_1x1<1, 2>(a, B, st, hb);
+  if (p.mt == 2) return p.nt == 4 ? launch_1x1<2, 4>(a, B, st, hb) : launch_1x1<2, 2>(a, B, st, hb);
+  if (p.mt == 3) return p.nt == 4 ? launch_1x1<3, 4>(a, B, st, hb) : launch_1x1<3, 2>(a, B, st, hb);
+  return p.nt == 4 ? launch_1x1<4, 4>(a, B, st, hb) : launch_1x1<4, 2>(a, B, st, hb);
 }
 
 template <int MT>
@@ -834,6 +870,65 @@
   a.W = W;
   a.flags = flags;
   return lea::conv_common(a, B, k, false, dtype, stream);
+}
+
+extern "C" const char* lea_conv1x1_heads_kernel_name(int B, int cout, int D, int H, int W) {
+  if (B <= 0 || cout <= 0 || D <= 0 || H <= 0 || W <= 0) return nullptr;
+  const lea::Plan p = lea::make_plan(B, cout, D, H, W, 1, false);
+  snprintf(lea::g_name, sizeof(lea::g_name), "conv1x1_heads_kernel<%d, %d>", p.mt, p.nt);
+  return lea::g_name;
+}
+
+extern "C" int lea_conv1x1_heads(const void* x, int64_t x_bstride, const void* x2, int64_t x2_bstride,
+                                 int cin2, const float* w_packed, const float* scale_a,
+                                 const float* shift_a, void* y_a, int64_t ya_bstride, int cout_a,
+                                 unsigned flags_a, const float* scale_b, const float* shift_b, void* y_b,
+                                 int64_t yb_bstride, int cout_b, unsigned flags_b, int B, int cin, int D,
+                                 int H, int W, int dtype, void* stream) {
+  using namespace lea;
+  clear_error();
+  LEA_CHECK_FLAGS(flags_a, LEA_RELU, "lea_conv1x1_heads");
+  LEA_CHECK_FLAGS(flags_b, LEA_RELU, "lea_conv1x1_heads");
+  LEA_CHECK_ARG(x && w_packed && y_a && y_b, "lea_conv1x1_heads: null pointer");
+  LEA_CHECK_ARG((scale_a == nullptr) == (shift_a == nullptr) && (scale_b == nullptr) == (shift_b == nullptr),
+                "lea_conv1x1_heads: a head's scale/shift must both be set or both NULL");
+  LEA_CHECK_ARG(B > 0 && cin > 0 && cout_a > 0 && cout_b > 0 && D > 0 && H > 0 && W > 0,
+                "lea_conv1x1_heads: bad shape B=%d cin=%d cout=%d+%d D=%d H=%d W=%d", B, cin, cout_a, cout_b,
+                D, H, W);
+  LEA_CHECK_ARG(cin2 >= 0 && cin2 <= cin && (cin2 == 0 || x2), "lea_conv1x1_heads: bad channel split %d/%d",
+                cin - cin2, cin);
+  const long long vox = (long long)D * H * W;
+  LEA_CHECK_ARG(vox * 4 < (1LL << 32) && (long long)(cout_a + cout_b + 63) * vox < (1LL << 31),
+                "lea_conv1x1_heads: volume too large");
+  LEA_CHECK_ARG(x != y_a && x != y_b && (x2 == nullptr || (x2 != y_a && x2 != y_b)),
+                "lea_conv1x1_heads: input aliases an output");
+  LEA_CHECK_ARG(!spans_overlap(y_a, (size_t)cout_a * vox * 4, y_b, (size_t)cout_b * vox * 4),
+                "lea_conv1x1_heads: the heads' outputs overlap");
+  if (dtype != LEA_F32) {
+    set_error("lea_conv1x1_heads: dtype %d unsupported", dtype);
+    return LEA_E_UNSUPPORTED;
+  }
+  ConvArgs a{};
+  a.x = (const float*)x;
+  a.xbs = x_bstride;
+  a.x2 = (const float*)x2;
+  a.x2bs = x2_bstride;
+  a.cin1 = cin - cin2;
+  a.wp = w_packed;
+  a.scale = scale_a;
+  a.shift = shift_a;
+  a.y = (float*)y_a;
+  a.ybs = ya_bstride;
+  a.cin = cin;
+  a.cout = cout_a + cout_b;
+  a.D = D;
+  a.H = H;
+  a.W = W;
+  a.flags = flags_a;
+  const Conv1x1HeadB hb{(float*)y_b, yb_bstride, scale_b, shift_b, cout_a, flags_b};
+  const Plan p = make_plan(B, a.cout, D, H, W, 1, false);
+  a.ncob = (a.cout + p.mt * 16 - 1) / (p.mt * 16);
+  return run_1x1(p, a, B, as_stream(stream), &hb);
 }
 
 extern "C" size_t lea_conv2d_packed_floats(int cout, int cin) {
@@ -913,6 +1008,98 @@
     case 3: return run_dma2d_mt3(p, a, B, st);
     default: return run_dma2d_mt4(p, a, B, st);
   }
+}
+
+namespace lea {
+
+int run_dma2d(ConvArgs a, int B, hipStream_t st) {
+  const Plan p = make_plan_2d(B, a.cout, a.H, a.W);
+  a.ncob = (a.cout + p.mt * 16 - 1) / (p.mt * 16);
+  switch (p.mt) {
+    case 1: return run_dma2d_mt1(p, a, B, st);
+    case 2: return run_dma2d_mt2(p, a, B, st);
+    case 3: return run_dma2d_mt3(p, a, B, st);
+    default: return run_dma2d_mt4(p, a, B, st);
+  }
+}
+
+constexpr int kWinTile = 16;
+
+}
+
+extern "C" int lea_conv2d_windowed_tiles(int W, int w1_begin, int w1_end, int w2_begin, int w2_end,
+                                         int* tiles) {
+  using namespace lea;
+  clear_error();
+  LEA_CHECK_ARG(tiles && W > 0 && 0 <= w1_begin && w1_begin < w1_end && w1_end <= W,
+                "lea_conv2d_windowed: bad first window [%d, %d) of %d columns", w1_begin, w1_end, W);
+  const bool two = w2_begin < w2_end;
+  LEA_CHECK_ARG(!two || (w1_end <= w2_begin && w2_end <= W),
+                "lea_conv2d_windowed: bad second window [%d, %d) after [%d, %d) of %d columns", w2_begin,
+                w2_end, w1_begin, w1_end, W);
+  const int all = (W + kWinTile - 1) / kWinTile;
+  tiles[0] = w1_begin / kWinTile;
+  tiles[1] = (w1_end + kWinTile - 1) / kWinTile;
+  tiles[2] = two ? w2_begin / kWinTile : all;
+  tiles[3] = two ? (w2_end + kWinTile - 1) / kWinTile : all;
+  if (tiles[2] <= tiles[1]) {
+    tiles[1] = std::max(tiles[1], tiles[3]);
+    tiles[2] = tiles[3] = all;
+  }
+  return LEA_OK;
+}
+
+extern "C" int lea_conv2d_bnrelu_windowed(const void* x, int64_t x_bstride, const float* w_packed,
+                                          const float* scale, const float* shift, void* y,
+                                          int64_t y_bstride, int B, int cin, int cout, int split, int H,
+                                          int W, int w1_begin, int w1_end, int w2_begin, int w2_end,
+                                          unsigned flags, int dtype, void* stream) {
+  using namespace lea;
+  clear_error();
+  LEA_CHECK_FLAGS(flags, LEA_RELU, "lea_conv2d_bnrelu_windowed");
+  LEA_CHECK_ARG(x && w_packed && y && x != y, "lea_conv2d_bnrelu_windowed: null or aliased pointer");
+  LEA_CHECK_ARG((scale == nullptr) == (shift == nullptr),
+                "lea_conv2d_bnrelu_windowed: scale/shift must both be set or both NULL");
+  LEA_CHECK_ARG(B > 0 && cin > 0 && cout > 0 && H > 0 && W > 0 && split >= 0 && split < cout,
+                "lea_conv2d_bnrelu_windowed: bad shape B=%d cin=%d cout=%d split=%d H=%d W=%d", B, cin, cout,
+                split, H, W);
+  LEA_CHECK_ARG((long long)(cout + 63) * H * W < (1LL << 31), "lea_conv2d_bnrelu_windowed: plane too large");
+  int t[4];
+  if (const int rc = lea_conv2d_windowed_tiles(W, w1_begin, w1_end, w2_begin, w2_end, t)) return rc;
+  if (dtype != LEA_F32) {
+    set_error("lea_conv2d_bnrelu_windowed: dtype %d unsupported", dtype);
+    return LEA_E_UNSUPPORTED;
+  }
+  ConvArgs a{};
+  a.x = (const float*)x;
+  a.xbs = x_bstride;
+  a.cin1 = cin;
+  a.cin = cin;
+  a.ybs = y_bstride;
+  a.D = 1;
+  a.H = H;
+  a.W = W;
+  a.flags = flags;
+  hipStream_t st = as_stream(stream);
+  if (split > 0) {
+    a.wp = w_packed;
+    a.scale = scale;
+    a.shift = shift;
+    a.y = (float*)y;
+    a.cout = split;
+    if (const int rc = run_dma2d(a, B, st)) return rc;
+  }
+  a.wp = w_packed + (split > 0 ? packed_floats_2d(split, cin) : 0);
+  a.scale = scale ? scale + split : nullptr;
+  a.shift = shift ? shift + split : nullptr;
+  a.y = (float*)y + (long long)split * H * W;
+  a.cout = cout - split;
+  a.wn1 = t[1] - t[0];
+  a.wt1 = t[0];
+  a.wt2 = t[2];
+  a.wtiles = a.wn1 + (t[3] - t[2]);
+  if (a.wtiles == (W + kWinTile - 1) / kWinTile) a.wtiles = a.wn1 = a.wt1 = a.wt2 = 0;
+  return run_dma2d(a, B, st);
 }
 
 extern "C" const char* lea_conv3d_costvolume_kernel_name(int B, int cout, int D3, int H, int W) {
diff --git a/leastereo_amd/csrc/conv3d_impl.h b/leastereo_amd/csrc/conv3d_impl.h
--- a/leastereo_amd/csrc/conv3d_impl.h
+++ b/leastereo_amd/csrc/conv3d_impl.h
@@ -40,6 +40,7 @@
   int csplit;
   long long uoff;
   int grp;
+  int wtiles, wn1, wt1, wt2;
 };
 
 template <int KS, int MT, int KD = KS>
@@ -287,7 +288,8 @@
   const int tile = (lin / a.ndz) % a.ntiles;
   const int bc = lin / (a.ndz * a.ntiles);
   const int h0 = (tile / a.tiles_w) * C::TH;
-  const int w0 = (tile % a.tiles_w) * TW;
+  const int tc = tile % a.tiles_w;
+  const int w0 = (tc < a.wn1 ? a.wt1 + tc : a.wt2 + tc - a.wn1) * TW;
   const int d0 = dz * DSTEP;
   const int b = bc / a.ncob;
   const int co0 = (bc - b * a.ncob) * C::COP;
@@ -402,7 +404,7 @@
 template <typename K>
 int launch_dma(K kernel, const ConvArgs& a0, int th, int tw, int td, int B, hipStream_t st) {
   ConvArgs a = a0;
-  a.tiles_w = (a.W + tw - 1) / tw;
+  a.tiles_w = a.wtiles > 0 ? a.wtiles : (a.W + tw - 1) / tw;
   a.ntiles = a.tiles_w * ((a.H + th - 1) / th);
   a.ndz = (a.D + td - 1) / td;
   const long long n = (long long)a.ntiles * a.ndz * B * a.ncob;
diff --git a/leastereo_amd/csrc/cv_stem.hip b/leastereo_amd/csrc/cv_stem.hip
--- a/leastereo_amd/csrc/cv_stem.hip
+++ b/leastereo_amd/csrc/cv_stem.hip
@@ -38,6 +38,10 @@
 __device__ __forceinline__ bool bz_valid(int z, int W) { return z >= -1 && z < W; }
 __device__ __forceinline__ bool plane_valid(int d, int kd, int D) {
   return d + kd - 1 >= 0 && d + kd - 1 < D;
+}
+
+__device__ __forceinline__ int lmap_channel(const Args& a, int kd, int t, int o) {
+  return ((a.flags & LEA_CVS_TMAJOR) ? 3 * t + kd : 3 * kd + t) * a.cout + o;
 }
 
 __device__ __forceinline__ float left_sum(const float lk[3][3], int d, int u, int D) {
@@ -164,7 +168,7 @@
     for (int t = 0; t < 3; ++t) {
       float4 v = make_float4(0.f, 0.f, 0.f, 0.f);
       if (t == 0 || band)
-        v = *reinterpret_cast<const float4*>(lk + (long long)((3 * kd + t) * a.cout + o) * HW +
+        v = *reinterpret_cast<const float4*>(lk + (long long)lmap_channel(a, kd, t, o) * HW +
                                              (long long)T.h * W + w);
       lkv[kd][t][0] = v.x;
       lkv[kd][t][1] = v.y;
@@ -276,7 +280,7 @@
       for (int t = 0; t < 3; ++t) {
         float4 v = make_float4(0.f, 0.f, 0.f, 0.f);
         if (t == 0 || band)
-          v = *reinterpret_cast<const float4*>(lk + (long long)((3 * kd + t) * a.cout + o) * HW +
+          v = *reinterpret_cast<const float4*>(lk + (long long)lmap_channel(a, kd, t, o) * HW +
                                                (long long)(2 * hp + r) * W + w);
         lkv[kd][t][0] = v.x;
         lkv[kd][t][1] = v.y;
@@ -610,8 +614,9 @@
   a.D = D3;
   a.H = H;
   a.W = W;
-  LEA_CHECK_FLAGS(flags, LEA_RELU | 0x300u, "lea_cv_stem_combine");
-  a.flags = flags & (LEA_RELU | 0x300u);
+  LEA_CHECK_FLAGS(flags, LEA_RELU | LEA_CVS_TMAJOR | 0x300u, "lea_cv_stem_combine");
+  LEA_CHECK_ARG(!(flags & LEA_CVS_TMAJOR) || dtype == LEA_F32, "lea_cv_stem_combine: LEA_CVS_TMAJOR is f32 only");
+  a.flags = flags & (LEA_RELU | LEA_CVS_TMAJOR | 0x300u);
   a.nseg = (W + cvs::WS - 1) / cvs::WS;
   const int ob = dtype == LEA_F32 ? cvs::OB : cvs::OB8;
   a.dchunk = std::min(D3, (cvs::kLdsBytes / (int)sizeof(float) / ob - (3 * cvs::WS - 1)) / 2);
@@ -627,6 +632,18 @@
   return launch_status("lea_cv_stem_combine");
 }
 
+extern "C" int lea_cv_stem_map_windows(int D3, int W, int* left, int* right) {
+  clear_error();
+  LEA_CHECK_ARG(left && right && D3 >= 2 && W > 0, "lea_cv_stem_map_windows: bad arguments D3=%d W=%d", D3, W);
+  left[0] = 0;
+  left[1] = std::min(W, D3 + 4);
+  right[0] = 0;
+  right[1] = 1;
+  right[2] = std::max(W - D3, 1);
+  right[3] = W;
+  return LEA_OK;
+}
+
 static bool cv_stem_down2_ok(int cout, int D3, int H, int W, int dtype) {
   if (dtype != LEA_F32 || cout <= 0 || D3 < 2 || H < 2 || W < 4 || D3 % 2 || H % 2 || W % 4) return false;
   return (size_t)2 * cvs::OB * (2 * D3 + 3 * cvs::WS - 1) * sizeof(float) <= (size_t)cvs::kLdsBytes;
@@ -647,7 +664,7 @@
                 "lea_cv_stem_combine_down2: scale/shift must both be set or both NULL");
   LEA_CHECK_ARG(B > 0 && cout > 0 && D3 >= 2 && H > 0 && W > 0,
                 "lea_cv_stem_combine_down2: bad shape B=%d cout=%d D3=%d H=%d W=%d", B, cout, D3, H, W);
-  LEA_CHECK_FLAGS(flags, LEA_RELU, "lea_cv_stem_combine_down2");
+  LEA_CHECK_FLAGS(flags, LEA_RELU | LEA_CVS_TMAJOR, "lea_cv_stem_combine_down2");
   if (!cv_stem_down2_ok(cout, D3, H, W, dtype)) {
     set_error("lea_cv_stem_combine_down2: needs f32, even D3 and H, W %% 4 == 0 and unsplit planes "
               "(D3=%d H=%d W=%d dtype=%d)", D3, H, W, dtype);
@@ -675,7 +692,7 @@
   a.D = D3;
   a.H = H;
   a.W = W;
-  a.flags = flags & LEA_RELU;
+  a.flags = flags & (LEA_RELU | LEA_CVS_TMAJOR);
   a.rd = axis_ratio(D3, D3 / 2, 1);
   a.rh = axis_ratio(H, H / 2, 1);
   a.rw = axis_ratio(W, W / 2, 1);
diff --git a/leastereo_amd/executor.py b/leastereo_amd/executor.py
--- a/leastereo_amd/executor.py
+++ b/leastereo_amd/executor.py
@@ -64,6 +64,7 @@
         return t.detach().clone()
 
     SHARE_DOWNSAMPLE = os.environ.get("LEASTEREO_SHARE_DOWNSAMPLE", "1") != "0"
+    FANOUT_1X1 = False
     SPLIT_S1_GROUP48 = False
     PAIR_S0 = False
     PAIR_STEPS = False
@@ -155,6 +156,48 @@
                         mods[0], torch.cat([m.conv.weight for m in mods], 0),
                         (torch.cat([f[0] for f in folded]).contiguous(),
                          torch.cat([f[1] for f in folded]).contiguous()))
+            for i, (cell, nxt) in enumerate(zip(cells, cells[1:])) if self.FANOUT_1X1 else ():
+                wa, wb = cell.preprocess.conv.weight, nxt.pre_preprocess.conv.weight
+                if (f"cells.{i}.share" in self.p or getattr(cell, "dims", 3) != 3
+                        or wa.dim() != 5 or wa.shape[-1] != 1 or wb.shape[-1] != 1 or wa.shape[1] != wb.shape[1]
+                        or cell.downup_sample < 0 or cell.downup_sample + nxt.downup_sample < 0
+                        or wb.shape[1] == nxt.c_out):
+                    continue
+                p = _conv_params(cell.preprocess, torch.cat([wa, wb], 0), (None, None))
+                p.relu = False
+                self.p[f"cells.{i}.fanout"] = p
+
+    def _fanout_takes(self, x):
+        return x.is_cuda and x.dtype == torch.float32
+
+    def _fanout_forms(self, i, src, size):
+        nxt = self.m.cells[i + 1]
+        sc = {0: None, -1: 0.5, 1: 2}[nxt.downup_sample]
+        nsize = tuple(size) if sc is None else tuple(scale_dimension(n, sc) for n in size)
+        ups = []
+        for s in (tuple(size), nsize):
+            if s != tuple(src) and not all(o >= n for o, n in zip(s, src)):
+                return None
+            ups.append(s != tuple(src))
+        return nsize, ups[0], ups[1]
+
+    def _fanout(self, i, x, size, forms, out, dn_out):
+        nsize, up_a, up_b = forms
+        pa, pb = self.p[f"cells.{i}.preprocess"], self.p[f"cells.{i + 1}.pre_preprocess"]
+        b, src = x.shape[0], self._volume(x)
+        za = self._empty(b, pa.cout, src, x) if up_a or out is None else out
+        zb = self._empty(b, pb.cout, src, x)
+        fold = lambda p, up: (None, None, False) if up else (p.scale, p.shift, p.relu)
+        kernels.conv1x1_heads(x, self.p[f"cells.{i}.fanout"].packed, pa.cout, *fold(pa, up_a),
+                              pb.cout, *fold(pb, up_b), out_a=za, out_b=zb)
+        if up_b:
+            zb = kernels.resample_trilinear(zb, nsize, True, None, pb.scale, pb.shift, pb.relu)
+        self._share_memo = (x, nsize, zb)
+        if not up_a:
+            return za
+        if dn_out is not None:
+            return kernels.resample_trilinear_down2(za, size, out, dn_out, pa.scale, pa.shift, pa.relu)[0]
+        return kernels.resample_trilinear(za, size, True, out, pa.scale, pa.shift, pa.relu)
 
     def conv(self, name, x, out=None, accumulate=False, x2=None, size=None, residual=None, down=None,
              down_only=False):
@@ -300,8 +343,15 @@
             self._share_memo = (prev_input, size, self._channels(big, 0, c))
             s1 = self._channels(big, c, 2 * c)
         else:
-            s1 = self.conv(f"cells.{i}.preprocess", s1, out=slot.get(1), size=size,
-                           **({} if dn is None else {"down": dslot[1]}))
+            forms = None
+            if (self.FANOUT_1X1 and f"cells.{i}.fanout" in self.p and not s1_down
+                    and not isinstance(self, _C8Layout) and self._fanout_takes(s1)):
+                forms = self._fanout_forms(i, self._volume(s1), size)
+            if forms is not None and (dn is None or forms[1]):
+                s1 = self._fanout(i, s1, size, forms, slot.get(1), None if dn is None else dslot[1])
+            else:
+                s1 = self.conv(f"cells.{i}.preprocess", s1, out=slot.get(1), size=size,
+                               **({} if dn is None else {"down": dslot[1]}))
         states = [s0, s1]
         pairs = self.pair_steps.get(i)
         if pairs is not None:
@@ -371,6 +421,8 @@
     PAIR_STEPS = WINOGRAD and os.environ.get("LEASTEREO_PAIR_STEPS", "0") != "0"
     FUSED_DOWN = os.environ.get("LEASTEREO_FUSED_DOWN", "1") != "0"
     FUSED_DOWN_CELLS = os.environ.get("LEASTEREO_FUSED_DOWN_CELLS", "1") != "0"
+    WINDOWED_MAPS = os.environ.get("LEASTEREO_WINDOWED_MAPS", "1") != "0"
+    FANOUT_1X1 = os.environ.get("LEASTEREO_FANOUT_1X1", "1") != "0"
 
     def run(self, x):
         return self._from_stem0(self.conv("stem0", x))
@@ -393,11 +445,18 @@
 
     def _cv_stem(self, fl5, fr5, d3):
         p, (wl, wr) = self.p["stem0"], self.cv
-        lm = kernels.conv2d_bnrelu(fl5, wl, 9 * p.cout, None, None, relu=False)
-        rm = kernels.conv2d_bnrelu(fr5, wr, 6 * p.cout, None, None, relu=False)
+        windowed = (self.WINDOWED_MAPS and self.cv_win is not None and fl5.is_cuda
+                    and fl5.dtype == torch.float32)
+        if windowed:
+            lwin, rwin = kernels.cv_stem_map_windows(d3, fl5.shape[4])
+            lm = kernels.conv2d_bnrelu_windowed(fl5, self.cv_win[0], 9 * p.cout, 3 * p.cout, (lwin,))
+            rm = kernels.conv2d_bnrelu_windowed(fr5, self.cv_win[1], 6 * p.cout, 3 * p.cout, rwin)
+        else:
+            lm = kernels.conv2d_bnrelu(fl5, wl, 9 * p.cout, None, None, relu=False)
+            rm = kernels.conv2d_bnrelu(fr5, wr, 6 * p.cout, None, None, relu=False)
         if self._cell0_takes_down((d3,) + tuple(lm.shape[3:5])) and kernels.cv_stem_down2_supported(lm, p.cout, d3):
-            return kernels.cv_stem_combine_down2(lm, rm, p.cout, d3, p.scale, p.shift, p.relu)
-        return kernels.cv_stem_combine(lm, rm, p.cout, d3, p.scale, p.shift, p.relu), None
+            return kernels.cv_stem_combine_down2(lm, rm, p.cout, d3, p.scale, p.shift, p.relu, tmajor=windowed)
+        return kernels.cv_stem_combine(lm, rm, p.cout, d3, p.scale, p.shift, p.relu, tmajor=windowed), None
 
     def _cell0_takes_down(self, vol):
         cells = self.m.cells
@@ -527,9 +586,15 @@
             taps = last3.permute(0, 2, 3, 4, 1).reshape(co * 27, ci, 1, 1, 1)
             self.p["last_3.taps"] = ConvParams(kernels.pack_conv_weight(taps), None, None,
                                                ci, co * 27, 1, False)
-            self.cv = None
+            self.cv = self.cv_win = None
             if CV_STEM:
-                self.cv = self._cv_stem_pack(*kernels.cv_stem_split_weights(matching.stem0.conv.weight))
+                wl, wr = kernels.cv_stem_split_weights(matching.stem0.conv.weight)
+                self.cv = self._cv_stem_pack(wl, wr)
+                if self.WINDOWED_MAPS and not isinstance(self, _C8Layout):
+                    co = wl.shape[0] // 9
+                    wlt = wl.view(3, 3, co, *wl.shape[1:]).transpose(0, 1).reshape(wl.shape)
+                    self.cv_win = (kernels.pack_conv2d_weight_windowed(wlt, 3 * co),
+                                   kernels.pack_conv2d_weight_windowed(wr, 3 * co))
         self._use_winograd()
 
 
@@ -537,10 +602,11 @@
 
     SPLIT_S1_GROUP48 = False
     PAIR_STEPS = False
+    FANOUT_1X1 = False
 
     def __init__(self, matching):
         super().__init__(matching)
-        self.cv = None
+        self.cv = self.cv_win = None
 
     def _use_winograd(self):
         """Direct engine only."""
@@ -655,6 +721,7 @@
 class MatchingExecutorBF16(_C8Layout, MatchingExecutor):
 
     SPLIT_S1_GROUP48 = False
+    FANOUT_1X1 = False
     PAIR_STEPS = os.environ.get("LEASTEREO_PAIR_STEPS", "1") != "0"
 
     def __init__(self, matching):
diff --git a/leastereo_amd/kernels.py b/leastereo_amd/kernels.py
--- a/leastereo_amd/kernels.py
+++ b/leastereo_amd/kernels.py
@@ -2,6 +2,7 @@
 
 import collections
 import contextlib
+import ctypes
 import math
 import os
 
@@ -9,7 +10,7 @@
 import torch
 
 from . import _lib
-from ._lib import LEA_BF16, LEA_F32, LEA_PAIR_SUM, LEA_RELU, LEA_RESIDUAL, check
+from ._lib import LEA_BF16, LEA_CVS_TMAJOR, LEA_F32, LEA_PAIR_SUM, LEA_RELU, LEA_RESIDUAL, check
 
 
 def _stream():
@@ -304,6 +305,28 @@
             _flags(relu, rptr is not None), LEA_F32,
             probe=lambda: _conv_record(b, cin + cin2, cout, d, h, w, k, rptr is not None, b * d * h * w, False))
     return out
+
+
+def conv1x1_heads(x: torch.Tensor, packed: torch.Tensor, cout_a: int, scale_a, shift_a, relu_a: bool,
+                  cout_b: int, scale_b, shift_b, relu_b: bool, out_a: torch.Tensor | None = None,
+                  out_b: torch.Tensor | None = None, x2: torch.Tensor | None = None,
+                  accumulate: bool = False, residual: torch.Tensor | None = None):
+    if accumulate or residual is not None:
+        raise ValueError("conv1x1_heads: neither head accumulates or takes a residual")
+    _require_cuda(x, x2, packed, scale_a, shift_a, scale_b, shift_b, out_a, out_b)
+    b, cin, d, h, w = x.shape
+    xbs = _check_volume_view(x, "x")
+    x2ptr, x2bs, cin2 = _second_source(x2, b, (d, h, w))
+    out_a, abs_ = _out_view(out_a, _act_shape(b, cout_a, (d, h, w)), x.device, name="out_a")
+    out_b, bbs = _out_view(out_b, _act_shape(b, cout_b, (d, h, w)), x.device, name="out_b")
+    cout = cout_a + cout_b
+    _launch("lea_conv1x1_heads", x.data_ptr(), xbs, x2ptr, x2bs, cin2, packed.data_ptr(),
+            _ptr(scale_a), _ptr(shift_a), out_a.data_ptr(), abs_, cout_a, _flags(relu_a),
+            _ptr(scale_b), _ptr(shift_b), out_b.data_ptr(), bbs, cout_b, _flags(relu_b),
+            b, cin + cin2, d, h, w, LEA_F32,
+            probe=lambda: _conv_record(b, cin + cin2, cout, d, h, w, 1, False, b * d * h * w, False,
+                                       name=_decode(_lib.load().lea_conv1x1_heads_kernel_name(b, cout, d, h, w))))
+    return out_a, out_b
 
 
 def costvolume_kernel_name(b, cout, d3, h, w):
@@ -380,6 +403,42 @@
             probe=lambda: _op_record(
                 conv2d_kernel_name(b, cout, h, w, cin), 2.0 * b * h * w * cout * cin * 9,
                 4.0 * b * h * w * (cin + cout * (2 if rptr is not None else 1)) + 36.0 * cout * cin))
+    return out
+
+
+def pack_conv2d_weight_windowed(w: torch.Tensor, split: int) -> torch.Tensor:
+    w, cout, _ = _conv2d_weight(w)
+    if not 0 <= split < cout:
+        raise ValueError(f"split {split} must be in [0, {cout})")
+    return torch.cat([pack_conv2d_weight(part) for part in (w[:split], w[split:]) if part.shape[0]])
+
+
+def conv2d_windowed_tiles(w: int, windows):
+    w1, w2 = (tuple(windows) + ((0, 0),))[:2]
+    t = (ctypes.c_int * 4)()
+    check(_lib.load().lea_conv2d_windowed_tiles(w, w1[0], w1[1], w2[0], w2[1], t), "lea_conv2d_windowed_tiles")
+    return [(t[i], t[i + 1]) for i in (0, 2) if t[i] < t[i + 1]]
+
+
+def conv2d_bnrelu_windowed(x: torch.Tensor, packed: torch.Tensor, cout: int, split: int, windows,
+                           scale: torch.Tensor | None = None, shift: torch.Tensor | None = None,
+                           relu: bool = False, out: torch.Tensor | None = None) -> torch.Tensor:
+    _require_cuda(x, packed, scale, shift, out)
+    b, cin, d, h, w = x.shape
+    if d != 1:
+        raise ValueError("conv2d_bnrelu_windowed takes [B, C, 1, H, W] views")
+    xbs = _check_volume_view(x, "x")
+    out, ybs = _conv_out(b, cout, (1, h, w), out, False, x.device)
+    w1, w2 = (tuple(windows) + ((0, 0),))[:2]
+    cols = sum(16 * (e - s) for s, e in conv2d_windowed_tiles(w, windows))
+
+    def record():
+        px = b * h * (split * w + (cout - split) * min(cols, w))
+        return _op_record(conv2d_kernel_name(b, cout - split, h, w, None) + " windowed", 2.0 * px * cin * 9,
+                          4.0 * (b * h * w * cin + px) + 36.0 * cout * cin, shape=(b, cin, cout, 1, h, w, 3))
+    _launch("lea_conv2d_bnrelu_windowed", x.data_ptr(), xbs, packed.data_ptr(), _ptr(scale), _ptr(shift),
+            out.data_ptr(), ybs, b, cin, cout, split, h, w, w1[0], w1[1], w2[0], w2[1], _flags(relu), LEA_F32,
+            probe=record)
     return out
 
 
@@ -1210,6 +1269,12 @@
     return wl, wr
 
 
+def cv_stem_map_windows(d3: int, w: int):
+    left, right = (ctypes.c_int * 2)(), (ctypes.c_int * 4)()
+    check(_lib.load().lea_cv_stem_map_windows(d3, w, left, right), "lea_cv_stem_map_windows")
+    return (left[0], left[1]), ((right[0], right[1]), (right[2], right[3]))
+
+
 def cv_stem_supported(cout: int, d3: int, w: int, bf16: bool) -> bool:
     return d3 >= 2 and (cout % 8 == 0 if bf16 else w % 4 == 0)
 
@@ -1226,7 +1291,7 @@
 
 def cv_stem_combine(lmaps: torch.Tensor, rmaps: torch.Tensor, cout: int, d3: int,
                     scale: torch.Tensor | None, shift: torch.Tensor | None, relu: bool = True,
-                    name: str = "cv_stem_f32_kernel") -> torch.Tensor:
+                    name: str = "cv_stem_f32_kernel", tmajor: bool = False) -> torch.Tensor:
     c8 = lmaps.dtype == torch.bfloat16
     b, h, w, lbs, rbs = _cv_stem_maps("cv_stem_combine", lmaps, rmaps, cout, c8)
     out = torch.empty(_act_shape(b, cout, (d3, h, w), c8), device=lmaps.device,
@@ -1235,7 +1300,8 @@
     if tuple(rmaps.shape[0:1]) != (b,) or tuple(rmaps.shape[3:5]) != (h, w):
         raise ValueError("cv_stem_combine: left/right maps differ in batch or size")
     _launch("lea_cv_stem_combine", lmaps.data_ptr(), lbs, rmaps.data_ptr(), rbs, _ptr(scale), _ptr(shift),
-            out.data_ptr(), out.stride(0), b, cout, d3, h, w, _flags(relu), LEA_BF16 if c8 else LEA_F32,
+            out.data_ptr(), out.stride(0), b, cout, d3, h, w, _flags(relu) | (LEA_CVS_TMAJOR if tmajor else 0),
+            LEA_BF16 if c8 else LEA_F32,
             probe=lambda: _op_record(name, 0.0, out.numel() * out.element_size(), 0.0,
                                      shape=(b, 0, cout, d3, h, w, 0)))
     return out
@@ -1248,7 +1314,8 @@
 
 
 def cv_stem_combine_down2(lmaps: torch.Tensor, rmaps: torch.Tensor, cout: int, d3: int,
-                          scale: torch.Tensor | None, shift: torch.Tensor | None, relu: bool = True):
+                          scale: torch.Tensor | None, shift: torch.Tensor | None, relu: bool = True,
+                          tmajor: bool = False):
     _require_cuda(scale, shift)
     b, h, w, lbs, rbs = _cv_stem_maps("cv_stem_combine_down2", lmaps, rmaps, cout)
     if tuple(rmaps.shape[0:1]) != (b,) or tuple(rmaps.shape[3:5]) != (h, w):
@@ -1256,7 +1323,8 @@
     out = torch.empty((b, cout, d3, h, w), device=lmaps.device, dtype=torch.float32)
     out2 = torch.empty((b, cout, d3 // 2, h // 2, w // 2), device=lmaps.device, dtype=torch.float32)
     _launch("lea_cv_stem_combine_down2", lmaps.data_ptr(), lbs, rmaps.data_ptr(), rbs, _ptr(scale), _ptr(shift),
-            out.data_ptr(), out.stride(0), out2.data_ptr(), out2.stride(0), b, cout, d3, h, w, _flags(relu), LEA_F32,
+            out.data_ptr(), out.stride(0), out2.data_ptr(), out2.stride(0), b, cout, d3, h, w,
+            _flags(relu) | (LEA_CVS_TMAJOR if tmajor else 0), LEA_F32,
             probe=lambda: _op_record("cv_stem_f32_down2_kernel", 0.0,
                                      4.0 * (lmaps.numel() + rmaps.numel() + out.numel() + out2.numel())))
     return out, out2
```

After: 166.7 pairs/s (median of 6 runs). +1.5%, better.
